# lab4d-org/lab4d

Hardware: AMD Instinct MI355X
Metric: rendered rays/sec (fwd+bwd) at 512² × 128 samples; PSNR vs ref (higher is better)
Workload: dtype bf16

## Files before the change

include/lab4d_mlp.h:

```cpp
#ifndef LAB4D_MLP_H
#define LAB4D_MLP_H

#include <stdint.h>

#define LAB4D_MLP_MAX_LAYERS 12

#define LAB4D_NET_FG_BASE 0
#define LAB4D_NET_FG_COLOR 1
#define LAB4D_NET_VIS 2
#define LAB4D_NET_FEAT 3
#define LAB4D_NET_SKIN 4
#define LAB4D_NET_DENSE 5
#define LAB4D_NET_BG_BASE 6
#define LAB4D_NET_BG_COLOR 7
#define LAB4D_NET_SKIN18 8
#define LAB4D_NET_HASH_GEO 9
#define LAB4D_NET_HASH_COLOR 10
#define LAB4D_NET_DENSE6 11
#define LAB4D_NET_SKIN_A 12
#define LAB4D_NET_SKIN18_A 13
#define LAB4D_NET_COUNT 14

#define LAB4D_PREC_F32 0
#define LAB4D_PREC_BF16 1

typedef struct {
  int ke;
  int kin;
  int mout;
  int mout_pad;
  int relu;
  int pf_bias;
  int add_ext;
  int ext_grad;
} lab4d_mlp_layer;

typedef struct {
  int n_layers;
  int emb_kind;
  int n_freq;
  int c_in;
  int emb_slots;
  int ke;
  int c_out;
  lab4d_mlp_layer layers[LAB4D_MLP_MAX_LAYERS];
} lab4d_mlp_desc;

int lab4d_mlp_describe(int net, lab4d_mlp_desc* out);

int64_t lab4d_mlp_packed_bytes(int net, int layer, int precision);

int lab4d_mlp_pack(int net, int layer, int precision, int transposed, const float* W_ref, int k_ref,
                   const int32_t* col_map, void* packed, void* stream);

typedef struct {
  int net, precision;
  int S;
  int S_pad;
  int ld;
  int spf;
  const float* x;
  const float* freq_w;
  const void* W[LAB4D_MLP_MAX_LAYERS];
  const float* bias[LAB4D_MLP_MAX_LAYERS];
  const float* pf_bias[LAB4D_MLP_MAX_LAYERS];
  void* act[LAB4D_MLP_MAX_LAYERS];
  void* mask[LAB4D_MLP_MAX_LAYERS];
  void* emb;
  const void* ext;
  float* out;
  const float* x2;
  const int32_t* S_dev;
  const int32_t* frame_idx;
  const float* aff;
} lab4d_mlp_fwd_args;
int lab4d_mlp_forward(const lab4d_mlp_fwd_args* a, void* stream);

typedef struct {
  int net, precision, S, spf;
  const float* x;
  const float* freq_w;
  const float* aff;
  const void* W[LAB4D_MLP_MAX_LAYERS];
  const void* WT[LAB4D_MLP_MAX_LAYERS];
  const float* bias[LAB4D_MLP_MAX_LAYERS];
  const float* pf_bias[LAB4D_MLP_MAX_LAYERS];
  const float* d_out;
  float* d_x;
  float* g_aff;
  float* dW[LAB4D_MLP_MAX_LAYERS];
  float* db[LAB4D_MLP_MAX_LAYERS];
  float* pf_db[LAB4D_MLP_MAX_LAYERS];
} lab4d_mlp_bwd_fused_args;
int lab4d_mlp_backward_fused(const lab4d_mlp_bwd_fused_args* a, void* stream);
int lab4d_mlp_fused_backward_supported(int net, int precision, int spf);

int lab4d_mlp_forward_tangent(const lab4d_mlp_fwd_args* a, void* stream);

typedef struct {
  int net, precision, S, S_pad, ld, spf;
  const void* WT[LAB4D_MLP_MAX_LAYERS];
  const void* act[LAB4D_MLP_MAX_LAYERS];
  const void* mask[LAB4D_MLP_MAX_LAYERS];
  const void* emb;
  const void* ext;
  const float* d_out;
  const void* ext_gin;
  void* ext_gout;
  void* dz[LAB4D_MLP_MAX_LAYERS];
  float* d_x;
  float* d_x2;
  const float* x;
  const float* aff;
  float* g_aff;
} lab4d_mlp_bwd_args;
int lab4d_mlp_backward(const lab4d_mlp_bwd_args* a, void* stream);

int lab4d_mlp_wgrad(int net, int layer, int precision, int S, int S_pad, int ld, int spf, const void* dz, const void* emb,
                    const void* act_prev, float* dW, float* db, float* pf_db, int M, void* stream);
int lab4d_mlp_wgrad_mapped(int net, int layer, int precision, int S, int S_pad, int ld, int spf, const void* dz, const void* emb,
                           const void* act_prev, float* dW_ref, int ld_ref, const int32_t* col_map, float* db, float* pf_db, int M,
                           void* stream);

#endif
```

lab4d_amd/csrc/mlp.hip:

```cpp
#include <cstdlib>
#include "mlp_kernels.hpp"
#include "mlp_fused_bwd.hpp"

namespace lab4d {

struct DwMap {
  const int* cmap;
  int ld, mout, db_rows;
};
__device__ __forceinline__ int dw_col(int k, const DwMap& wm) { return wm.cmap ? wm.cmap[k] : k; }
__device__ __forceinline__ void dw_add(float* dW, int o, int c, int K, const DwMap& wm, float v) {
  if (wm.cmap) {
    if (c >= 0 && o < wm.mout) atomicAdd(dW + (size_t)o * wm.ld + c, v);
  } else {
    atomicAdd(dW + (size_t)o * K + c, v);
  }
}

template <class P, int TM>
__global__ void __launch_bounds__(256) k_mlp_wgrad(const typename P::store_t* __restrict__ dz, const typename P::store_t* __restrict__ emb,
                                                    const typename P::store_t* __restrict__ actp, int mo_tiles, int ke, int kin,
                                                    int S_pad, int chunk, int spf, int cpf, float* __restrict__ dW, float* __restrict__ db, DwMap wm) {
  constexpr int TN = 4;
  constexpr int SPS = P::BF16 ? 16 : 8;
  __shared__ float red[TM * TN * 16 * 64];
  const int lane = threadIdx.x & 63, wid = threadIdx.x >> 6, row = lane & 31, h = lane >> 5;
  const int K = ke + kin, nk_tiles = K / 32;
  const int ob_n = (mo_tiles + TM - 1) / TM, kb_n = (nk_tiles + TN - 1) / TN;
  const int job = blockIdx.x;
  const int c = job / (ob_n * kb_n), rem = job - c * (ob_n * kb_n);
  const int ob = rem / kb_n, kb = rem - ob * kb_n;
  int s_begin, s_end;
  if (cpf > 0) {
    const int m = c / cpf, lc = c - m * cpf;
    s_begin = m * spf + lc * chunk;
    s_end = min(min(S_pad, (m + 1) * spf), s_begin + chunk);
    if (db) db += (size_t)m * (mo_tiles * 32);
    if (s_end == (m + 1) * spf && S_pad - s_end < 64 && S_pad > s_end) s_end = S_pad;
  } else {
    s_begin = c * chunk;
    s_end = min(S_pad, s_begin + chunk);
  }

  f32x16_t acc[TM][TN];
#pragma unroll
  for (int i = 0; i < TM; ++i)
#pragma unroll
    for (int j = 0; j < TN; ++j)
#pragma unroll
      for (int r = 0; r < 16; ++r) acc[i][j][r] = 0.f;
  float rs[TM];
#pragma unroll
  for (int i = 0; i < TM; ++i) rs[i] = 0.f;

  const typename P::store_t* ap[TM];
  const typename P::store_t* bp[TN];
  bool av_[TM], bv_[TN];
  int bF[TN];
#pragma unroll
  for (int i = 0; i < TM; ++i) {
    const int t = ob * TM + i;
    av_[i] = t < mo_tiles;
    ap[i] = dz + (size_t)(32 * (av_[i] ? t : 0) + row) * 64;
  }
#pragma unroll
  for (int j = 0; j < TN; ++j) {
    const int t = kb * TN + j;
    bv_[j] = t < nk_tiles;
    const int kr = 32 * (bv_[j] ? t : 0) + row;
    bp[j] = kr < ke ? emb + (size_t)kr * 64 : actp + (size_t)(kr - ke) * 64;
    bF[j] = kr < ke ? ke : kin;
  }
  const int off = P::BF16 ? 8 * h : 4 * h;
  const int moF = mo_tiles * 32;
  auto load_step = [&](int s, uint4 (&a4)[TM], uint4 (&b4)[TN]) {
    const size_t blk = (size_t)(s >> 6);
    const int in = (s & 63) + off;
#pragma unroll
    for (int i = 0; i < TM; ++i) a4[i] = av_[i] ? *reinterpret_cast<const uint4*>(ap[i] + blk * block_stride(moF) + in) : make_uint4(0, 0, 0, 0);
#pragma unroll
    for (int j = 0; j < TN; ++j) b4[j] = bv_[j] ? *reinterpret_cast<const uint4*>(bp[j] + blk * block_stride(bF[j]) + in) : make_uint4(0, 0, 0, 0);
  };
  auto compute = [&](const uint4 (&a4)[TM], const uint4 (&b4)[TN]) {
    if (kb == 0 && db) {
#pragma unroll
      for (int i = 0; i < TM; ++i) {
        if constexpr (P::BF16) {
          const unsigned int w[4] = {a4[i].x, a4[i].y, a4[i].z, a4[i].w};
#pragma unroll
          for (int q = 0; q < 4; ++q) rs[i] += bf2f((unsigned short)(w[q] & 0xffffu)) + bf2f((unsigned short)(w[q] >> 16));
        } else {
          rs[i] += __uint_as_float(a4[i].x) + __uint_as_float(a4[i].y) + __uint_as_float(a4[i].z) + __uint_as_float(a4[i].w);
        }
      }
    }
#pragma unroll
    for (int i = 0; i < TM; ++i)
#pragma unroll
      for (int j = 0; j < TN; ++j) mma_unit<P>(acc[i][j], a4[i], b4[j]);
  };
  const int step = 4 * SPS;
  int s = s_begin + wid * SPS;
  uint4 a0[TM], b0[TN], a1[TM], b1[TN];
  if (s < s_end) load_step(s, a0, b0);
  while (s < s_end) {
    const int s1 = s + step;
    if (s1 < s_end) load_step(s1, a1, b1);
    compute(a0, b0);
    if (s1 >= s_end) break;
    const int s2 = s1 + step;
    if (s2 < s_end) load_step(s2, a0, b0);
    compute(a1, b1);
    s = s2;
  }
  if (wid == 0) {
#pragma unroll
    for (int i = 0; i < TM; ++i)
#pragma unroll
      for (int j = 0; j < TN; ++j)
#pragma unroll
        for (int r = 0; r < 16; ++r) red[((i * TN + j) * 16 + r) * 64 + lane] = acc[i][j][r];
  }
  __syncthreads();
  if (wid != 0) {
#pragma unroll
    for (int i = 0; i < TM; ++i)
#pragma unroll
      for (int j = 0; j < TN; ++j)
#pragma unroll
        for (int r = 0; r < 16; ++r) atomicAdd(&red[((i * TN + j) * 16 + r) * 64 + lane], acc[i][j][r]);
  }
  __syncthreads();
  for (int e = threadIdx.x; e < TM * TN * 16 * 64; e += 256) {
    const int l2 = e & 63, r = (e >> 6) & 15, ij = e >> 10;
    const int i = ij / TN, j = ij - i * TN;
    const int to = ob * TM + i, tk = kb * TN + j;
    if (to < mo_tiles && tk < nk_tiles) {
      const int o = 32 * to + drow(r, l2 >> 5);
      const int k = 32 * tk + (l2 & 31);
      dw_add(dW, o, dw_col(k, wm), K, wm, red[e]);
    }
  }
  if (kb == 0 && db) {
#pragma unroll
    for (int i = 0; i < TM; ++i) {
      const float v = rs[i] + __shfl_xor(rs[i], 32, 64);
      if (h == 0 && av_[i] && 32 * (ob * TM + i) + row < wm.db_rows) atomicAdd(db + 32 * (ob * TM + i) + row, v);
    }
  }
}

template <class P>
__global__ void __launch_bounds__(256) k_mlp_wgrad_big(const typename P::store_t* __restrict__ dz, const typename P::store_t* __restrict__ emb,
                                                        const typename P::store_t* __restrict__ actp, int mo_tiles, int ke, int kin,
                                                        int S_pad, int chunk, int spf, int cpf, float* __restrict__ dW, float* __restrict__ db, DwMap wm) {
  constexpr int TM = 4, TN = 4;
  constexpr int SPS = P::BF16 ? 16 : 8;
  const int lane = threadIdx.x & 63, wid = threadIdx.x >> 6, row = lane & 31, h = lane >> 5;
  const int wr = wid >> 1, wc = wid & 1;
  const int K = ke + kin, nk_tiles = K / 32;
  const int ob_n = (mo_tiles + 7) / 8, kb_n = (nk_tiles + 7) / 8;
  const int job = blockIdx.x;
  const int c = job / (ob_n * kb_n), rem = job - c * (ob_n * kb_n);
  const int ob = rem / kb_n, kb = rem - ob * kb_n;
  int s_begin, s_end;
  if (cpf > 0) {
    const int m = c / cpf, lc = c - m * cpf;
    s_begin = m * spf + lc * chunk;
    s_end = min(min(S_pad, (m + 1) * spf), s_begin + chunk);
    if (db) db += (size_t)m * (mo_tiles * 32);
  } else {
    s_begin = c * chunk;
    s_end = min(S_pad, s_begin + chunk);
  }
  f32x16_t acc[TM][TN];
#pragma unroll
  for (int i = 0; i < TM; ++i)
#pragma unroll
    for (int j = 0; j < TN; ++j)
#pragma unroll
      for (int r = 0; r < 16; ++r) acc[i][j][r] = 0.f;
  float rs[TM];
#pragma unroll
  for (int i = 0; i < TM; ++i) rs[i] = 0.f;
  const typename P::store_t* ap[TM];
  const typename P::store_t* bp[TN];
  bool av_[TM], bv_[TN];
  int bF[TN];
#pragma unroll
  for (int i = 0; i < TM; ++i) {
    const int t = ob * 8 + wr * 4 + i;
    av_[i] = t < mo_tiles;
    ap[i] = dz + (size_t)(32 * (av_[i] ? t : 0) + row) * 64;
  }
#pragma unroll
  for (int j = 0; j < TN; ++j) {
    const int t = kb * 8 + wc * 4 + j;
    bv_[j] = t < nk_tiles;
    const int kr = 32 * (bv_[j] ? t : 0) + row;
    bp[j] = kr < ke ? emb + (size_t)kr * 64 : actp + (size_t)(kr - ke) * 64;
    bF[j] = kr < ke ? ke : kin;
  }
  const bool any = (av_[0] && bv_[0]);
  const bool do_db = (kb == 0 && wc == 0 && db != nullptr);
  const int off = P::BF16 ? 8 * h : 4 * h;
  const int moF = mo_tiles * 32;
  auto load_step = [&](int s, uint4 (&a4)[TM], uint4 (&b4)[TN]) {
    const size_t blk = (size_t)(s >> 6);
    const int in = (s & 63) + off;
#pragma unroll
    for (int i = 0; i < TM; ++i) a4[i] = av_[i] ? *reinterpret_cast<const uint4*>(ap[i] + blk * block_stride(moF) + in) : make_uint4(0, 0, 0, 0);
#pragma unroll
    for (int j = 0; j < TN; ++j) b4[j] = bv_[j] ? *reinterpret_cast<const uint4*>(bp[j] + blk * block_stride(bF[j]) + in) : make_uint4(0, 0, 0, 0);
  };
  auto compute = [&](const uint4 (&a4)[TM], const uint4 (&b4)[TN]) {
    if (do_db) {
#pragma unroll
      for (int i = 0; i < TM; ++i) {
        if constexpr (P::BF16) {
          const unsigned int w[4] = {a4[i].x, a4[i].y, a4[i].z, a4[i].w};
#pragma unroll
          for (int q = 0; q < 4; ++q) rs[i] += bf2f((unsigned short)(w[q] & 0xffffu)) + bf2f((unsigned short)(w[q] >> 16));
        } else {
          rs[i] += __uint_as_float(a4[i].x) + __uint_as_float(a4[i].y) + __uint_as_float(a4[i].z) + __uint_as_float(a4[i].w);
        }
      }
    }
#pragma unroll
    for (int i = 0; i < TM; ++i)
#pragma unroll
      for (int j = 0; j < TN; ++j) mma_unit<P>(acc[i][j], a4[i], b4[j]);
  };
  if (any) {
    int s = s_begin;
    uint4 a0[TM], b0[TN], a1[TM], b1[TN];
    if (s < s_end) load_step(s, a0, b0);
    while (s < s_end) {
      const int s1 = s + SPS;
      if (s1 < s_end) load_step(s1, a1, b1);
      compute(a0, b0);
      if (s1 >= s_end) break;
      const int s2 = s1 + SPS;
      if (s2 < s_end) load_step(s2, a0, b0);
      compute(a1, b1);
      s = s2;
    }
#pragma unroll
    for (int i = 0; i < TM; ++i) {
      if (!av_[i]) continue;
#pragma unroll
      for (int j = 0; j < TN; ++j) {
        if (!bv_[j]) continue;
        const int c = dw_col(32 * (kb * 8 + wc * 4 + j) + row, wm);
#pragma unroll
        for (int r = 0; r < 16; ++r) {
          const int o = 32 * (ob * 8 + wr * 4 + i) + drow(r, h);
          dw_add(dW, o, c, K, wm, acc[i][j][r]);
        }
      }
      if (do_db) {
        const float v = rs[i] + __shfl_xor(rs[i], 32, 64);
        if (h == 0 && 32 * (ob * 8 + wr * 4 + i) + row < wm.db_rows) atomicAdd(db + 32 * (ob * 8 + wr * 4 + i) + row, v);
      }
    }
  }
}

__device__ __forceinline__ void dma_1k(const void* gsrc_lane, void* lds_wave_base) {
  __builtin_amdgcn_global_load_lds((const __attribute__((address_space(1))) unsigned int*)gsrc_lane,
                                   (__attribute__((address_space(3))) unsigned int*)lds_wave_base, 16, 0, 0);
}
template <int OFF>
__device__ __forceinline__ u32x4_t lds_read16(unsigned addr) {
  u32x4_t v;
  asm volatile("ds_read_b128 %0, %1 offset:%2" : "=v"(v) : "v"(addr), "n"(OFF));
  return v;
}

template <int V>
using IC = std::integral_constant<int, V>;

template <int N>
__device__ __forceinline__ void wait_vmcnt() {
  asm volatile("s_waitcnt vmcnt(%0)" ::"n"(N) : "memory");
}

template <int MT, int NBW, int NW = 4, int WC = 2>
__global__ void __launch_bounds__(64 * NW) k_mlp_wgrad_dma(const unsigned short* __restrict__ dz, const unsigned short* __restrict__ emb,
                                                        const unsigned short* __restrict__ actp, int ke, int kin, int S_pad, int chunk,
                                                        int spf, int cpf, float* __restrict__ dW, float* __restrict__ db, DwMap wm) {
  using P = PBF16;
  static_assert(NW == 4 || NW == 8, "wave grid");
  constexpr int WR = NW / WC;
  static_assert(WR * WC == NW && (2 * NBW) % WC == 0, "wave grid");
  constexpr int TM = MT / WR, TN = 2 * NBW / WC, MO = 32 * MT, KB = 64 * NBW;
  static_assert(TM >= 1 && TM * WR == MT, "row tiles per wave");
  constexpr int A_BYTES = MT * 2048, STAGE = A_BYTES + NBW * 4096;
  constexpr int NS0 = 65536 / STAGE, NSTAGE = NS0 < 4 ? 4 : (NS0 > 8 ? 8 : NS0);
  constexpr int PA = (2 * MT + NW - 1) / NW, PB = (4 * NBW + NW - 1) / NW, PW = PA + PB;
  static_assert(PA * NW == 2 * MT || MT == 1, "A pieces per wave (MT = 1: two pieces, the other waves re-fetch the last one)");
  constexpr int AHEAD = NSTAGE - 1;
  constexpr bool DB_MFMA = WC == 2;
  static_assert(PW * (NSTAGE - 2) <= 63, "vmcnt range");
  static_assert(TM + TN <= 15, "lgkmcnt range");
  static_assert(NSTAGE * STAGE <= 160 * 1024, "LDS");
  __shared__ __attribute__((aligned(16))) unsigned char lds[NSTAGE * STAGE];
  const int lane = threadIdx.x & 63, wid = __builtin_amdgcn_readfirstlane((int)(threadIdx.x >> 6)), row = lane & 31, h = lane >> 5;
  const int wr = wid / WC, wc = wid % WC;
  const int K = ke + kin;
  const int kb_n = (K + KB - 1) / KB;
  const int job = blockIdx.x;
  const int c = job / kb_n, kb = job - c * kb_n;
  int s_begin, s_end;
  if (cpf > 0) {
    const int m = c / cpf, lc = c - m * cpf;
    s_begin = m * spf + lc * chunk;
    s_end = min(min(S_pad, (m + 1) * spf), s_begin + chunk);
    if (db) db += (size_t)m * MO;
  } else {
    s_begin = c * chunk;
    s_end = min(S_pad, s_begin + chunk);
  }
  const int k0 = kb * KB, nb = min(KB, K - k0);
  const int n1 = k0 < ke ? min(nb, ke - k0) : 0;
  const int r2 = (k0 > ke ? k0 : ke) - ke;
  bool bv_[TN];
#pragma unroll
  for (int j = 0; j < TN; ++j) bv_[j] = (wc * TN + j) * 32 < nb;
  const bool do_db = (kb == 0 && wc == 0 && db != nullptr);

  f32x16_t acc[TM][TN];
#pragma unroll
  for (int i = 0; i < TM; ++i)
#pragma unroll
    for (int j = 0; j < TN; ++j)
#pragma unroll
      for (int r = 0; r < 16; ++r) acc[i][j][r] = 0.f;
  float rs[TM];
  f32x4_t dbacc[TM];
#pragma unroll
  for (int i = 0; i < TM; ++i) {
    rs[i] = 0.f;
    dbacc[i] = f32x4_t{0.f, 0.f, 0.f, 0.f};
  }

  const int lane_src = (lane >> 2) * 128 + (((lane & 3) ^ ((lane >> 4) & 3)) * 16);
  const int nbp = nb / 16;
  auto issue = [&](int st_idx, int buf) {
    int blk = (s_begin >> 6) + (st_idx >> 1);
    const int half = st_idx & 1;
#ifdef LAB4D_ABL_WGRAD_L2
    blk &= 31;
#endif
    unsigned char* st = lds + buf * STAGE;
    const unsigned char* ga = reinterpret_cast<const unsigned char*>(dz + (size_t)blk * block_stride(MO)) + half * 64 + lane_src;
#pragma unroll
    for (int p = 0; p < PA; ++p) {
      int piece = wid + NW * p;
      if constexpr (PA * NW != 2 * MT) piece = piece < 2 * MT ? piece : 2 * MT - 1;
      dma_1k(ga + piece * 2048, st + piece * 1024);
    }
    unsigned char* sb = st + A_BYTES;
    const unsigned char* g1 = reinterpret_cast<const unsigned char*>(emb + (size_t)blk * block_stride(ke) + (size_t)k0 * 64) + half * 64 + lane_src;
    const unsigned char* g2 = reinterpret_cast<const unsigned char*>(actp + (size_t)blk * block_stride(kin) + (size_t)r2 * 64) + half * 64 + lane_src;
#pragma unroll
    for (int p = 0; p < PB; ++p) {
      int q = wid + NW * p;
      q = q < nbp ? q : nbp - 1;
      const int r0 = 16 * q;
      const unsigned char* src = r0 < n1 ? g1 + (size_t)r0 * 128 : g2 + (size_t)(r0 - n1) * 128;
      dma_1k(src, sb + q * 1024);
    }
  };
  const unsigned lds_base = (unsigned)(size_t)(__attribute__((address_space(3))) unsigned char*)lds;
  const unsigned f = (row >> 2) & 3;
  const unsigned la0 = lds_base + (unsigned)((wr * TM * 32 + row) * 64) + ((unsigned)(h ^ f) * 16u);
  const unsigned lb0 = lds_base + (unsigned)A_BYTES + (unsigned)((wc * TN * 32 + row) * 64) + ((unsigned)(h ^ f) * 16u);
  auto read_frags = [&](int buf, auto subc, u32x4_t (&a4)[TM], u32x4_t (&b4)[TN]) {
    constexpr unsigned X = 32u * decltype(subc)::value;
    const unsigned xa = (la0 + (unsigned)buf * STAGE) ^ X, xb = (lb0 + (unsigned)buf * STAGE) ^ X;
    sfor<0, TM>([&](auto ic) { a4[decltype(ic)::value] = lds_read16<decltype(ic)::value * 2048>(xa); });
    sfor<0, TN>([&](auto jc) { b4[decltype(jc)::value] = lds_read16<decltype(jc)::value * 2048>(xb); });
  };
  auto wait_frags = [&](auto cntc, u32x4_t (&a4)[TM], u32x4_t (&b4)[TN]) {
    constexpr int CNT = decltype(cntc)::value;
    if constexpr (TM == 4) asm volatile("s_waitcnt lgkmcnt(%4)" : "+v"(a4[0]), "+v"(a4[1]), "+v"(a4[2]), "+v"(a4[3]) : "n"(CNT));
    else if constexpr (TM == 2) asm volatile("s_waitcnt lgkmcnt(%2)" : "+v"(a4[0]), "+v"(a4[1]) : "n"(CNT));
    else asm volatile("s_waitcnt lgkmcnt(%1)" : "+v"(a4[0]) : "n"(CNT));
    if constexpr (TN == 5) asm volatile("" : "+v"(b4[0]), "+v"(b4[1]), "+v"(b4[2]), "+v"(b4[3]), "+v"(b4[4]));
    else if constexpr (TN == 4) asm volatile("" : "+v"(b4[0]), "+v"(b4[1]), "+v"(b4[2]), "+v"(b4[3]));
    else if constexpr (TN == 3) asm volatile("" : "+v"(b4[0]), "+v"(b4[1]), "+v"(b4[2]));
    else if constexpr (TN == 2) asm volatile("" : "+v"(b4[0]), "+v"(b4[1]));
    else asm volatile("" : "+v"(b4[0]));
    __builtin_amdgcn_sched_barrier(0);
  };
  const unsigned one2 = (((lane & 15) ^ (lane >> 4)) & 1) == 0 ? 0x3f803f80u : 0u;
  const u32x4_t ones4 = {one2, one2, one2, one2};
  auto mfmas = [&](const u32x4_t (&a4)[TM], const u32x4_t (&b4)[TN]) {
    if (do_db) {
      if constexpr (DB_MFMA) {
        bf16x8_t ov;
        __builtin_memcpy(&ov, &ones4, 16);
#pragma unroll
        for (int i = 0; i < TM; ++i) {
          bf16x8_t av;
          __builtin_memcpy(&av, &a4[i], 16);
          dbacc[i] = __builtin_amdgcn_mfma_f32_16x16x32_bf16(av, ov, dbacc[i], 0, 0, 0);
        }
      } else {
#pragma unroll
        for (int i = 0; i < TM; ++i) {
          const unsigned int w[4] = {a4[i].x, a4[i].y, a4[i].z, a4[i].w};
#pragma unroll
          for (int q = 0; q < 4; ++q) rs[i] += bf2f((unsigned short)(w[q] & 0xffffu)) + bf2f((unsigned short)(w[q] >> 16));
        }
      }
    }
#pragma unroll
    for (int i = 0; i < TM; ++i)
#pragma unroll
      for (int j = 0; j < TN; ++j) {
        bf16x8_t av, bv;
        __builtin_memcpy(&av, &a4[i], 16);
        __builtin_memcpy(&bv, &b4[j], 16);
        acc[i][j] = __builtin_amdgcn_mfma_f32_32x32x16_bf16(av, bv, acc[i][j], 0, 0, 0);
      }
    __builtin_amdgcn_sched_barrier(0);
  };
  auto wait_landed = [&](int later) {
    if (later == NSTAGE - 2) wait_vmcnt<PW * (NSTAGE - 2)>();
    else {
      bool done = false;
      sfor<0, NSTAGE - 2>([&](auto rc) {
        constexpr int R = decltype(rc)::value;
        if (!done && later == R) { wait_vmcnt<PW * R>(); done = true; }
      });
    }
  };
  const int N = ((s_end >> 6) - (s_begin >> 6)) * 2;
  if (N > 0) {
    u32x4_t a0[TM], b0[TN], a1[TM], b1[TN];
#pragma unroll
    for (int i = 0; i < AHEAD; ++i)
      if (i < N) issue(i, i);
    wait_landed(min(AHEAD - 1, N - 1));
    __builtin_amdgcn_s_barrier();
    asm volatile("" ::: "memory");
    read_frags(0, IC<0>{}, a0, b0);
    int buf = 0;
    for (int s = 0; s < N; ++s) {
      const int prev = buf == 0 ? NSTAGE - 1 : buf - 1, next = buf + 1 == NSTAGE ? 0 : buf + 1;
      read_frags(buf, IC<1>{}, a1, b1);
      wait_frags(IC<TM + TN>{}, a0, b0);
      mfmas(a0, b0);
      wait_frags(IC<0>{}, a1, b1);
      if (s + 1 < N) {
        if (s + NSTAGE - 1 < N) issue(s + NSTAGE - 1, prev);
        wait_landed(min(NSTAGE - 2, N - 2 - s));
        __builtin_amdgcn_s_barrier();
        asm volatile("" ::: "memory");
        read_frags(next, IC<0>{}, a0, b0);
        __builtin_amdgcn_sched_barrier(0);
      }
      mfmas(a1, b1);
      buf = next;
    }
  }
#pragma unroll
  for (int i = 0; i < TM; ++i) {
#pragma unroll
    for (int j = 0; j < TN; ++j) {
      if (!bv_[j]) continue;
      const int c = dw_col(k0 + 32 * (wc * TN + j) + row, wm);
#pragma unroll
      for (int r = 0; r < 16; ++r) {
        const int o = 32 * (wr * TM + i) + drow(r, h);
        dw_add(dW, o, c, K, wm, acc[i][j][r]);
      }
    }
    if (do_db) {
      if constexpr (DB_MFMA) {
        if ((lane & 15) < 2) {
#pragma unroll
          for (int r = 0; r < 4; ++r) {
            const int o = 32 * (wr * TM + i) + 16 * (lane & 15) + 4 * (lane >> 4) + r;
            if (o < wm.db_rows) atomicAdd(db + o, dbacc[i][r]);
          }
        }
      } else {
        const float v = rs[i] + __shfl_xor(rs[i], 32, 64);
        if (h == 0 && 32 * (wr * TM + i) + row < wm.db_rows) atomicAdd(db + 32 * (wr * TM + i) + row, v);
      }
    }
  }
}

template <class P>
__global__ void __launch_bounds__(256) k_rowsum_pf(const typename P::store_t* __restrict__ dz, int mo_pad, int S, int ld, int spf,
                                                    int M, int nseg, float* __restrict__ pf_db) {
  constexpr int SEG = 4096;
  const int lane = threadIdx.x & 63;
  const long job = (long)blockIdx.x * 4 + (threadIdx.x >> 6);
  if (job >= (long)mo_pad * nseg) return;
  const int o = (int)(job / nseg), seg = (int)(job % nseg);
  const long b = (long)seg * SEG, e = min((long)S, b + SEG);
  const typename P::store_t* row = dz + (size_t)o * 64;
  long i = b;
  while (i < e) {
    const int m = (int)(i / spf);
    const long fe = min(e, (long)(m + 1) * spf);
    float s = 0.f;
    for (long k = i + lane; k < fe; k += 64) {
      const size_t idx = (size_t)(k >> 6) * block_stride(mo_pad) + (k & 63);
      if constexpr (P::BF16) s += bf2f(row[idx]);
      else s += row[idx];
    }
    s = wave_sum(s);
    if (lane == 0) atomicAdd(pf_db + (size_t)m * mo_pad + o, s);
    i = fe;
  }
}

template <class P>
__global__ void __launch_bounds__(256) k_pack(const float* __restrict__ Wref, int mout, int k_ref, const int32_t* __restrict__ col_map,
                                               int ke, int kin, int mo_pad, int transposed, typename P::store_t* __restrict__ out) {
  constexpr int EPL = P::BF16 ? 8 : 4;
  const int K = ke + kin;
  const int rows = transposed ? K : mo_pad;
  const int kdim = transposed ? mo_pad : K;
  const int G = kdim / P::FPG;
  const long total = (long)(rows / 32) * G * 64 * EPL;
  for (long e = (long)blockIdx.x * blockDim.x + threadIdx.x; e < total; e += (long)gridDim.x * blockDim.x) {
    const int j = (int)(e % EPL);
    const int lane = (int)((e / EPL) % 64);
    const int g = (int)((e / (EPL * 64)) % G);
    const int mt = (int)(e / ((long)EPL * 64 * G));
    const int row = 32 * mt + (lane & 31), h = lane >> 5;
    const int ge = transposed ? 0 : ke / P::FPG;
    int kk;
    if (g < ge) {
      kk = P::BF16 ? 16 * g + 8 * h + j : 2 * (4 * g + j) + h;
    } else {
      const int gg = g - ge;
      int b, r;
      if (P::BF16) { b = gg >> 1; r = 8 * (gg & 1) + j; }
      else { const int kap = 4 * gg + j; b = kap >> 4; r = kap & 15; }
      kk = (transposed ? 0 : ke) + 32 * b + drow(r, h);
    }
    const int o = transposed ? kk : row;
    const int c = transposed ? row : kk;
    float v = 0.f;
    if (o < mout && c < K) {
      const int cr = col_map[c];
      if (cr >= 0) v = Wref[(size_t)o * k_ref + cr];
    }
    if constexpr (P::BF16) out[e] = f2bf(v);
    else out[e] = v;
  }
}

}
using namespace lab4d;

namespace {

template <class F>
int with_net(int net, F&& f) {
  switch (net) {
    case LAB4D_NET_FG_BASE: return f(NetFgBase{});
    case LAB4D_NET_FG_COLOR: return f(NetFgColor{});
    case LAB4D_NET_VIS: return f(NetVis{});
    case LAB4D_NET_FEAT: return f(NetFeat{});
    case LAB4D_NET_SKIN: return f(NetSkin{});
    case LAB4D_NET_SKIN18: return f(NetSkin18{});
    case LAB4D_NET_SKIN_A: return f(NetSkinA{});
    case LAB4D_NET_SKIN18_A: return f(NetSkin18A{});
    case LAB4D_NET_DENSE: return f(NetDense{});
    case LAB4D_NET_DENSE6: return f(NetDense6{});
    case LAB4D_NET_BG_BASE: return f(NetBgBase{});
    case LAB4D_NET_BG_COLOR: return f(NetBgColor{});
    case LAB4D_NET_HASH_GEO: return f(NetHashGeo{});
    case LAB4D_NET_HASH_COLOR: return f(NetHashColor{});
    default: set_error("unknown net id %d", net); return LAB4D_EINVAL;
  }
}

}

extern "C" int lab4d_mlp_describe(int net, lab4d_mlp_desc* out) {
  LAB4D_REQUIRE(out, "mlp_describe: null out");
  memset(out, 0, sizeof(*out));
  return with_net(net, [&](auto n) { fill_desc<decltype(n)>(out); return LAB4D_OK; });
}

extern "C" int64_t lab4d_mlp_packed_bytes(int net, int layer, int precision) {
  lab4d_mlp_desc d;
  if (lab4d_mlp_describe(net, &d) != LAB4D_OK || layer < 0 || layer >= d.n_layers) return -1;
  const lab4d_mlp_layer& L = d.layers[layer];
  return (int64_t)L.mout_pad * (L.ke + L.kin) * (precision == LAB4D_PREC_BF16 ? 2 : 4);
}

extern "C" int lab4d_mlp_pack(int net, int layer, int precision, int transposed, const float* W_ref, int k_ref,
                              const int32_t* col_map, void* packed, void* stream) {
  lab4d_mlp_desc d;
  if (int e = lab4d_mlp_describe(net, &d)) return e;
  LAB4D_REQUIRE(layer >= 0 && layer < d.n_layers, "mlp_pack: bad layer %d", layer);
  LAB4D_REQUIRE(W_ref && col_map && packed, "mlp_pack: null pointer");
  const lab4d_mlp_layer& L = d.layers[layer];
  const long total = (long)L.mout_pad * (L.ke + L.kin);
  int grid = div_up(total, 256); if (grid > 2048) grid = 2048;
  if (precision == LAB4D_PREC_BF16)
    hipLaunchKernelGGL((k_pack<PBF16>), dim3(grid), dim3(256), 0, (hipStream_t)stream, W_ref, L.mout, k_ref, col_map, L.ke, L.kin,
                       L.mout_pad, transposed, (unsigned short*)packed);
  else if (precision == LAB4D_PREC_F32)
    hipLaunchKernelGGL((k_pack<PF32>), dim3(grid), dim3(256), 0, (hipStream_t)stream, W_ref, L.mout, k_ref, col_map, L.ke, L.kin,
                       L.mout_pad, transposed, (float*)packed);
  else { set_error("mlp_pack: bad precision %d", precision); return LAB4D_EINVAL; }
  return check_launch("mlp_pack");
}

extern "C" int lab4d_mlp_forward(const lab4d_mlp_fwd_args* a, void* stream) {
  LAB4D_REQUIRE(a, "mlp_forward: null args");
  LAB4D_REQUIRE(a->S >= 0 && a->S_pad >= a->S && a->S_pad % 256 == 0 && a->spf > 0 && a->ld >= a->S_pad && a->ld % 8 == 0,
                "mlp_forward: bad sizes (S_pad must be a multiple of 256) S=%d S_pad=%d ld=%d spf=%d", a->S, a->S_pad, a->ld, a->spf);
  LAB4D_REQUIRE(a->x && a->out, "mlp_forward: null x/out");
  if (a->S == 0) return LAB4D_OK;
  return with_net(a->net, [&](auto n) {
    using Net = decltype(n);
    FwdK k;
    memset(&k, 0, sizeof(k));
    k.S = a->S; k.S_pad = a->S_pad; k.ld = a->ld; k.spf = a->spf; k.x = a->x; k.freq_w = a->freq_w; k.emb = a->emb; k.ext = a->ext; k.out = a->out; k.x2 = a->x2;
    k.S_dev = a->S_dev; k.frame_idx = a->frame_idx; k.aff = a->aff;
    LAB4D_REQUIRE(!a->aff || Net::EMB != 0, "mlp_forward: aff is for the raw-input nets only");
    LAB4D_REQUIRE(Net::EMB != 2 || a->aff, "mlp_forward: this network needs the per-frame affine table aff (M, ke, 4)");
    LAB4D_REQUIRE(!Net::AUX3 || a->x2, "mlp_forward: this network needs the second input x2");
    LAB4D_REQUIRE(!(a->S_dev && a->emb), "mlp_forward: a device-side sample count is for the evaluation path (no stored activations)");
    for (int l = 0; l < Net::NL; ++l) {
      LAB4D_REQUIRE(a->W[l] && a->bias[l], "mlp_forward: layer %d weights/bias missing", l);
      LAB4D_REQUIRE(!Net::L[l].pf || a->pf_bias[l], "mlp_forward: layer %d needs a per-frame bias", l);
      LAB4D_REQUIRE(!Net::L[l].add_ext || a->ext, "mlp_forward: layer %d needs ext", l);
      if (a->emb && l + 1 < Net::NL) {
        LAB4D_REQUIRE(a->act[l] || (dx_only_ok<Net>() && !a->act[0]), "mlp_forward: training mode (emb != NULL) needs act[%d]", l);
        LAB4D_REQUIRE(!Net::L[l].relu || a->mask[l], "mlp_forward: training mode (emb != NULL) needs mask[%d]", l);
      }
      k.W[l] = a->W[l]; k.bias[l] = a->bias[l]; k.pf_bias[l] = a->pf_bias[l]; k.act[l] = a->act[l]; k.mask[l] = (unsigned int*)a->mask[l];
    }
    return launch_mlp_fwd<Net>(a->precision, k, a->S, (hipStream_t)stream);
  });
}

extern "C" int lab4d_mlp_backward(const lab4d_mlp_bwd_args* a, void* stream) {
  LAB4D_REQUIRE(a, "mlp_backward: null args");
  LAB4D_REQUIRE(a->S >= 0 && a->S_pad >= a->S && a->S_pad % 256 == 0 && a->spf > 0 && a->ld >= a->S_pad && a->ld % 8 == 0, "mlp_backward: bad sizes (S_pad must be a multiple of 256)");
  LAB4D_REQUIRE(a->d_out, "mlp_backward: null d_out");
  if (a->S == 0) return LAB4D_OK;
  return with_net(a->net, [&](auto n) {
    using Net = decltype(n);
    BwdK k;
    memset(&k, 0, sizeof(k));
    k.S = a->S; k.S_pad = a->S_pad; k.ld = a->ld; k.spf = a->spf; k.emb = a->emb; k.ext = a->ext; k.d_out = a->d_out; k.ext_gin = a->ext_gin;
    k.ext_gout = a->ext_gout; k.d_x = a->d_x; k.d_x2 = a->d_x2; k.x = a->x; k.aff = a->aff; k.g_aff = a->g_aff;
    if (Net::EMB == 2) {
      LAB4D_REQUIRE(a->x && a->aff && a->emb, "mlp_backward: this network needs x, aff and the stored embedding");
    } else {
      LAB4D_REQUIRE(!a->g_aff, "mlp_backward: g_aff is for the affine-first-layer nets only");
    }
    LAB4D_REQUIRE(!(a->d_x && Net::EMB == 0) || a->emb, "mlp_backward: d_x needs the stored embedding");
    for (int l = 0; l < Net::NL; ++l) {
      LAB4D_REQUIRE(a->WT[l], "mlp_backward: layer %d transposed weights missing", l);
      LAB4D_REQUIRE(!(Net::L[l].relu && l + 1 < Net::NL) || a->mask[l], "mlp_backward: layer %d ReLU mask missing", l);
      LAB4D_REQUIRE(!Net::L[l].ext_grad || a->ext_gin, "mlp_backward: layer %d needs ext_gin", l);
      LAB4D_REQUIRE(a->dz[l] || (dx_only_ok<Net>() && !a->dz[0] && a->d_x), "mlp_backward: dz[%d] missing (every layer's dZ is written, or none: point gradient only)", l);
      LAB4D_REQUIRE(!Net::L[l].add_ext || a->ext_gout, "mlp_backward: layer %d needs ext_gout", l);
      k.WT[l] = a->WT[l]; k.act[l] = a->act[l]; k.mask[l] = (const unsigned int*)a->mask[l]; k.dz[l] = a->dz[l];
    }
    return launch_mlp_bwd<Net>(a->precision, k, a->S, (hipStream_t)stream);
  });
}

extern "C" int lab4d_mlp_fused_backward_supported(int net, int precision, int spf) {
  if (precision != LAB4D_PREC_BF16 || spf <= 0 || spf % 64 != 0) return 0;
  static const int vis_env = getenv("LAB4D_FUSED_VIS") ? atoi(getenv("LAB4D_FUSED_VIS")) : 0;
  return net == LAB4D_NET_SKIN_A || net == LAB4D_NET_SKIN18_A || (net == LAB4D_NET_VIS && vis_env != 0);
}

extern "C" int lab4d_mlp_backward_fused(const lab4d_mlp_bwd_fused_args* a, void* stream) {
  LAB4D_REQUIRE(a, "mlp_backward_fused: null args");
  LAB4D_REQUIRE(lab4d_mlp_fused_backward_supported(a->net, a->precision, a->spf), "mlp_backward_fused: net %d / precision %d / spf %d not supported (bf16, narrow nets, spf %% 64 == 0)",
                a->net, a->precision, a->spf);
  LAB4D_REQUIRE(a->S >= 0 && a->x && a->d_out, "mlp_backward_fused: null x / d_out");
  if (a->S == 0) return LAB4D_OK;
  auto run = [&](auto n) {
    using Net = decltype(n);
    FusedK k;
    memset(&k, 0, sizeof(k));
    k.S = a->S; k.spf = a->spf; k.ntiles = (a->S + 63) / 64; k.x = a->x; k.freq_w = a->freq_w; k.aff = a->aff; k.d_out = a->d_out; k.d_x = a->d_x; k.g_aff = a->g_aff;
    LAB4D_REQUIRE(Net::EMB != 2 || a->aff, "mlp_backward_fused: this network needs the per-frame affine table aff");
    for (int l = 0; l < Net::NL; ++l) {
      LAB4D_REQUIRE(a->WT[l] && a->dW[l], "mlp_backward_fused: layer %d transposed weights / dW missing", l);
      LAB4D_REQUIRE(l + 1 == Net::NL || (a->W[l] && (Net::L[l].pf ? (const void*)a->pf_bias[l] : (const void*)a->bias[l])), "mlp_backward_fused: layer %d forward weights / bias missing", l);
      LAB4D_REQUIRE((((uintptr_t)a->W[l] | (uintptr_t)a->WT[l]) & 15) == 0, "mlp_backward_fused: packed weights must be 16-byte aligned");
      k.W[l] = a->W[l]; k.WT[l] = a->WT[l]; k.bias[l] = a->bias[l]; k.pf_bias[l] = a->pf_bias[l]; k.dW[l] = a->dW[l]; k.db[l] = a->db[l]; k.pf_db[l] = a->pf_db[l];
    }
    return launch_mlp_bwd_fused<Net>(k, (hipStream_t)stream);
  };
  switch (a->net) {
    case LAB4D_NET_VIS: return run(NetVis{});
    case LAB4D_NET_SKIN_A: return run(NetSkinA{});
    default: return run(NetSkin18A{});
  }
}

extern "C" int lab4d_mlp_wgrad(int net, int layer, int precision, int S, int S_pad, int ld, int spf, const void* dz, const void* emb,
                               const void* act_prev, float* dW, float* db, float* pf_db, int M, void* stream) {
  return lab4d_mlp_wgrad_mapped(net, layer, precision, S, S_pad, ld, spf, dz, emb, act_prev, dW, 0, nullptr, db, pf_db, M, stream);
}

extern "C" int lab4d_mlp_wgrad_mapped(int net, int layer, int precision, int S, int S_pad, int ld, int spf, const void* dz, const void* emb,
                                      const void* act_prev, float* dW, int ld_ref, const int32_t* col_map, float* db, float* pf_db, int M,
                                      void* stream) {
  lab4d_mlp_desc d;
  if (int e = lab4d_mlp_describe(net, &d)) return e;
  LAB4D_REQUIRE(layer >= 0 && layer < d.n_layers, "mlp_wgrad: bad layer %d", layer);
  const lab4d_mlp_layer& L = d.layers[layer];
  LAB4D_REQUIRE(dz && dW, "mlp_wgrad: null dz/dW");
  LAB4D_REQUIRE(col_map == nullptr || ld_ref > 0, "mlp_wgrad_mapped: a column map needs the reference row stride");
  LAB4D_REQUIRE(L.ke == 0 || emb, "mlp_wgrad: layer %d needs the stored embedding", layer);
  LAB4D_REQUIRE(L.kin == 0 || act_prev, "mlp_wgrad: layer %d needs the previous activation", layer);
  LAB4D_REQUIRE(S_pad % 64 == 0 && S_pad >= S && ld >= S_pad && ld % 8 == 0, "mlp_wgrad: bad S_pad/ld");
  if (S == 0) return LAB4D_OK;
  const int mo_tiles = L.mout_pad / 32, nk_tiles = (L.ke + L.kin) / 32;
  const bool big = mo_tiles >= 8;
  const int Kt = L.ke + L.kin;
  static const int head_dma = getenv("LAB4D_WGRAD_HEAD_DMA") ? atoi(getenv("LAB4D_WGRAD_HEAD_DMA")) : 1;
  const bool dma = precision == LAB4D_PREC_BF16 && (mo_tiles == 8 || mo_tiles == 4 || mo_tiles == 2 || (mo_tiles == 1 && head_dma && Kt <= 256));
  const int nbw = (dma && mo_tiles == 1) ? (Kt <= 128 ? 2 : 4)
                  : Kt <= 64 ? 1 : (Kt <= 128 ? 2 : (Kt <= 192 ? 3 : (Kt <= 256 ? 4 : (mo_tiles == 8 && Kt <= 320 ? 5 : 3))));
  const int TM = mo_tiles >= 4 ? 4 : (mo_tiles >= 2 ? 2 : 1);
  const int ob_n = dma ? 1 : (big ? div_up(mo_tiles, 8) : div_up(mo_tiles, TM));
  const int kb_n = dma ? div_up(Kt, 64 * nbw) : (big ? div_up(nk_tiles, 8) : div_up(nk_tiles, 4));
  static const int jobs_env = getenv("LAB4D_WGRAD_JOBS") ? atoi(getenv("LAB4D_WGRAD_JOBS")) : 0;
  const int jobs_target = jobs_env > 0 ? jobs_env : ((dma && mo_tiles < 8) ? 512 : 256);
  int nchunks = jobs_target / (ob_n * kb_n); if (nchunks < 1) nchunks = 1;
  int chunk = div_up(div_up(S_pad, nchunks), 256) * 256; if (chunk < 1024) chunk = 1024;
  const bool fold_pf = pf_db != nullptr && spf % 256 == 0 && M > 0 && (long)M * spf >= S;
  LAB4D_REQUIRE(pf_db == nullptr || fold_pf || (M > 0 && spf > 0 && (long)M * spf >= S), "mlp_wgrad: pf_db needs M and spf, with M * spf >= S");
  int cpf = 0;
  if (fold_pf) {
    if (chunk > spf) chunk = spf;
    cpf = div_up(spf, chunk);
    nchunks = cpf * M;
  } else {
    nchunks = div_up(S_pad, chunk);
  }
  const int jobs = ob_n * kb_n * nchunks;
  const dim3 grid(jobs), block(256), block8(512);
  float* db_arg = fold_pf ? pf_db : db;
  const DwMap wm = {col_map, ld_ref, L.mout, (col_map && !fold_pf) ? L.mout : L.mout_pad};
  hipStream_t st = (hipStream_t)stream;
#define WG(P, TMV) hipLaunchKernelGGL((k_mlp_wgrad<P, TMV>), grid, block, 0, st, (const typename P::store_t*)dz, (const typename P::store_t*)emb, \
                                      (const typename P::store_t*)act_prev, mo_tiles, L.ke, L.kin, S_pad, chunk, spf, cpf, dW, db_arg, wm)
#define WGB(P) hipLaunchKernelGGL((k_mlp_wgrad_big<P>), grid, block, 0, st, (const typename P::store_t*)dz, (const typename P::store_t*)emb, \
                                  (const typename P::store_t*)act_prev, mo_tiles, L.ke, L.kin, S_pad, chunk, spf, cpf, dW, db_arg, wm)
#define WGD(MTV, NBV) hipLaunchKernelGGL((k_mlp_wgrad_dma<MTV, NBV>), grid, block, 0, st, (const unsigned short*)dz, (const unsigned short*)emb, \
                                         (const unsigned short*)act_prev, L.ke, L.kin, S_pad, chunk, spf, cpf, dW, db_arg, wm)
#define WGD8(NBV) hipLaunchKernelGGL((k_mlp_wgrad_dma<8, NBV, 8>), grid, block8, 0, st, (const unsigned short*)dz, (const unsigned short*)emb, \
                                     (const unsigned short*)act_prev, L.ke, L.kin, S_pad, chunk, spf, cpf, dW, db_arg, wm)
#define WGD_NB(MTV) do { if (nbw == 1) WGD(MTV, 1); else if (nbw == 2) WGD(MTV, 2); else if (nbw == 3) WGD(MTV, 3); else WGD(MTV, 4); } while (0)
  if (dma) {
    if (mo_tiles == 8) {
      if (nbw == 1) WGD8(1); else if (nbw == 2) WGD8(2); else if (nbw == 3) WGD8(3); else if (nbw == 4) WGD8(4); else WGD8(5);
    } else if (mo_tiles == 4) WGD_NB(4); else if (mo_tiles == 2) WGD_NB(2);
    else if (nbw == 2) hipLaunchKernelGGL((k_mlp_wgrad_dma<1, 2, 4, 4>), grid, block, 0, st, (const unsigned short*)dz, (const unsigned short*)emb,
                                          (const unsigned short*)act_prev, L.ke, L.kin, S_pad, chunk, spf, cpf, dW, db_arg, wm);
    else hipLaunchKernelGGL((k_mlp_wgrad_dma<1, 4, 4, 4>), grid, block, 0, st, (const unsigned short*)dz, (const unsigned short*)emb,
                            (const unsigned short*)act_prev, L.ke, L.kin, S_pad, chunk, spf, cpf, dW, db_arg, wm);
  }
#undef WGD_NB
#undef WGD8
#undef WGD
  else if (precision == LAB4D_PREC_BF16) { if (big) WGB(PBF16); else if (TM == 4) WG(PBF16, 4); else if (TM == 2) WG(PBF16, 2); else WG(PBF16, 1); }
  else if (precision == LAB4D_PREC_F32) { if (big) WGB(PF32); else if (TM == 4) WG(PF32, 4); else if (TM == 2) WG(PF32, 2); else WG(PF32, 1); }
  else { set_error("mlp_wgrad: bad precision %d", precision); return LAB4D_EINVAL; }
#undef WGB
#undef WG
  if (int e = check_launch("mlp_wgrad")) return e;
  if (pf_db && !fold_pf) {
    const int nseg = div_up(S, 4096);
    const long jobs2 = (long)L.mout_pad * nseg;
    if (precision == LAB4D_PREC_BF16)
      hipLaunchKernelGGL((k_rowsum_pf<PBF16>), dim3(div_up(jobs2, 4)), dim3(256), 0, st, (const unsigned short*)dz, L.mout_pad, S, ld, spf, M, nseg, pf_db);
    else
      hipLaunchKernelGGL((k_rowsum_pf<PF32>), dim3(div_up(jobs2, 4)), dim3(256), 0, st, (const float*)dz, L.mout_pad, S, ld, spf, M, nseg, pf_db);
    return check_launch("mlp_rowsum_pf");
  }
  return LAB4D_OK;
}

namespace {
template <class Net>
int forward_tangent_impl(const lab4d_mlp_fwd_args* a, void* stream) {
  FwdK k;
  memset(&k, 0, sizeof(k));
  k.S = a->S; k.S_pad = a->S_pad; k.ld = a->ld; k.spf = a->spf; k.x = a->x; k.emb = a->emb; k.out = a->out;
  for (int l = 0; l < Net::NL; ++l) {
    LAB4D_REQUIRE(a->W[l], "mlp_forward_tangent: layer %d weights missing", l);
    LAB4D_REQUIRE(!(Net::L[l].relu) || a->mask[l], "mlp_forward_tangent: layer %d primal ReLU mask missing", l);
    LAB4D_REQUIRE(l + 1 == Net::NL || a->act[l], "mlp_forward_tangent: act[%d] missing", l);
    k.W[l] = a->W[l]; k.bias[l] = a->bias[l] ? a->bias[l] : (const float*)a->W[l]; k.act[l] = a->act[l]; k.mask[l] = (unsigned int*)a->mask[l];
  }
  return launch_mlp_fwd_tangent<Net>(a->precision, k, a->S, (hipStream_t)stream);
}
}

extern "C" int lab4d_mlp_forward_tangent(const lab4d_mlp_fwd_args* a, void* stream) {
  LAB4D_REQUIRE(a, "mlp_forward_tangent: null args");
  LAB4D_REQUIRE(a->net == LAB4D_NET_FG_BASE || a->net == LAB4D_NET_BG_BASE,
                "mlp_forward_tangent: only the basefield/sdf networks (fg, bg) have an eikonal term (got net %d)", a->net);
  LAB4D_REQUIRE(a->S >= 0 && a->S_pad >= a->S && a->S_pad % 256 == 0 && a->spf > 0, "mlp_forward_tangent: bad sizes (S_pad must be a multiple of 256)");
  LAB4D_REQUIRE(a->x && a->emb, "mlp_forward_tangent: null x / emb");
  if (a->S == 0) return LAB4D_OK;
  if (a->net == LAB4D_NET_FG_BASE) return forward_tangent_impl<NetFgBase>(a, stream);
  return forward_tangent_impl<NetBgBase>(a, stream);
}
```

lab4d_amd/csrc/mlp_kernels.hpp:

```cpp
#pragma once
#include <cstddef>
#include <cstdlib>
#include <type_traits>

#include "common.hpp"
#include "mlp_nets.hpp"

namespace lab4d {

typedef __attribute__((ext_vector_type(8))) short bf16x8_t;
typedef __attribute__((ext_vector_type(16))) float f32x16_t;

struct PBF16 {
  static constexpr bool BF16 = true;
  static constexpr int NT = 2, TILE = 64, FPG = 16, UPT = 2;
  using store_t = unsigned short;
};
struct PF32 {
  static constexpr bool BF16 = false;
  static constexpr int NT = 1, TILE = 32, FPG = 8, UPT = 4;
  using store_t = float;
};

__device__ __forceinline__ unsigned short f2bf(float x) {
// ... 639 lines not shown
            float w[4];
#pragma unroll
            for (int e = 0; e < 4; ++e) {
              float v0, v1;
              emb_pair<Net>(4 * g + e, x, a.freq_w, v0, v1);
              w[e] = h ? v1 : v0;
            }
            emb[t][g] = make_uint4(__float_as_uint(w[0]), __float_as_uint(w[1]), __float_as_uint(w[2]), __float_as_uint(w[3]));
          }
        }
      } else {
        const float* xr = stagef + (NT * n + t) * CINR;
#pragma unroll
        for (int g = 0; g < UE; ++g) {
          if constexpr (P::BF16) {
            float v[8];
#pragma unroll
            for (int j = 0; j < 8; ++j) {
              const int c = 16 * g + 8 * h + j;
              v[j] = c < CINR ? xr[c] : 0.f;
            }
            emb[t][g] = make_uint4(pack2bf(v[0], v[1]), pack2bf(v[2], v[3]), pack2bf(v[4], v[5]), pack2bf(v[6], v[7]));
          } else {
            float v[4];
#pragma unroll
            for (int e = 0; e < 4; ++e) {
              const int c = 2 * (4 * g + e) + h;
              v[e] = c < CINR ? xr[c] : 0.f;
            }
            emb[t][g] = make_uint4(__float_as_uint(v[0]), __float_as_uint(v[1]), __float_as_uint(v[2]), __float_as_uint(v[3]));
          }
        }
      }
    }
    if constexpr (ST) {
      const int q = n & 3, kq = n >> 2;
      GLOBAL_AS char* base = (GLOBAL_AS char*)a.emb + tile_base_offset<P>(KE, s0, 0);
#pragma unroll
      for (int g = 0; g < UE; ++g) {
        if constexpr (P::BF16) {
          const unsigned int w0[4] = {emb[0][g].x, emb[0][g].y, emb[0][g].z, emb[0][g].w};
          const unsigned int w1[4] = {emb[1][g].x, emb[1][g].y, emb[1][g].z, emb[1][g].w};
#pragma unroll
          for (int half = 0; half < 2; ++half) {
            unsigned int d[4];
#pragma unroll
            for (int jj = 0; jj < 4; ++jj) {
              const int j = 4 * half + jj;
              const unsigned int lo = (w0[j >> 1] >> (16 * (j & 1))) & 0xffffu, hi = (w1[j >> 1] >> (16 * (j & 1))) & 0xffffu;
              d[jj] = lo | (hi << 16);
            }
            quad_transpose(d, q);
            gst16(base + tile_lane_offset<P>(16 * g + 8 * h + 4 * half + q, kq), d[0], d[1], d[2], d[3]);
          }
        } else {
          unsigned int d[4] = {emb[0][g].x, emb[0][g].y, emb[0][g].z, emb[0][g].w};
          quad_transpose(d, q);
          gst16(base + tile_lane_offset<P>(2 * (4 * g + q) + h, kq), d[0], d[1], d[2], d[3]);
        }
      }
    }

#pragma nounroll
    for (int l = 0; l < Net::NL; ++l)
    sfor<0, Net::NL>([&](auto ri) {
      constexpr int R = decltype(ri)::value;
      if constexpr (fwd_rep<Net>(R) != R) return;
      constexpr unsigned MEMBERS = fwd_members<Net>(R);
      if (!((MEMBERS >> l) & 1u)) return;
      constexpr LS ls = Net::L[R];
      constexpr bool LAST = (R == Net::NL - 1);
      constexpr int MT = pad32(ls.mout) / 32;
      constexpr int GE = ls.ke / P::FPG, GA = ls.kin / P::FPG, G = GE + GA;
      constexpr int GL = G < ACG ? G : ACG, NQ = (GL + 3) / 4;
      const GLOBAL_AS void* Wl = KARG_PTR(FwdK, const void*, W, l);
      const GLOBAL_AS float* bl = KARG_PTR(FwdK, const float*, bias, l);
      const GLOBAL_AS float* pfl = KARG_PTR(FwdK, const float*, pf_bias, l);
      GLOBAL_AS unsigned int* maskl = KARG_PTR(FwdK, unsigned int*, mask, l);
      GLOBAL_AS void* actl = KARG_PTR(FwdK, void*, act, l);
      uint4 bin[NT][GA > 0 ? GA : 1];
#pragma unroll
      for (int t = 0; t < NT; ++t)
#pragma unroll
        for (int u = 0; u < GA; ++u) bin[t][u] = slab[(t * UW + u) * 64];
      constexpr int NB = (ls.pf != 0 && !TAN) ? NT : 1;
      auto load_bias = [&](int mt, f32x16_t (&bv)[NB]) {
        if constexpr (TAN) {
#pragma unroll
          for (int r = 0; r < 16; ++r) bv[0][r] = 0.f;
        } else {
#pragma unroll
          for (int t = 0; t < NB; ++t)
#pragma unroll
            for (int i = 0; i < 4; ++i) {
              const GLOBAL_AS float* src = (ls.pf != 0) ? pfl + (size_t)frame[t] * (32 * MT) : bl;
              const f32x4_t v = *(const GLOBAL_AS f32x4_t*)(src + 32 * mt + 8 * i + 4 * h);
              bv[t][4 * i + 0] = v.x; bv[t][4 * i + 1] = v.y; bv[t][4 * i + 2] = v.z; bv[t][4 * i + 3] = v.w;
            }
        }
      };
      auto mfma_tile = [&](auto has_pre, int pre, int rbuf, uint4 (&A)[G], f32x16_t (&bv)[NB], f32x16_t (&acc)[NT]) {
        constexpr bool PRE = decltype(has_pre)::value;
#pragma unroll
        for (int t = 0; t < NT; ++t) acc[t] = bv[NB == 1 ? 0 : t];
#pragma unroll
        for (int g = 0; g < G; ++g) {
#pragma unroll
          for (int t = 0; t < NT; ++t) mma_unit<P>(acc[t], A[g], g < GE ? emb[t][g < GE ? g : 0] : bin[t][g >= GE ? g - GE : 0]);
          if constexpr (PRE) {
            if (g >= GL) A[g] = load_a(Wl, G, pre, g, lane);
            else if (rbuf >= 0) A[g] = abuf[(rbuf * ACG + g) * 64 + lane];
          }
        }
        if constexpr (PRE) load_bias(pre, bv);
      };
      auto a_fetch = [&](int mt, uint4 (&stg)[NQ]) {
#pragma unroll
        for (int i = 0; i < NQ; ++i) {
          const int g = wid + 4 * i < GL ? wid + 4 * i : GL - 1;
          stg[i] = load_a(Wl, G, mt, g, lane);
        }
      };
      auto a_stash = [&](int buf, const uint4 (&stg)[NQ]) {
#pragma unroll
        for (int i = 0; i < NQ; ++i) {
          const int g = wid + 4 * i < GL ? wid + 4 * i : GL - 1;
          abuf[(buf * ACG + g) * 64 + lane] = stg[i];
        }
      };
      auto a_grab = [&](int buf, uint4 (&A)[G]) {
#pragma unroll
        for (int g = 0; g < GL; ++g) A[g] = abuf[(buf * ACG + g) * 64 + lane];
      };
      unsigned int tan_bits = 0;
      uint4 ext_raw[4];
      auto prefetch = [&](int mt) {
        if constexpr (TAN && ls.relu != 0) tan_bits = maskl[((size_t)tile * MT + mt) * 64 + lane];
        if constexpr (ls.add_ext != 0 && !TAN) load_tile_raw<P>((const GLOBAL_AS void*)a.ext, 32 * MT, s0, mt, lane, ext_raw);
      };
      constexpr bool PACKED = P::BF16 && !TAN && ls.add_ext == 0 && !LAST;
      auto epilogue = [&](int mt, f32x16_t (&acc)[NT], unsigned int (&w)[2][8], unsigned int& wbits) {
        if constexpr (PACKED) {
#pragma unroll
          for (int t = 0; t < NT; ++t) acc_fence_if<(want_occ<Net, P>() == 2)>(acc[t]);
#pragma unroll
          for (int t = 0; t < 2; ++t)
#pragma unroll
            for (int k = 0; k < 8; ++k) w[t][k] = pack2bf_op(acc[t][2 * k], acc[t][2 * k + 1]);
          if constexpr (ls.relu != 0) {
            if constexpr (ST) wbits = pk_alive_bits(w);
#pragma unroll
            for (int t = 0; t < 2; ++t)
#pragma unroll
              for (int k = 0; k < 8; ++k) w[t][k] = pk_relu_bf16(w[t][k]);
          }
#pragma unroll
          for (int t = 0; t < 2; ++t)
#pragma unroll
            for (int q = 0; q < 2; ++q) slab[(t * UW + 2 * mt + q) * 64] = make_uint4(w[t][4 * q], w[t][4 * q + 1], w[t][4 * q + 2], w[t][4 * q + 3]);
          return;
        }
        if constexpr (ls.relu != 0) {
          if constexpr (TAN) {
            const unsigned int bits = tan_bits;
#pragma unroll
            for (int t = 0; t < NT; ++t)
#pragma unroll
              for (int r = 0; r < 16; ++r)
                acc[t][r] = __uint_as_float(__float_as_uint(acc[t][r]) & (unsigned int)__builtin_amdgcn_sbfe((int)bits, mask_bit<P>(t, r), 1));
          } else {
            if constexpr (ST && !LAST) {
              unsigned int bits = 0;
#pragma unroll
              for (int t = 0; t < NT; ++t)
#pragma unroll
                for (int r = 0; r < 16; ++r) bits |= (acc[t][r] > 0.f ? 1u : 0u) << mask_bit<P>(t, r);
              maskl[((size_t)tile * MT + mt) * 64 + lane] = bits;
            }
#pragma unroll
            for (int t = 0; t < NT; ++t)
#pragma unroll
              for (int r = 0; r < 16; ++r) acc[t][r] = relu1(acc[t][r]);
          }
        }
        if constexpr (ls.add_ext != 0 && !TAN) {
          f32x16_t e[NT];
          tile_from_raw<P>(ext_raw, lane, e);
#pragma unroll
          for (int t = 0; t < NT; ++t)
#pragma unroll
            for (int r = 0; r < 16; ++r) acc[t][r] += e[t][r];
        }
        if constexpr (ST) {
          if constexpr (!LAST && ACTS) store_tile<P>(actl, 32 * MT, s0, mt, lane, acc);
        } else if constexpr (fwd_any_export<Net>(R)) {
          if (actl) store_tile<P>(actl, 32 * MT, s0, mt, lane, acc);
        }
        if constexpr (!LAST) {
#pragma unroll
          for (int t = 0; t < NT; ++t) {
            uint4 u[P::UPT];
            tile_to_units<P>(acc[t], u);
#pragma unroll
            for (int q = 0; q < P::UPT; ++q) slab[(t * UW + P::UPT * mt + q) * 64] = u[q];
          }
        } else if constexpr (head_staged<Net>() && !TAN) {
          static_assert(pad32(Net::COUT) == 32, "one row tile");
          __builtin_amdgcn_wave_barrier();
#pragma unroll
          for (int t = 0; t < NT; ++t)
#pragma unroll
            for (int r = 0; r < 16; ++r) {
              const int f = drow(r, h);
              if (f < Net::COUT) stagef[(NT * n + t) * Net::COUT + f] = acc[t][r];
            }
          __builtin_amdgcn_wave_barrier();
          if (a.out) stage_out(stagef, a.out, (long)s0 * Net::COUT, TILE * Net::COUT, (long)S_eff * Net::COUT - 1, lane);
          __builtin_amdgcn_wave_barrier();
        } else {
#pragma unroll
          for (int t = 0; t < NT; ++t)
#pragma unroll
            for (int r = 0; r < 16; ++r) {
              const int f = 32 * mt + drow(r, h);
              if (f < Net::COUT && sidx[t] < S_eff && a.out) a.out[(size_t)sidx[t] * Net::COUT + f] = acc[t][r];
            }
        }
      };
      auto flush = [&](int mt, const unsigned int (&w)[2][8], unsigned int wbits) {
        if constexpr (PACKED) {
          if constexpr (ST) {
            if constexpr (ls.relu != 0) maskl[((size_t)tile * MT + mt) * 64 + lane] = wbits;
            if constexpr (ACTS) store_tile_packed(actl, 32 * MT, s0, mt, lane, w);
          } else if constexpr (fwd_any_export<Net>(R)) {
            if (actl) store_tile_packed(actl, 32 * MT, s0, mt, lane, w);
          }
        }
      };
      uint4 A[G], stg[NQ];
      f32x16_t bv[NB];
      f32x16_t acc0[NT], acc1[NT];
      unsigned int pw[2][8], pbits = 0;
      wg_step_barrier();
      a_fetch(0, stg);
      a_stash(0, stg);
      if constexpr (MT > 1) {
        a_fetch(1, stg);
        a_stash(1, stg);
      }
      a_fetch(MT > 2 ? 2 : MT - 1, stg);
#pragma unroll
      for (int g = GL; g < G; ++g) A[g] = load_a(Wl, G, 0, g, lane);
      load_bias(0, bv);
      prefetch(0);
      wg_step_barrier();
      a_grab(0, A);
      constexpr int NSTEP = MT - 1, NPAIR = NSTEP / 2;
      mfma_tile(std::bool_constant<(MT > 1)>{}, 1, -1, A, bv, acc0);
      if constexpr (NPAIR > 0) {
#pragma nounroll
        for (int k = 0; k < 2 * NPAIR; k += 2) {
          wg_step_barrier();
          a_grab(1, A);
          mfma_tile(std::true_type{}, k + 2 < MT ? k + 2 : MT - 1, -1, A, bv, acc1);
          epilogue(k, acc0, pw, pbits);
          prefetch(k + 1);
          a_stash(0, stg);
          a_fetch(k + 3 < MT ? k + 3 : MT - 1, stg);
          flush(k, pw, pbits);
          wg_step_barrier();
          a_grab(0, A);
          mfma_tile(std::true_type{}, k + 3 < MT ? k + 3 : MT - 1, -1, A, bv, acc0);
          epilogue(k + 1, acc1, pw, pbits);
          prefetch(k + 2 < MT ? k + 2 : MT - 1);
          a_stash(1, stg);
          a_fetch(k + 4 < MT ? k + 4 : MT - 1, stg);
          flush(k + 1, pw, pbits);
        }
      }
      if constexpr (NSTEP % 2 == 1) {
        wg_step_barrier();
        a_grab(1, A);
        mfma_tile(std::false_type{}, 0, -1, A, bv, acc1);
        epilogue(MT - 2, acc0, pw, pbits);
        flush(MT - 2, pw, pbits);
        prefetch(MT - 1);
        epilogue(MT - 1, acc1, pw, pbits);
        flush(MT - 1, pw, pbits);
      } else {
        epilogue(MT - 1, acc0, pw, pbits);
        flush(MT - 1, pw, pbits);
      }
    });
  }
}

template <class Net>
constexpr int emb_layer_count() {
  int c = 0;
  for (int l = 0; l < Net::NL; ++l) c += Net::L[l].ke ? 1 : 0;
  return c;
}

template <class Net, class P, bool AU = true, bool DZ = true>
__global__ void __launch_bounds__(256, (want_occ<Net, P, true>())) k_mlp_bwd(BwdK a) {
  static_assert(Net::EMB == 0 || emb_layer_count<Net>() == 1, "raw-input nets may use the input in one layer only");
  constexpr int NT = P::NT, TILE = P::TILE, NL = Net::NL, UW = Slab<Net, P>::UW;
  constexpr int ACG = acache_g<Net, P>();
  __shared__ uint4 slab_all[4 * Slab<Net, P>::UNITS_PER_WAVE];
  __shared__ uint4 abuf0[ACG * 64];
  __shared__ uint4 abuf1[ACG * 64];
#define LAB4D_ABUF(buf) ((buf) ? abuf1 : abuf0)
  __shared__ float4 afftab[Net::EMB == 2 ? 4 * 96 : 1];
  constexpr int NGA = (Net::EMB == 2 && AU) ? (Net::KE / 32) * 16 * 4 : 1;
  float gacc[NGA];
#pragma unroll
  for (int i = 0; i < NGA; ++i) gacc[i] = 0.f;
  int gframe = -1;
  auto gram_flush = [&]() {
    if constexpr (Net::EMB == 2 && AU) {
      if (gframe >= 0 && a.g_aff != nullptr) {
#pragma unroll
        for (int i = 0; i < NGA; ++i) {
          float v = gacc[i];
#pragma unroll
          for (int off = 1; off < 32; off <<= 1) v += __shfl_xor(v, off, 64);
          const int mt = i / 64, r = (i >> 2) & 15, j = i & 3;
          if ((threadIdx.x & 31) == 0) atomicAdd(a.g_aff + ((size_t)gframe * Net::KE + 32 * mt + drow(r, (int)((threadIdx.x & 63) >> 5))) * 4 + j, v);
          gacc[i] = 0.f;
        }
      }
    }
  };
  const int lane = threadIdx.x & 63, n = lane & 31, h = lane >> 5;
  const int wid = __builtin_amdgcn_readfirstlane((int)(threadIdx.x >> 6));
  uint4* slab = slab_all + wid * Slab<Net, P>::UNITS_PER_WAVE + lane;
  float* stagef = reinterpret_cast<float*>(slab_all + wid * Slab<Net, P>::UNITS_PER_WAVE);
  const int wave = blockIdx.x * 4 + wid, nwaves = gridDim.x * 4;

  for (int tile = wave; tile < a.ntiles; tile += nwaves) {
    const int s0 = tile * TILE;
    int sidx[NT];
#pragma unroll
    for (int t = 0; t < NT; ++t) sidx[t] = s0 + NT * n + t;
    float dx[NT][3];
    float dx2[NT][3];
#pragma unroll
    for (int t = 0; t < NT; ++t) { dx[t][0] = dx[t][1] = dx[t][2] = 0.f; dx2[t][0] = dx2[t][1] = dx2[t][2] = 0.f; }
    float xs[NT][3];
    int frm[NT];
    float4* ltab = afftab + wid * 96;
    constexpr bool uni = AU;
    if constexpr (Net::EMB == 2) {
#pragma unroll
      for (int t = 0; t < NT; ++t) {
        const int sc = sidx[t] < a.S ? sidx[t] : a.S - 1;
        frm[t] = sc / a.spf;
#pragma unroll
        for (int k = 0; k < 3; ++k) xs[t][k] = ((const GLOBAL_AS float*)a.x)[(size_t)sc * 3 + k];
      }
      if constexpr (uni) {
        const int m = __builtin_amdgcn_readfirstlane(frm[0]);
        if (m != gframe) {
          gram_flush();
          gframe = m;
        }
        for (int e = lane; e < Net::KE; e += 64) {
          const f32x4_t r4 = *(const GLOBAL_AS f32x4_t*)((const GLOBAL_AS float4*)a.aff + (size_t)m * Net::KE + e);
          ltab[e] = make_float4(r4.x, r4.y, r4.z, r4.w);
        }
      }
      __builtin_amdgcn_wave_barrier();
    }

    {
      f32x16_t g[NT];
      if constexpr (head_staged<Net>()) {
        __builtin_amdgcn_wave_barrier();
        stage_in<TILE * Net::COUT>(stagef, a.d_out, (long)s0 * Net::COUT, (long)a.S * Net::COUT - 1, lane);
        __builtin_amdgcn_wave_barrier();
#pragma unroll
        for (int t = 0; t < NT; ++t)
#pragma unroll
          for (int r = 0; r < 16; ++r) {
            const int f = drow(r, h);
            g[t][r] = (f < Net::COUT && sidx[t] < a.S) ? stagef[(NT * n + t) * Net::COUT + (f < Net::COUT ? f : 0)] : 0.f;
          }
        __builtin_amdgcn_wave_barrier();
      } else {
#pragma unroll
      for (int t = 0; t < NT; ++t)
#pragma unroll
        for (int r = 0; r < 16; ++r) {
          const int f = drow(r, h);
          g[t][r] = (f < Net::COUT && sidx[t] < a.S) ? a.d_out[(size_t)sidx[t] * Net::COUT + f] : 0.f;
        }
      }
      if constexpr (DZ) store_tile<P>((GLOBAL_AS void*)a.dz[NL - 1], pad32(Net::L[NL - 1].mout), s0, 0, lane, g);
#pragma unroll
      for (int t = 0; t < NT; ++t) {
        uint4 u[P::UPT];
        tile_to_units<P>(g[t], u);
#pragma unroll
        for (int q = 0; q < P::UPT; ++q) slab[(t * UW + q) * 64] = u[q];
      }
    }

#pragma nounroll
    for (int l = NL - 1; l >= 0; --l)
    sfor<0, NL>([&](auto ri) {
      constexpr int R = NL - 1 - decltype(ri)::value;
      if constexpr (bwd_rep<Net>(R) != R) return;
      constexpr unsigned MEMBERS = bwd_members<Net>(R);
      if (!((MEMBERS >> l) & 1u)) return;
      constexpr LS ls = Net::L[R];
      constexpr LS lp = Net::L[R > 0 ? R - 1 : 0];
      constexpr int GK = pad32(ls.mout) / P::FPG;
      constexpr int GL = GK < ACG ? GK : ACG, NQ = (GL + 3) / 4;
      constexpr int MTE = ls.ke / 32, MTA = ls.kin / 32;
      constexpr bool DO_ACT = (R > 0 && MTA > 0);
      const int lm1 = l > 0 ? l - 1 : 0;
      const GLOBAL_AS void* Wt = KARG_PTR(BwdK, const void*, WT, l);
      const GLOBAL_AS unsigned int* maskp = KARG_PTR(BwdK, const unsigned int*, mask, lm1);
      GLOBAL_AS void* dzp = KARG_PTR(BwdK, void*, dz, lm1);
      uint4 bin[NT][GK];
#pragma unroll
      for (int t = 0; t < NT; ++t)
#pragma unroll
        for (int u = 0; u < GK; ++u) bin[t][u] = slab[(t * UW + u) * 64];

      auto mfma_tile = [&](auto has_pre, int pre, int rbuf, uint4 (&A)[GK], f32x16_t (&acc)[NT]) {
        constexpr bool PRE = decltype(has_pre)::value;
#pragma unroll
        for (int t = 0; t < NT; ++t)
#pragma unroll
          for (int r = 0; r < 16; ++r) acc[t][r] = 0.f;
        sfor<0, GK>([&](auto gc) {
          constexpr int g = decltype(gc)::value;
#pragma unroll
          for (int t = 0; t < NT; ++t) mma_unit<P>(acc[t], A[g], bin[t][g]);
          if constexpr (PRE) {
            if (g >= GL) A[g] = load_a(Wt, GK, pre, g, lane);
            else if (rbuf >= 0) A[g] = LAB4D_ABUF(rbuf)[g * 64 + lane];
          }
        });
      };
      auto a_fetch = [&](int mt, uint4 (&stg)[NQ]) {
#pragma unroll
        for (int i = 0; i < NQ; ++i) {
          const int g = wid + 4 * i < GL ? wid + 4 * i : GL - 1;
          stg[i] = load_a(Wt, GK, mt, g, lane);
        }
      };
      auto a_stash = [&](int buf, const uint4 (&stg)[NQ]) {
#pragma unroll
        for (int i = 0; i < NQ; ++i) {
          const int g = wid + 4 * i < GL ? wid + 4 * i : GL - 1;
          LAB4D_ABUF(buf)[g * 64 + lane] = stg[i];
        }
      };
      auto a_grab = [&](int buf, uint4 (&A)[GK]) {
#pragma unroll
        for (int g = 0; g < GL; ++g) A[g] = LAB4D_ABUF(buf)[g * 64 + lane];
      };
      auto pipeline = [&](auto n_c, int tile0, auto&& pre, auto&& epi, auto&& fl, auto&& prem) {
        constexpr int N = decltype(n_c)::value;
        if constexpr (N > 0) {
          uint4 A[GK], stg[NQ];
          f32x16_t acc0[NT], acc1[NT];
          unsigned int pw[2][8];
          wg_step_barrier();
          a_fetch(tile0, stg);
          a_stash(0, stg);
          if constexpr (N > 1) {
            a_fetch(tile0 + 1, stg);
            a_stash(1, stg);
          }
          a_fetch(tile0 + (N > 2 ? 2 : N - 1), stg);
#pragma unroll
          for (int g = GL; g < GK; ++g) A[g] = load_a(Wt, GK, tile0, g, lane);
          pre(0);
          prem(std::integral_constant<int, 0>{}, 0);
          prem(std::integral_constant<int, 1>{}, N > 1 ? 1 : 0);
          wg_step_barrier();
          a_grab(0, A);
          constexpr int NSTEP = N - 1, NPAIR = NSTEP / 2;
          mfma_tile(std::bool_constant<(N > 1)>{}, tile0 + 1, 1, A, acc0);
          if constexpr (N > 1) {
            wg_step_barrier();
            a_stash(0, stg);
            a_fetch(tile0 + (N > 3 ? 3 : N - 1), stg);
          }
          if constexpr (NPAIR > 0) {
#pragma nounroll
            for (int k = 0; k < 2 * NPAIR; k += 2) {
              wg_step_barrier();
              mfma_tile(std::true_type{}, tile0 + (k + 2 < N ? k + 2 : N - 1), 0, A, acc1);
              epi(k, acc0, pw);
              pre(k + 1);
              prem(std::integral_constant<int, 0>{}, k + 2 < N ? k + 2 : N - 1);
              a_stash(1, stg);
              a_fetch(tile0 + (k + 4 < N ? k + 4 : N - 1), stg);
              fl(k, pw);
              wg_step_barrier();
              mfma_tile(std::true_type{}, tile0 + (k + 3 < N ? k + 3 : N - 1), 1, A, acc0);
              epi(k + 1, acc1, pw);
              pre(k + 2 < N ? k + 2 : N - 1);
              prem(std::integral_constant<int, 1>{}, k + 3 < N ? k + 3 : N - 1);
              a_stash(0, stg);
              a_fetch(tile0 + (k + 5 < N ? k + 5 : N - 1), stg);
              fl(k + 1, pw);
            }
          }
          if constexpr (NSTEP % 2 == 1) {
            wg_step_barrier();
            mfma_tile(std::false_type{}, 0, -1, A, acc1);
            epi(N - 2, acc0, pw);
            fl(N - 2, pw);
            pre(N - 1);
            epi(N - 1, acc1, pw);
            fl(N - 1, pw);
          } else {
            epi(N - 1, acc0, pw);
            fl(N - 1, pw);
          }
        }
      };
      uint4 raw[4];
      unsigned int mb0 = 0, mb1 = 0;
      auto no_prem = [&](auto, int) {};
      auto pre_mask = [&](auto par_c, int j) {
        if constexpr (lp.relu != 0) {
          const unsigned int v = maskp[((size_t)tile * (pad32(lp.mout) / 32) + j) * 64 + lane];
          if constexpr (decltype(par_c)::value == 0) mb0 = v; else mb1 = v;
        }
      };
      auto pre_emb = [&](int mt) {
        if constexpr (Net::EMB != 1) load_tile_raw<P>((const GLOBAL_AS void*)a.emb, Net::KE, s0, mt, lane, raw);
      };
      auto pre_act = [&](int j) {
        if constexpr (lp.ext_grad != 0) load_tile_raw<P>((const GLOBAL_AS void*)a.ext_gin, pad32(lp.mout), s0, j, lane, raw);
      };
      auto no_flush = [&](int, const unsigned int (&)[2][8]) {};
      auto epi_emb = [&](int mt, f32x16_t (&acc)[NT], unsigned int (&)[2][8]) {
        if constexpr (Net::EMB == 0) {
          f32x16_t e[NT];
          tile_from_raw<P>(raw, lane, e);
          constexpr int L = Net::NFREQ;
#pragma unroll
          for (int t = 0; t < NT; ++t)
#pragma unroll
            for (int r = 0; r < 16; ++r) {
              const int slot = 32 * mt + drow(r, h);
              const float gv = acc[t][r];
              if (slot < 6 * L) {
                const int pair = slot >> 1, f = pair / 3, ax = pair - 3 * f;
                const float partner = e[t][r ^ 1];
                const float c = ldexpf((r & 1) ? -partner : partner, f) * gv;
                dx[t][0] += ax == 0 ? c : 0.f;
                dx[t][1] += ax == 1 ? c : 0.f;
                dx[t][2] += ax == 2 ? c : 0.f;
              } else if (slot < 6 * L + 3) {
                const int ax = slot - 6 * L;
                dx[t][0] += ax == 0 ? gv : 0.f;
                dx[t][1] += ax == 1 ? gv : 0.f;
                dx[t][2] += ax == 2 ? gv : 0.f;
              } else if (Net::AUX3 && slot < 6 * L + 6) {
                const int ax = slot - 6 * L - 3;
                dx2[t][0] += ax == 0 ? gv : 0.f;
                dx2[t][1] += ax == 1 ? gv : 0.f;
                dx2[t][2] += ax == 2 ? gv : 0.f;
              }
            }
        } else if constexpr (Net::EMB == 2) {
          f32x16_t e[NT];
          tile_from_raw<P>(raw, lane, e);
          auto body = [&](auto uni_c) {
            constexpr bool U = decltype(uni_c)::value;
            sfor<0, 16>([&](auto rc) {
              constexpr int r = decltype(rc)::value;
              const int slot = 32 * mt + drow(r, h);
              float4 row;
              if constexpr (U) row = ltab[slot];
#pragma unroll
              for (int t = 0; t < NT; ++t) {
                if constexpr (!U) {
                  const f32x4_t g4 = *(const GLOBAL_AS f32x4_t*)((const GLOBAL_AS float4*)a.aff + (size_t)frm[t] * Net::KE + slot);
                  row = make_float4(g4.x, g4.y, g4.z, g4.w);
                }
                const float dz = e[t][r] > 0.f ? acc[t][r] : 0.f;
                dx[t][0] += row.x * dz;
                dx[t][1] += row.y * dz;
                dx[t][2] += row.z * dz;
                if constexpr (U) {
                  sfor<0, Net::KE / 32>([&](auto mc) {
                    constexpr int mm = decltype(mc)::value;
                    if (mt == mm) {
                      gacc[(mm * 16 + r) * 4 + 0] += dz * xs[t][0];
                      gacc[(mm * 16 + r) * 4 + 1] += dz * xs[t][1];
                      gacc[(mm * 16 + r) * 4 + 2] += dz * xs[t][2];
                      gacc[(mm * 16 + r) * 4 + 3] += dz;
                    }
                  });
                } else if (a.g_aff != nullptr && dz != 0.f && sidx[t] < a.S) {
                  float* gp = a.g_aff + ((size_t)frm[t] * Net::KE + slot) * 4;
                  atomicAdd(gp + 0, dz * xs[t][0]);
                  atomicAdd(gp + 1, dz * xs[t][1]);
                  atomicAdd(gp + 2, dz * xs[t][2]);
                  atomicAdd(gp + 3, dz);
                }
              }
            });
          };
          body(std::bool_constant<uni>{});
        } else {
#pragma unroll
          for (int t = 0; t < NT; ++t)
#pragma unroll
            for (int r = 0; r < 16; ++r) {
              const int c = 32 * mt + drow(r, h);
              if (c < Net::CIN) stagef[(NT * n + t) * Net::CIN + c] = acc[t][r];
            }
        }
      };
      auto epi_act = [&](int j, f32x16_t (&acc)[NT], unsigned int (&w)[2][8]) {
        const unsigned int bits = (j & 1) ? mb1 : mb0;
        if constexpr (P::BF16) {
#pragma unroll
          for (int t = 0; t < NT; ++t) acc_fence_if<(want_occ<Net, P, true>() == 2)>(acc[t]);
        }
        if constexpr (lp.ext_grad != 0) {
          f32x16_t eg[NT];
          tile_from_raw<P>(raw, lane, eg);
#pragma unroll
          for (int t = 0; t < NT; ++t)
#pragma unroll
            for (int r = 0; r < 16; ++r) acc[t][r] += eg[t][r];
        }
        if constexpr (lp.add_ext != 0) {
          store_tile<P>((GLOBAL_AS void*)a.ext_gout, pad32(lp.mout), s0, j, lane, acc);
        }
        if constexpr (P::BF16) {
#pragma unroll
          for (int t = 0; t < 2; ++t)
#pragma unroll
            for (int k = 0; k < 8; ++k) w[t][k] = pack2bf_op(acc[t][2 * k], acc[t][2 * k + 1]);
          {
            unsigned int alive = lp.relu != 0 ? bits : 0xffffffffu;
#pragma unroll
            for (int t = 0; t < 2; ++t)
              if (sidx[t] >= a.S) alive &= ~(0x00ff00ffu << (8 * t));
#pragma unroll
            for (int t = 0; t < 2; ++t)
#pragma unroll
              for (int k = 0; k < 8; ++k) w[t][k] = pk_mask_bf16(w[t][k], pk_m01(alive, t, k));
          }
#pragma unroll
          for (int t = 0; t < 2; ++t)
#pragma unroll
            for (int q = 0; q < 2; ++q) slab[(t * UW + 2 * j + q) * 64] = make_uint4(w[t][4 * q], w[t][4 * q + 1], w[t][4 * q + 2], w[t][4 * q + 3]);
        } else {
          unsigned int keep = lp.relu != 0 ? bits : 0xffffffffu;
#pragma unroll
          for (int t = 0; t < NT; ++t)
            if (sidx[t] >= a.S) keep &= ~(0xffffu << (16 * t));
#pragma unroll
          for (int t = 0; t < NT; ++t)
#pragma unroll
            for (int r = 0; r < 16; ++r)
              acc[t][r] = __uint_as_float(__float_as_uint(acc[t][r]) & (unsigned int)__builtin_amdgcn_sbfe((int)keep, 16 * t + r, 1));
          if constexpr (DZ) store_tile<P>(dzp, pad32(lp.mout), s0, j, lane, acc);
#pragma unroll
          for (int t = 0; t < NT; ++t) {
            uint4 u[P::UPT];
            tile_to_units<P>(acc[t], u);
#pragma unroll
            for (int q = 0; q < P::UPT; ++q) slab[(t * UW + P::UPT * j + q) * 64] = u[q];
          }
        }
      };
      auto flush_act = [&](int j, const unsigned int (&w)[2][8]) {
        if constexpr (P::BF16 && DZ) store_tile_packed(dzp, pad32(lp.mout), s0, j, lane, w);
      };
      if constexpr (MTE > 0) {
        if (a.d_x != nullptr) {
          pipeline(std::integral_constant<int, MTE>{}, 0, pre_emb, epi_emb, no_flush, no_prem);
          if constexpr (Net::EMB == 1) stage_out(stagef, a.d_x, (long)s0 * Net::CIN, TILE * Net::CIN, (long)a.S * Net::CIN - 1, lane);
        }
      }
      if constexpr (DO_ACT) pipeline(std::integral_constant<int, MTA>{}, MTE, pre_act, epi_act, flush_act, pre_mask);
    });

    if constexpr (Net::EMB != 1) {
      if (a.d_x) {
#pragma unroll
        for (int t = 0; t < NT; ++t) {
#pragma unroll
          for (int k = 0; k < 3; ++k) dx[t][k] += __shfl_xor(dx[t][k], 32, 64);
          if (h == 0 && sidx[t] < a.S) {
            a.d_x[(size_t)sidx[t] * 3 + 0] = dx[t][0];
            a.d_x[(size_t)sidx[t] * 3 + 1] = dx[t][1];
            a.d_x[(size_t)sidx[t] * 3 + 2] = dx[t][2];
          }
          if constexpr (Net::AUX3) {
#pragma unroll
            for (int k = 0; k < 3; ++k) dx2[t][k] += __shfl_xor(dx2[t][k], 32, 64);
            if (h == 0 && sidx[t] < a.S && a.d_x2) {
              a.d_x2[(size_t)sidx[t] * 3 + 0] = dx2[t][0];
              a.d_x2[(size_t)sidx[t] * 3 + 1] = dx2[t][1];
              a.d_x2[(size_t)sidx[t] * 3 + 2] = dx2[t][2];
            }
          }
        }
      }
    }
  }
  gram_flush();
#undef LAB4D_ABUF
}

template <class Net>
int launch_mlp_fwd(int precision, const FwdK& k, int S, hipStream_t st);
template <class Net>
int launch_mlp_bwd(int precision, const BwdK& k, int S, hipStream_t st);
template <class Net>
int launch_mlp_fwd_tangent(int precision, const FwdK& k, int S, hipStream_t st);

template <auto kernel>
inline int mlp_grid(int ntiles) {
  static int per_cu = 0, n_cu = 0;
  if (per_cu == 0) {
    int nb = 0, dev = 0;
    hipDeviceProp_t prop;
    if (hipOccupancyMaxActiveBlocksPerMultiprocessor(&nb, kernel, 256, 0) != hipSuccess || nb < 1) nb = 1;
    if (hipGetDevice(&dev) != hipSuccess || hipGetDeviceProperties(&prop, dev) != hipSuccess) prop.multiProcessorCount = 256;
    n_cu = prop.multiProcessorCount > 0 ? prop.multiProcessorCount : 256;
    per_cu = nb > 2 ? 2 : nb;
  }
  int g = (ntiles + 3) / 4;
  if (g > n_cu * per_cu) g = n_cu * per_cu;
  static const int grid_env = getenv("LAB4D_CHAIN_GRID") ? atoi(getenv("LAB4D_CHAIN_GRID")) : 0;
  if (grid_env > 0 && g > grid_env * per_cu) g = grid_env * per_cu;
  return g < 1 ? 1 : g;
}
#define LAB4D_MLP_LAUNCH(KERNEL, k, st)                                                              \
  do {                                                                                               \
    constexpr auto kfn = &KERNEL;                                                                    \
    hipLaunchKernelGGL(kfn, dim3(mlp_grid<kfn>((k).ntiles)), dim3(256), 0, st, k);                   \
  } while (0)

}
#include "mlp_kernels_ws.hpp"
namespace lab4d {
template <class Net>
constexpr bool dx_only_ok() { return Net::ID == LAB4D_NET_FG_BASE || Net::ID == LAB4D_NET_BG_BASE; }
template <class Net>
inline bool launch_ws_bwd(const BwdK& k0, hipStream_t st) {
  if constexpr (ws_ok<Net>()) {
    if (!ws_enabled()) return false;
    if (!k0.dz[0]) {
      if constexpr (dx_only_ok<Net>()) {
        hipLaunchKernelGGL((k_mlp_bwd_ws<Net, false>), dim3(mlp_grid_ws(k0.S_pad / WS_TILE)), dim3(512), 0, st, k0);
        return true;
      }
      return false;
    }
    hipLaunchKernelGGL((k_mlp_bwd_ws<Net, true>), dim3(mlp_grid_ws(k0.S_pad / WS_TILE)), dim3(512), 0, st, k0);
    return true;
  } else {
    return false;
  }
}
template <class Net>
inline bool launch_ws_fwd(const FwdK& k0, hipStream_t st) {
  if constexpr (ws_ok<Net>()) {
    if (!ws_enabled()) return false;
    FwdK k = k0;
    if (k.emb && !k.act[0]) {
      if constexpr (dx_only_ok<Net>()) {
        hipLaunchKernelGGL((k_mlp_fwd_ws<Net, true, false>), dim3(mlp_grid_ws(k.S_pad / WS_TILE)), dim3(512), 0, st, k);
        return true;
      }
      return false;
    }
    if (k.emb) hipLaunchKernelGGL((k_mlp_fwd_ws<Net, true>), dim3(mlp_grid_ws(k.S_pad / WS_TILE)), dim3(512), 0, st, k);
    else hipLaunchKernelGGL((k_mlp_fwd_ws<Net, false>), dim3(mlp_grid_ws(k.S_pad / WS_TILE)), dim3(512), 0, st, k);
    return true;
  } else {
    return false;
  }
}

#define LAB4D_MLP_INSTANTIATE(Net)                                                                                        \
  namespace lab4d {                                                                                                       \
  template <>                                                                                                             \
  int launch_mlp_fwd<Net>(int precision, const FwdK& k0, int S, hipStream_t st) {                                         \
    FwdK k = k0;                                                                                                          \
    if (precision == LAB4D_PREC_BF16) {                                                                                   \
      if (launch_ws_fwd<Net>(k, st)) return check_launch("mlp_forward");                                                  \
      k.ntiles = k.S_pad / PBF16::TILE;                                                                                   \
      if (k.emb && !k.act[0]) {                                                                                           \
        if constexpr (dx_only_ok<Net>()) LAB4D_MLP_LAUNCH((k_mlp_fwd<Net, PBF16, false, true, false>), k, st);            \
      } else if (k.emb) LAB4D_MLP_LAUNCH((k_mlp_fwd<Net, PBF16, false, true>), k, st);  \
      else LAB4D_MLP_LAUNCH((k_mlp_fwd<Net, PBF16, false, false>), k, st);       \
    } else if (precision == LAB4D_PREC_F32) {                                                                             \
      k.ntiles = k.S_pad / PF32::TILE;                                                                                   \
      if (k.emb && !k.act[0]) {                                                                                           \
        if constexpr (dx_only_ok<Net>()) LAB4D_MLP_LAUNCH((k_mlp_fwd<Net, PF32, false, true, false>), k, st);             \
      } else if (k.emb) LAB4D_MLP_LAUNCH((k_mlp_fwd<Net, PF32, false, true>), k, st);   \
      else LAB4D_MLP_LAUNCH((k_mlp_fwd<Net, PF32, false, false>), k, st);        \
    } else {                                                                                                              \
      set_error("mlp_forward: bad precision %d", precision);                                                              \
      return LAB4D_EINVAL;                                                                                                \
    }                                                                                                                     \
    return check_launch("mlp_forward");                                                                                   \
  }                                                                                                                       \
  template <>                                                                                                             \
  int launch_mlp_bwd<Net>(int precision, const BwdK& k0, int S, hipStream_t st) {                                         \
    BwdK k = k0;                                                                                                          \
    if (precision == LAB4D_PREC_BF16) {                                                                                   \
      if (launch_ws_bwd<Net>(k, st)) return check_launch("mlp_backward");                                                 \
      k.ntiles = k.S_pad / PBF16::TILE;                                                                                   \
      if constexpr (Net::EMB == 2) {                                                                                      \
        if (k.spf % PBF16::TILE) LAB4D_MLP_LAUNCH((k_mlp_bwd<Net, PBF16, false>), k, st);                                 \
        else LAB4D_MLP_LAUNCH((k_mlp_bwd<Net, PBF16, true>), k, st);                                                      \
      } else if (!k.dz[0]) {                                                                                              \
        if constexpr (dx_only_ok<Net>()) LAB4D_MLP_LAUNCH((k_mlp_bwd<Net, PBF16, true, false>), k, st);                   \
      } else LAB4D_MLP_LAUNCH((k_mlp_bwd<Net, PBF16>), k, st);                         \
    } else if (precision == LAB4D_PREC_F32) {                                                                             \
      k.ntiles = k.S_pad / PF32::TILE;                                                                                   \
      if constexpr (Net::EMB == 2) {                                                                                      \
        if (k.spf % PF32::TILE) LAB4D_MLP_LAUNCH((k_mlp_bwd<Net, PF32, false>), k, st);                                   \
        else LAB4D_MLP_LAUNCH((k_mlp_bwd<Net, PF32, true>), k, st);                                                       \
      } else if (!k.dz[0]) {                                                                                              \
        if constexpr (dx_only_ok<Net>()) LAB4D_MLP_LAUNCH((k_mlp_bwd<Net, PF32, true, false>), k, st);                    \
      } else LAB4D_MLP_LAUNCH((k_mlp_bwd<Net, PF32>), k, st);                          \
    } else {                                                                                                              \
      set_error("mlp_backward: bad precision %d", precision);                                                             \
      return LAB4D_EINVAL;                                                                                                \
    }                                                                                                                     \
    return check_launch("mlp_backward");                                                                                  \
  }                                                                                                                       \
  }

}
```

lab4d_amd/csrc/mlp_kernels_ws.hpp:

```cpp
#pragma once
#include "mlp_kernels.hpp"

namespace lab4d {

template <class Net>
constexpr bool ws_ok() {
  if (!(Net::EMB == 0 && Net::AUX3 == 0 && net_wmax<Net>() == 256 && Net::KE % 32 == 0)) return false;
  for (int l = 0; l < Net::NL; ++l) {
    const int mt = pad32(Net::L[l].mout) / 32;
    if (!(mt == 1 || mt == 2 || mt == 4 || mt == 8)) return false;
    if (Net::L[l].kin % 32 != 0 || Net::L[l].kin > 256) return false;
    if (Net::L[l].ke != 0 && Net::L[l].ke != Net::KE) return false;
  }
  return true;
}
template <class Net>
constexpr int ws_g(int l) { return (Net::L[l].ke + Net::L[l].kin) / 16; }
template <class Net>
constexpr int ws_mt(int l) { return pad32(Net::L[l].mout) / 32; }
template <class Net>
constexpr int ws_gmax() {
  int g = 0;
  for (int l = 0; l < Net::NL; ++l) g = ws_g<Net>(l) > g ? ws_g<Net>(l) : g;
  return g;
// ... 317 lines not shown
          gst16(base + tile_lane_offset<P>(16 * g + 8 * h + 4 * half + q, kq), d[0], d[1], d[2], d[3]);
        }
      }
    }
    wg_step_barrier();

#pragma nounroll
    for (int l = 0; l < NL; ++l)
    sfor<0, NL>([&](auto ri) {
      constexpr int R = decltype(ri)::value;
      if constexpr (wsf_rep<Net>(R) != R) return;
      constexpr unsigned MEMBERS = wsf_members<Net>(R);
      if (!((MEMBERS >> l) & 1u)) return;
      constexpr LS ls = Net::L[R];
      constexpr bool LAST = (R == NL - 1);
      constexpr int MT = ws_mt<Net>(R), GE = ls.ke / 16, GA = ls.kin / 16, G = GE + GA;
      constexpr int Gn = ws_g<Net>((R + 1) % NL);
      using IT = WsItems<MT>;
      const GLOBAL_AS float* bl = KARG_PTR(FwdK, const float*, bias, l);
      const GLOBAL_AS float* pfl = KARG_PTR(FwdK, const float*, pf_bias, l);
      const int ln = l + 1 < NL ? l + 1 : 0;
      const GLOBAL_AS void* Wn = Wn_c;
      const int mtn = w & (ws_mt_rt<Net>(ln) - 1);
      const int ib = l & 1;
      const uint4* xin = xbuf + ib * WS_BUF;
      uint4* xout = xbuf + (ib ^ 1) * WS_BUF;
      const int mt = IT::mt(w);
      const bool active = IT::active(w);

      const bool bias_lds_path = ls.pf == 0 || tile_uni;
      u32x4_t br[4];
      auto load_bias = [&](int b, f32x16_t (&bv)[2]) {
        if (bias_lds_path) return;
#pragma unroll
        for (int t = 0; t < (ls.pf != 0 ? 2 : 1); ++t) {
          const int fr = frame[0][t] + b * (frame[1][t] - frame[0][t]);
          const GLOBAL_AS float* src = (ls.pf != 0) ? pfl + (size_t)fr * (32 * MT) : bl;
#pragma unroll
          for (int i = 0; i < 4; ++i) {
            const f32x4_t v = *(const GLOBAL_AS f32x4_t*)(src + 32 * mt + 8 * i + 4 * h);
            bv[t][4 * i + 0] = v.x; bv[t][4 * i + 1] = v.y; bv[t][4 * i + 2] = v.z; bv[t][4 * i + 3] = v.w;
          }
        }
        if constexpr (ls.pf == 0) bv[1] = bv[0];
      };
      uint4 ext_raw[4];
      auto load_ext = [&](int b) {
        if constexpr (ls.add_ext != 0) load_tile_raw<P>((const GLOBAL_AS void*)a.ext, 32 * MT, s0 + 64 * b, mt, lane, ext_raw);
      };

#pragma unroll
      for (int g = G; g < Gn; ++g) A[g] = load_a(Wn, Gn, mtn, g, lane);
      unsigned int tbits[2] = {0xffffffffu, 0xffffffffu};
      if constexpr (TAN && ls.relu != 0 && !LAST) {
        if (active) {
          const GLOBAL_AS unsigned int* mown = KARG_PTR(FwdK, unsigned int*, mask, l);
#pragma unroll
          for (int k = 0; k < IT::IPW; ++k) tbits[k] = mown[((size_t)(2 * tile + IT::blk(w, k)) * MT + mt) * 64 + lane];
        }
      }
      f32x16_t bv[2];
      if (active) {
        if (bias_lds_path) {
          const unsigned ba = lds_addr(bias_lds) + (unsigned)((l * 256 + 32 * mt + 4 * h) * 4);
          ws_lds_read<0>(br[0], ba);
          ws_lds_read<32>(br[1], ba);
          ws_lds_read<64>(br[2], ba);
          ws_lds_read<96>(br[3], ba);
        } else {
          load_bias(IT::blk(w, 0), bv);
        }
        load_ext(IT::blk(w, 0));
      }
      constexpr int MTp = R > 0 ? ws_mt<Net>(R > 0 ? R - 1 : 0) : 1;
      using ITp = WsItems<MTp>;
      constexpr int NP = R > 0 ? 4 * ITp::IPW : 0;
      constexpr int NHOST = IT::IPW;
      constexpr int NPI = NP / NHOST;
      constexpr bool SPREAD = ST && ACTS && R > 0 && !LAST && IT::ITEMS >= 8 && ITp::ITEMS >= 8 && NP % NHOST == 0 && WsSpread<G, (NPI > 0 ? NPI : 1)>::OK;
      GLOBAL_AS void* actp = act_c;
      GLOBAL_AS unsigned int* maskp = mask_c;
      const GLOBAL_AS void* Wn_n = KARG_PTR(FwdK, const void*, W, (ln + 1 < NL ? ln + 1 : 0));
      GLOBAL_AS void* act_n = KARG_PTR(FwdK, void*, act, l);
      GLOBAL_AS unsigned int* mask_n = KARG_PTR(FwdK, unsigned int*, mask, l);
      const int mtp = ITp::mt(w);
      if constexpr (R > 0 && !SPREAD) {
        auto flush_prev = [&]() {
#pragma unroll
          for (int k = 0; k < ITp::IPW; ++k) {
            const int b = ITp::blk(w, k);
            if constexpr (ACTS) {
              {
                const unsigned tb_ = xbuf_lds + (unsigned)(ib * WS_BUF * 16 + b * 2 * 16 * 1024 + mtp * 2048);
                ws_tr_issue(tb_ + trl, tb_ + trl2, trt);
              }
              tr_wait(trt);
              tr_store(actp, 32 * MTp, s0 + 64 * b, mtp, lane, trt);
            }
            if constexpr (ST && !TAN && Net::L[R > 0 ? R - 1 : 0].relu != 0) maskp[((size_t)(2 * tile + b) * MTp + mtp) * 64 + lane] = pbits[k];
          }
        };
        if constexpr (ST) {
          if (ITp::active(w)) flush_prev();
        } else {
          if (actp != nullptr && ITp::active(w)) flush_prev();
        }
      }
      WsPiece tp;

      if (active) {
        sfor<0, IT::IPW>([&](auto kc) {
          constexpr int k = decltype(kc)::value;
          const int b = IT::blk(w, k);
          constexpr int KL = IT::IPW - 1;
          f32x16_t acc[2];
          constexpr int BD = G < WS_BD ? G : WS_BD;
          u32x4_t bq[BD][2];
          const unsigned pe_a = ebuf_lds + (unsigned)((2 * b * UE) * 1024 + lane * 16), px_a = xbuf_lds + (unsigned)(ib * WS_BUF * 16 + (2 * b * 16) * 1024 + lane_s * 16);
          auto b_read = [&](auto gc, u32x4_t (&dst)[2]) {
            constexpr int g = decltype(gc)::value;
            if constexpr (g < GE) {
              ws_lds_read<g * 1024>(dst[0], pe_a);
              ws_lds_read<(UE + g) * 1024>(dst[1], pe_a);
            } else {
              ws_lds_read<(g - GE) * 1024>(dst[0], px_a);
              ws_lds_read<(16 + g - GE) * 1024>(dst[1], px_a);
            }
          };
          sfor<0, BD>([&](auto gc) { b_read(gc, bq[decltype(gc)::value]); });
          if constexpr (k == 0) {
            if (bias_lds_path) {
              ws_lds_wait4<2 * BD>(br);
#pragma unroll
              for (int i = 0; i < 4; ++i) {
                bv[0][4 * i + 0] = __uint_as_float(br[i].x); bv[0][4 * i + 1] = __uint_as_float(br[i].y);
                bv[0][4 * i + 2] = __uint_as_float(br[i].z); bv[0][4 * i + 3] = __uint_as_float(br[i].w);
              }
              bv[1] = bv[0];
            }
          }
          acc[0] = bv[0];
          acc[1] = bv[1];
          sfor<0, G>([&](auto gc) {
            constexpr int g = decltype(gc)::value;
            constexpr int NEWER = 2 * ((G - 1 - g) < (BD - 1) ? (G - 1 - g) : (BD - 1));
            ws_lds_wait<NEWER>(bq[g % BD][0], bq[g % BD][1]);
            mma_b(acc[0], A[g], bq[g % BD][0]);
            mma_b(acc[1], A[g], bq[g % BD][1]);
            if constexpr (SPREAD && k < NHOST) {
              using SP = WsSpread<G, (NPI > 0 ? NPI : 1)>;
              sfor<0, (SPREAD ? NPI : 0)>([&](auto ic) {
                constexpr int i = decltype(ic)::value, pi = k * NPI + i, kp = pi / 4, qa = pi % 4;
                if constexpr (SP::issue_at(i) == g) {
                  const unsigned tb_ = xbuf_lds + (unsigned)(ib * WS_BUF * 16 + ITp::blk(w, kp) * 2 * 16 * 1024 + mtp * 2048);
                  ws_trp_issue<qa>(tb_ + trl, tb_ + trl2, tp);
                }
              });
            }
            if constexpr (g + BD < G) b_read(std::integral_constant<int, g + BD>{}, bq[g % BD]);
            if constexpr (SPREAD && k < NHOST) {
              using SP = WsSpread<G, (NPI > 0 ? NPI : 1)>;
              sfor<0, (SPREAD ? NPI : 0)>([&](auto ic) {
                constexpr int i = decltype(ic)::value, pi = k * NPI + i, kp = pi / 4, qa = pi % 4;
                if constexpr (SP::perm_at(i) == g) ws_trp_perm<SP::newer(SP::issue_at(i), true, g, BD)>(tp);
                if constexpr (SP::store_at(i) == g) {
                  ws_trp_store<qa, SP::newer(SP::perm_at(i), false, g, BD)>(actp, 32 * MTp, s0 + 64 * ITp::blk(w, kp), mtp, lane, tp);
                  if constexpr (!TAN && qa == 3 && Net::L[R > 0 ? R - 1 : 0].relu != 0) maskp[((size_t)(2 * tile + ITp::blk(w, kp)) * MTp + mtp) * 64 + lane] = pbits[kp];
                }
              });
            }
            if (k == KL && g < Gn) A[g] = load_a(Wn, Gn, mtn, g, lane);
          });
          if (k < KL) {
            if constexpr (ls.pf != 0) load_bias(IT::blk(w, k + 1), bv);
          }
          if constexpr (!LAST && ls.add_ext == 0) {
#pragma unroll
            for (int t = 0; t < 2; ++t) acc_fence(acc[t]);
            unsigned int pw[2][8];
#pragma unroll
            for (int t = 0; t < 2; ++t)
#pragma unroll
              for (int kk = 0; kk < 8; ++kk) pw[t][kk] = pack2bf_op(acc[t][2 * kk], acc[t][2 * kk + 1]);
            if constexpr (ls.relu != 0 && TAN) {
#pragma unroll
              for (int t = 0; t < 2; ++t)
#pragma unroll
                for (int kk = 0; kk < 8; ++kk) pw[t][kk] = pk_mask_bf16(pw[t][kk], pk_m01(tbits[k], t, kk));
            } else if constexpr (ls.relu != 0) {
              if constexpr (ST) pbits[k] = pk_alive_bits(pw);
#pragma unroll
              for (int t = 0; t < 2; ++t)
#pragma unroll
                for (int kk = 0; kk < 8; ++kk) pw[t][kk] = pk_relu_bf16(pw[t][kk]);
            }
#pragma unroll
            for (int t = 0; t < 2; ++t)
#pragma unroll
              for (int q = 0; q < 2; ++q)
                xout[((2 * b + t) * 16 + 2 * mt + q) * 64 + lane_s] = make_uint4(pw[t][4 * q], pw[t][4 * q + 1], pw[t][4 * q + 2], pw[t][4 * q + 3]);
          } else if constexpr (!LAST) {
            if constexpr (ls.relu != 0) {
              if constexpr (ST) {
                unsigned int bits = 0;
#pragma unroll
                for (int t = 0; t < 2; ++t)
#pragma unroll
                  for (int r = 0; r < 16; ++r) bits |= (acc[t][r] > 0.f ? 1u : 0u) << mask_bit<P>(t, r);
                pbits[k] = bits;
              }
#pragma unroll
              for (int t = 0; t < 2; ++t)
#pragma unroll
                for (int r = 0; r < 16; ++r) acc[t][r] = relu1(acc[t][r]);
            }
            {
              f32x16_t e[2];
              tile_from_raw<P>(ext_raw, lane, e);
#pragma unroll
              for (int t = 0; t < 2; ++t)
#pragma unroll
                for (int r = 0; r < 16; ++r) acc[t][r] += e[t][r];
            }
            if (k < KL) load_ext(IT::blk(w, k + 1));
#pragma unroll
            for (int t = 0; t < 2; ++t) {
              uint4 u[2];
              tile_to_units<P>(acc[t], u);
#pragma unroll
              for (int q = 0; q < 2; ++q) xout[((2 * b + t) * 16 + 2 * mt + q) * 64 + lane_s] = u[q];
            }
          } else {
#pragma unroll
            for (int t = 0; t < 2; ++t) {
              const int s = s0 + 64 * b + 2 * n + t;
#pragma unroll
              for (int r = 0; r < 16; ++r) {
                const int f = 32 * mt + drow(r, h);
                if (f < Net::COUT && s < S_eff && a.out) a.out[(size_t)s * Net::COUT + f] = acc[t][r];
              }
            }
          }
        });
      } else {
        a_load(std::integral_constant<int, 0>{}, std::integral_constant<int, (Gn < G ? Gn : G)>{}, Wn, Gn, mtn);
      }
      ws_layer_barrier();
      Wn_c = Wn_n;
      act_c = act_n;
      mask_c = mask_n;
      ws_pin_sgpr(Wn_c);
      ws_pin_sgpr(act_c);
      ws_pin_sgpr(mask_c);
    });
    xcur = xnext;
  }
}

template <class Net>
constexpr int wsb_gk(int l) { return pad32(Net::L[l].mout) / 16; }
template <class Net>
constexpr bool wsb_same(int a, int b) {
  if (!bwd_same<Net>(a, b)) return false;
  if ((a == Net::NL - 1) != (b == Net::NL - 1)) return false;
  const int an = a > 0 ? a - 1 : Net::NL - 1, bn = b > 0 ? b - 1 : Net::NL - 1;
  return wsb_gk<Net>(an) == wsb_gk<Net>(bn);
}
template <class Net>
constexpr int wsb_rep(int l) {
  for (int j = Net::NL - 1; j > l; --j)
    if (wsb_same<Net>(j, l)) return j;
  return l;
}
template <class Net>
constexpr unsigned wsb_members(int r) {
  unsigned m = 0;
  for (int l = 0; l < Net::NL; ++l)
    if (wsb_rep<Net>(l) == r) m |= 1u << l;
  return m;
}
template <class Net>
__device__ __forceinline__ int wsb_first_tile(int l, int w, bool want_dx) {
  int v = 0;
  sfor<0, Net::NL>([&](auto ic) {
    constexpr int i = decltype(ic)::value;
    constexpr int MTE = Net::L[i].ke / 32, MTA = Net::L[i].kin / 32;
    if (l == i) {
      if (MTE > 0 && want_dx && w < 2 * MTE) v = w % (MTE > 0 ? MTE : 1);
      else v = (i > 0 && MTA > 0) ? MTE + (w & ((MTA > 0 ? MTA : 1) - 1)) : 0;
    }
  });
  return v;
}
template <class Net>
__device__ __forceinline__ int wsb_mta_rt(int l) {
  int v = 0;
  sfor<0, Net::NL>([&](auto ic) {
    constexpr int i = decltype(ic)::value;
    if (l == i) v = i > 0 ? Net::L[i].kin / 32 : 0;
  });
  return v;
}

template <class Net, bool DZ = true>
__global__ void __launch_bounds__(512) k_mlp_bwd_ws(BwdK a) {
  static_assert(ws_ok<Net>(), "weights-stationary chain: 256-wide posenc nets only");
  using P = PBF16;
  constexpr int NL = Net::NL, KE = Net::KE, GMAX = 16;
  constexpr int MTE_ANY = KE / 32;
  __shared__ uint4 xbuf[2 * WS_BUF];
  __shared__ float red[8 * 2 * 3 * 32];
  const int tid = threadIdx.x, lane = tid & 63, n = lane & 31, h = lane >> 5;
  const int w = __builtin_amdgcn_readfirstlane((int)(threadIdx.x >> 6));
  const unsigned xbuf_lds = lds_addr(xbuf);
  const unsigned trl = ws_tr_lane(lane), trl2 = trl ^ 32u;
  const int lane_s = ws_slot(lane);
  const int ntw = a.S_pad / WS_TILE;
  const bool want_dx = a.d_x != nullptr;

  uint4 A[GMAX];
  auto a_load = [&](auto g1c, const GLOBAL_AS void* Wp, int G, int rt) {
    constexpr int G1 = decltype(g1c)::value;
#pragma unroll
    for (int g = 0; g < G1; ++g) A[g] = load_a(Wp, G, rt, g, lane);
  };
  if ((int)blockIdx.x < ntw) {
    constexpr int GK0 = wsb_gk<Net>(NL - 1);
    a_load(std::integral_constant<int, GK0>{}, KARG_PTR(BwdK, const void*, WT, NL - 1), GK0, wsb_first_tile<Net>(NL - 1, w, want_dx));
  }
  TrTile trt;
  auto mask_slot_after = [](int ln_) { const int q = ln_ > 0 ? ln_ - 1 : 0; return q >= 1 ? q - 1 : 0; };
  const GLOBAL_AS void* Wn_c = KARG_PTR(BwdK, const void*, WT, (NL >= 2 ? NL - 2 : 0));
  GLOBAL_AS void* dz_c = KARG_PTR(BwdK, void*, dz, NL - 1);
  const GLOBAL_AS unsigned int* maskq_c = KARG_PTR(BwdK, const unsigned int*, mask, mask_slot_after(NL - 1));
  auto mask_req = [&](int lq , int tile, unsigned int (&m)[2], const GLOBAL_AS unsigned int* mp) {
    int mta = wsb_mta_rt<Net>(lq >= 1 ? lq : 1);
    mta = mta > 0 ? mta : 8;
    const int j = w & (mta - 1);
#pragma unroll
    for (int k = 0; k < 2; ++k) {
      const int b = mta >= 8 ? k : ((w / mta) & 1);
      m[k] = mp[((size_t)(2 * tile + b) * mta + j) * 64 + lane];
    }
  };

  constexpr bool DPRE = Net::COUT <= 4;
  constexpr int DN = DPRE ? Net::COUT : 1;
  auto d_fetch = [&](int tile_, float (&d)[2][DN]) {
    if constexpr (DPRE) {
      if (w < 2 && tile_ < ntw) {
#pragma unroll
        for (int t = 0; t < 2; ++t) {
          const int s = tile_ * WS_TILE + 64 * w + 2 * n + t;
#pragma unroll
          for (int r = 0; r < DN; ++r) {
            const int f = drow(r, h);
            d[t][r] = (f < Net::COUT && s < a.S) ? a.d_out[(size_t)s * Net::COUT + f] : 0.f;
          }
        }
      }
    }
  };
  float dcur[2][DN], dnext[2][DN];
#pragma unroll
  for (int t = 0; t < 2; ++t)
#pragma unroll
    for (int r = 0; r < DN; ++r) dcur[t][r] = dnext[t][r] = 0.f;
  d_fetch((int)blockIdx.x, dcur);
  for (int tile = blockIdx.x; tile < ntw; tile += gridDim.x) {
    const int s0 = tile * WS_TILE;
    d_fetch(tile + (int)gridDim.x, dnext);
    float dx[2][3];
#pragma unroll
    for (int t = 0; t < 2; ++t) dx[t][0] = dx[t][1] = dx[t][2] = 0.f;
    unsigned int mcur[2], mnext[2];
    mask_req(NL - 1, tile, mcur, KARG_PTR(BwdK, const unsigned int*, mask, (NL >= 2 ? NL - 2 : 0)));

    if (w < 2) {
      const int b = w;
      f32x16_t g[2];
#pragma unroll
      for (int t = 0; t < 2; ++t) {
        const int s = s0 + 64 * b + 2 * n + t;
#pragma unroll
        for (int r = 0; r < 16; ++r) {
          const int f = drow(r, h);
          if constexpr (DPRE) g[t][r] = r < DN ? dcur[t][r < DN ? r : 0] : 0.f;
          else g[t][r] = (f < Net::COUT && s < a.S) ? a.d_out[(size_t)s * Net::COUT + f] : 0.f;
        }
      }
      if constexpr (DZ) store_tile<P>((GLOBAL_AS void*)a.dz[NL - 1], pad32(Net::L[NL - 1].mout), s0 + 64 * b, 0, lane, g);
#pragma unroll
      for (int t = 0; t < 2; ++t) {
        uint4 u[2];
        tile_to_units<P>(g[t], u);
#pragma unroll
        for (int q = 0; q < 2; ++q) xbuf[((2 * b + t) * 16 + q) * 64 + lane_s] = u[q];
      }
    }
    wg_step_barrier();

#pragma nounroll
    for (int l = NL - 1; l >= 0; --l)
    sfor<0, NL>([&](auto ri) {
      constexpr int R = NL - 1 - decltype(ri)::value;
      if constexpr (wsb_rep<Net>(R) != R) return;
      constexpr unsigned MEMBERS = wsb_members<Net>(R);
      if (!((MEMBERS >> l) & 1u)) return;
      constexpr LS ls = Net::L[R];
      constexpr LS lp = Net::L[R > 0 ? R - 1 : 0];
      constexpr int GK = wsb_gk<Net>(R);
      constexpr int MTE = ls.ke / 32, MTA = ls.kin / 32;
      constexpr bool DO_ACT = (R > 0 && MTA > 0);
      constexpr int GKn = wsb_gk<Net>(R > 0 ? R - 1 : NL - 1);
      using IT = WsItems<(DO_ACT ? MTA : 1)>;
      const int lm1 = l > 0 ? l - 1 : 0;
      const int ln = l > 0 ? l - 1 : NL - 1;
      const GLOBAL_AS void* Wn = Wn_c;
      const GLOBAL_AS void* Wn_n = KARG_PTR(BwdK, const void*, WT, (ln > 0 ? ln - 1 : NL - 1));
      GLOBAL_AS void* dz_n = KARG_PTR(BwdK, void*, dz, ln);
      const GLOBAL_AS unsigned int* maskq_n = KARG_PTR(BwdK, const unsigned int*, mask, mask_slot_after(ln));
      const int rtn = wsb_first_tile<Net>(ln, w, want_dx);
      const int ib = (NL - 1 - l) & 1;
      uint4* xout = xbuf + (ib ^ 1) * WS_BUF;
      const bool act_on = DO_ACT && IT::active(w);
      const bool emb_on = MTE > 0 && want_dx && w < 2 * MTE;
      const int j = IT::mt(w);
      const int me = MTE > 0 ? w % (MTE > 0 ? MTE : 1) : 0, be = MTE > 0 ? (w / (MTE > 0 ? MTE : 1)) & 1 : 0;

#pragma unroll
      for (int g = GK; g < GKn; ++g) A[g] = load_a(Wn, GKn, rtn, g, lane);
      mask_req(lm1, tile, mnext, maskq_c);
      uint4 raw[4];
      if constexpr (MTE > 0) {
        if (emb_on) load_tile_raw<P>((const GLOBAL_AS void*)a.emb, KE, s0 + 64 * be, me, lane, raw);
      }
      if constexpr (DO_ACT && lp.ext_grad != 0) {
        if (act_on && !emb_on) load_tile_raw<P>((const GLOBAL_AS void*)a.ext_gin, pad32(lp.mout), s0 + 64 * IT::blk(w, 0), j, lane, raw);
      }
      static_assert(!(MTE > 0 && DO_ACT && lp.ext_grad != 0), "one prefetched tile per layer");
      constexpr int MTp = GK / 2;
      using ITp = WsItems<MTp>;
      constexpr int NP = (DZ && R < NL - 1) ? 4 * ITp::IPW : 0;
      constexpr int NHOST = IT::IPW;
      constexpr int NPI = NP / NHOST;
      constexpr bool SPREAD = NP > 0 && DO_ACT && IT::ITEMS >= 8 && ITp::ITEMS >= 8 && NP % NHOST == 0 && WsSpread<GK, (NPI > 0 ? NPI : 1)>::OK;
      GLOBAL_AS void* dzl = dz_c;
      const int jp = ITp::mt(w);
      if constexpr (NP > 0 && !SPREAD) {
        if (ITp::active(w)) {
#pragma unroll
          for (int k = 0; k < ITp::IPW; ++k) {
            const int b = ITp::blk(w, k);
            {
              const unsigned tb_ = xbuf_lds + (unsigned)(ib * WS_BUF * 16 + b * 2 * 16 * 1024 + jp * 2048);
              ws_tr_issue(tb_ + trl, tb_ + trl2, trt);
            }
            tr_wait(trt);
            tr_store(dzl, 32 * MTp, s0 + 64 * b, jp, lane, trt);
          }
        }
      }
      WsPiece tp;

      auto mfma_item = [&](int b, f32x16_t (&acc)[2], auto pf_c, auto gp_c, const GLOBAL_AS void* Wp, int rt, auto host_c) {
        constexpr bool PF = decltype(pf_c)::value;
        constexpr int GP = decltype(gp_c)::value;
        constexpr int HK = decltype(host_c)::value;
#pragma unroll
        for (int t = 0; t < 2; ++t)
#pragma unroll
          for (int r = 0; r < 16; ++r) acc[t][r] = 0.f;
        constexpr int BD = GK < WS_BD ? GK : WS_BD;
        u32x4_t bq[BD][2];
        const unsigned px_a = xbuf_lds + (unsigned)(ib * WS_BUF * 16 + (2 * b * 16) * 1024 + lane_s * 16);
        auto b_read = [&](auto gc, u32x4_t (&dst)[2]) {
          constexpr int g = decltype(gc)::value;
          ws_lds_read<g * 1024>(dst[0], px_a);
          ws_lds_read<(16 + g) * 1024>(dst[1], px_a);
        };
        sfor<0, BD>([&](auto gc) { b_read(gc, bq[decltype(gc)::value]); });
        sfor<0, GK>([&](auto gc) {
          constexpr int g = decltype(gc)::value;
          constexpr int NEWER = 2 * ((GK - 1 - g) < (BD - 1) ? (GK - 1 - g) : (BD - 1));
          ws_lds_wait<NEWER>(bq[g % BD][0], bq[g % BD][1]);
          mma_b(acc[0], A[g], bq[g % BD][0]);
          mma_b(acc[1], A[g], bq[g % BD][1]);
          if constexpr (SPREAD && HK >= 0 && HK < NHOST) {
            using SP = WsSpread<GK, (NPI > 0 ? NPI : 1)>;
            sfor<0, (SPREAD ? NPI : 0)>([&](auto ic) {
              constexpr int i = decltype(ic)::value, pi = (HK >= 0 ? HK : 0) * NPI + i, kp = pi / 4, qa = pi % 4;
              if constexpr (SP::issue_at(i) == g) {
                const unsigned tb_ = xbuf_lds + (unsigned)(ib * WS_BUF * 16 + ITp::blk(w, kp) * 2 * 16 * 1024 + jp * 2048);
                ws_trp_issue<qa>(tb_ + trl, tb_ + trl2, tp);
              }
            });
          }
          if constexpr (g + BD < GK) b_read(std::integral_constant<int, g + BD>{}, bq[g % BD]);
          if constexpr (SPREAD && HK >= 0 && HK < NHOST) {
            using SP = WsSpread<GK, (NPI > 0 ? NPI : 1)>;
            sfor<0, (SPREAD ? NPI : 0)>([&](auto ic) {
              constexpr int i = decltype(ic)::value, pi = (HK >= 0 ? HK : 0) * NPI + i, kp = pi / 4, qa = pi % 4;
              if constexpr (SP::perm_at(i) == g) ws_trp_perm<SP::newer(SP::issue_at(i), true, g, BD)>(tp);
              if constexpr (SP::store_at(i) == g) ws_trp_store<qa, SP::newer(SP::perm_at(i), false, g, BD)>(dzl, 32 * MTp, s0 + 64 * ITp::blk(w, kp), jp, lane, tp);
            });
          }
          if constexpr (PF && g < GP) A[g] = load_a(Wp, GP, rt, g, lane);
        });
      };

      bool loaded_next = false;
      if constexpr (MTE > 0) {
        if (emb_on) {
          f32x16_t acc[2];
          if constexpr (DO_ACT) mfma_item(be, acc, std::true_type{}, std::integral_constant<int, GK>{}, KARG_PTR(BwdK, const void*, WT, l), MTE + j, std::integral_constant<int, -1>{});
          else { mfma_item(be, acc, std::true_type{}, std::integral_constant<int, GKn>{}, Wn, rtn, std::integral_constant<int, -1>{}); loaded_next = true; }
          f32x16_t e[2];
          tile_from_raw<P>(raw, lane, e);
          constexpr int L = Net::NFREQ;
          sfor<0, (MTE > 0 ? MTE : 1)>([&](auto mc) {
            constexpr int MEc = decltype(mc)::value;
            if (me != MEc) return;
            sfor<0, 16>([&](auto rc) {
              constexpr int r = decltype(rc)::value;
              constexpr int S0 = 32 * MEc + (r & 3) + 8 * (r >> 2), S1 = S0 + 4;
              constexpr int K0 = S0 < 6 * L ? 1 : (S0 < 6 * L + 3 ? 2 : 0), K1 = S1 < 6 * L ? 1 : (S1 < 6 * L + 3 ? 2 : 0);
              if constexpr (K0 != 0 || K1 != 0) {
                constexpr int F0 = (S0 >> 1) / 3, F1 = (S1 >> 1) / 3;
                constexpr int A0 = K0 == 1 ? (S0 >> 1) % 3 : (K0 == 2 ? S0 - 6 * L : -1), A1 = K1 == 1 ? (S1 >> 1) % 3 : (K1 == 2 ? S1 - 6 * L : -1);
#pragma unroll
                for (int t = 0; t < 2; ++t) {
                  const float gv = acc[t][r];
                  const float partner = e[t][r ^ 1];
                  const float sp = (r & 1) ? -partner : partner;
                  float c;
                  if constexpr (K0 == 1 && K1 == 1) {
                    c = ldexpf(sp, h ? F1 : F0) * gv;
                  } else {
                    const float c0 = K0 == 1 ? ldexpf(sp, F0) * gv : (K0 == 2 ? gv : 0.f);
                    const float c1 = K1 == 1 ? ldexpf(sp, F1) * gv : (K1 == 2 ? gv : 0.f);
                    c = h ? c1 : c0;
                  }
#pragma unroll
                  for (int k = 0; k < 3; ++k) {
                    if (A0 == k && A1 == k) dx[t][k] += c;
                    else if (A0 == k) dx[t][k] += h ? 0.f : c;
                    else if (A1 == k) dx[t][k] += h ? c : 0.f;
                  }
                }
              }
            });
          });
        }
      }
      if constexpr (DO_ACT) {
        if (act_on) {
          sfor<0, IT::IPW>([&](auto kc) {
            constexpr int k = decltype(kc)::value;
            const int b = IT::blk(w, k);
            constexpr int KL = IT::IPW - 1;
              f32x16_t acc[2];
            if constexpr (k == KL) mfma_item(b, acc, std::true_type{}, std::integral_constant<int, GKn>{}, Wn, rtn, kc);
            else mfma_item(b, acc, std::false_type{}, std::integral_constant<int, 0>{}, Wn, rtn, kc);
            if constexpr (lp.ext_grad != 0) {
              f32x16_t eg[2];
              tile_from_raw<P>(raw, lane, eg);
#pragma unroll
              for (int t = 0; t < 2; ++t)
#pragma unroll
                for (int r = 0; r < 16; ++r) acc[t][r] += eg[t][r];
              if (k < KL) load_tile_raw<P>((const GLOBAL_AS void*)a.ext_gin, pad32(lp.mout), s0 + 64 * IT::blk(w, k + 1), j, lane, raw);
            }
            if constexpr (lp.add_ext != 0) store_tile<P>((GLOBAL_AS void*)a.ext_gout, pad32(lp.mout), s0 + 64 * b, j, lane, acc);
#pragma unroll
            for (int t = 0; t < 2; ++t) acc_fence(acc[t]);
            unsigned int pw[2][8];
#pragma unroll
            for (int t = 0; t < 2; ++t)
#pragma unroll
              for (int kk = 0; kk < 8; ++kk) pw[t][kk] = pack2bf_op(acc[t][2 * kk], acc[t][2 * kk + 1]);
            {
              unsigned int alive = lp.relu != 0 ? mcur[k] : 0xffffffffu;
#pragma unroll
              for (int t = 0; t < 2; ++t)
                if (s0 + 64 * b + 2 * n + t >= a.S) alive &= ~(0x00ff00ffu << (8 * t));
#pragma unroll
              for (int t = 0; t < 2; ++t)
#pragma unroll
                for (int kk = 0; kk < 8; ++kk) pw[t][kk] = pk_mask_bf16(pw[t][kk], pk_m01(alive, t, kk));
            }
#pragma unroll
            for (int t = 0; t < 2; ++t)
#pragma unroll
              for (int q = 0; q < 2; ++q)
                xout[((2 * b + t) * 16 + 2 * j + q) * 64 + lane_s] = make_uint4(pw[t][4 * q], pw[t][4 * q + 1], pw[t][4 * q + 2], pw[t][4 * q + 3]);
          });
          loaded_next = true;
        }
      }
      if (!loaded_next) a_load(std::integral_constant<int, (GKn < GK ? GKn : GK)>{}, Wn, GKn, rtn);
      mcur[0] = mnext[0];
      mcur[1] = mnext[1];
      ws_layer_barrier();
      Wn_c = Wn_n;
      dz_c = dz_n;
      maskq_c = maskq_n;
      ws_pin_sgpr(Wn_c);
      ws_pin_sgpr(dz_c);
      ws_pin_sgpr(maskq_c);
    });

#pragma unroll
    for (int t = 0; t < 2; ++t)
#pragma unroll
      for (int r = 0; r < DN; ++r) dcur[t][r] = dnext[t][r];
    if (want_dx) {
      if (w < 2 * MTE_ANY) {
#pragma unroll
        for (int t = 0; t < 2; ++t)
#pragma unroll
          for (int k = 0; k < 3; ++k) {
            const float v = dx[t][k] + __shfl_xor(dx[t][k], 32, 64);
            if (h == 0) red[((w * 2 + t) * 3 + k) * 32 + n] = v;
          }
      }
      wg_step_barrier();
      if (w < 2 && h == 0) {
        const int b = w;
#pragma unroll
        for (int t = 0; t < 2; ++t) {
          const int s = s0 + 64 * b + 2 * n + t;
          float v[3] = {0.f, 0.f, 0.f};
#pragma unroll
          for (int m = 0; m < MTE_ANY; ++m)
#pragma unroll
            for (int k = 0; k < 3; ++k) v[k] += red[(((b * MTE_ANY + m) * 2 + t) * 3 + k) * 32 + n];
          if (s < a.S) {
            a.d_x[(size_t)s * 3 + 0] = v[0];
            a.d_x[(size_t)s * 3 + 1] = v[1];
            a.d_x[(size_t)s * 3 + 2] = v[2];
          }
        }
      }
    }
  }
}

inline int mlp_grid_ws(int ntiles) {
  static int n_cu = 0;
  if (n_cu == 0) {
    int dev = 0;
    hipDeviceProp_t prop;
    if (hipGetDevice(&dev) != hipSuccess || hipGetDeviceProperties(&prop, dev) != hipSuccess) prop.multiProcessorCount = 256;
    n_cu = prop.multiProcessorCount > 0 ? prop.multiProcessorCount : 256;
  }
  const char* ge = getenv("LAB4D_CHAIN_GRID");
  const int grid_env = ge ? atoi(ge) : 0;
  int g = ntiles < n_cu ? ntiles : n_cu;
  if (grid_env > 0 && g > grid_env) g = grid_env;
  return g < 1 ? 1 : g;
}

inline bool ws_enabled() {
  const char* e = getenv("LAB4D_WS");
  return e == nullptr || atoi(e) != 0;
}

}
```

lab4d_amd/mlp.py:

```python
import ctypes
import os
import weakref
from typing import NamedTuple

import torch
from torch.autograd import Function
from torch.autograd.function import once_differentiable

from . import _lib

MAXL = 12
PREC_F32, PREC_BF16 = 0, 1
vp, ci = ctypes.c_void_p, ctypes.c_int


@_lib.mirrors("lab4d_mlp_layer")
class LayerDesc(ctypes.Structure):
    _fields_ = [(n, ci) for n in ("ke", "kin", "mout", "mout_pad", "relu", "pf_bias", "add_ext", "ext_grad")]


@_lib.mirrors("lab4d_mlp_desc")
class NetDesc(ctypes.Structure):
    _fields_ = [(n, ci) for n in ("n_layers", "emb_kind", "n_freq", "c_in", "emb_slots", "ke", "c_out")] + [("layers", LayerDesc * MAXL)]


@_lib.mirrors("lab4d_mlp_fwd_args")
class FwdArgs(ctypes.Structure):
    _fields_ = [("net", ci), ("precision", ci), ("S", ci), ("S_pad", ci), ("ld", ci), ("spf", ci), ("x", vp), ("freq_w", vp),
                ("W", vp * MAXL), ("bias", vp * MAXL), ("pf_bias", vp * MAXL), ("act", vp * MAXL), ("mask", vp * MAXL), ("emb", vp),
                ("ext", vp), ("out", vp), ("x2", vp), ("S_dev", vp), ("frame_idx", vp), ("aff", vp)]


@_lib.mirrors("lab4d_mlp_bwd_args")
class BwdArgs(ctypes.Structure):
    _fields_ = [("net", ci), ("precision", ci), ("S", ci), ("S_pad", ci), ("ld", ci), ("spf", ci), ("WT", vp * MAXL), ("act", vp * MAXL),
                ("mask", vp * MAXL), ("emb", vp), ("ext", vp), ("d_out", vp), ("ext_gin", vp), ("ext_gout", vp), ("dz", vp * MAXL), ("d_x", vp),
                ("d_x2", vp), ("x", vp), ("aff", vp), ("g_aff", vp)]


@_lib.mirrors("lab4d_mlp_bwd_fused_args")
class BwdFusedArgs(ctypes.Structure):
    _fields_ = [("net", ci), ("precision", ci), ("S", ci), ("spf", ci), ("x", vp), ("freq_w", vp), ("aff", vp), ("W", vp * MAXL), ("WT", vp * MAXL),
                ("bias", vp * MAXL), ("pf_bias", vp * MAXL), ("d_out", vp), ("d_x", vp), ("g_aff", vp), ("dW", vp * MAXL), ("db", vp * MAXL),
                ("pf_db", vp * MAXL)]


class NetInfo(NamedTuple):
    id: int
    name: str
    kernel: str
    macs: int
    ws: bool


NETS = (
    NetInfo(0, "fg_base", "FgBase", 572928 + 256, True),
    NetInfo(1, "fg_color", "FgColor", 158464 + 37248, True),
    NetInfo(2, "vis", "Vis", 10240, False),
    NetInfo(3, "feat", "Feat", 77568, False),
    NetInfo(4, "skin", "Skin", 20736, False),
    NetInfo(5, "dense", "Dense", 39 * 256 + 256 * 256 + 256 * 3, True),
    NetInfo(6, "bg_base", "BgBase", 100096 + 128, False),
    NetInfo(7, "bg_color", "BgColor", 43392 + 8576, False),
    NetInfo(8, "skin18", "Skin18", (54 + 160) * 64 + 64 * 64 + 64 * 18, False),
    NetInfo(9, "hash_geo", "HashGeo", 32 * 64 + 64 * 16, False),
    NetInfo(10, "hash_color", "HashColor", 19 * 64 + 64 * 64 + 64 * 3, False),
    NetInfo(11, "dense6", "Dense6", 199 * 256 + 3 * 256 * 256 + 455 * 256 + 256 * 256 + 256 * 3, True),
    NetInfo(12, "skin_a", "SkinA", 4 * 64 + 64 * 64 + 64 * 25, False),
    NetInfo(13, "skin18_a", "Skin18A", 4 * 64 + 64 * 64 + 64 * 18, False),
)
(NET_FG_BASE, NET_FG_COLOR, NET_VIS, NET_FEAT, NET_SKIN, NET_DENSE, NET_BG_BASE, NET_BG_COLOR, NET_SKIN18, NET_HASH_GEO, NET_HASH_COLOR, NET_DENSE6,
 NET_SKIN_A, NET_SKIN18_A) = (n.id for n in NETS)
NET_NAMES = {n.id: n.name for n in NETS}
KERNEL_NET = {n.id: n.kernel for n in NETS}
NET_MACS = {n.id: n.macs for n in NETS}
WS_NETS = tuple(n.id for n in NETS if n.ws)


def ws_active(net, prec, dx_only=False):
    e = os.environ.get("LAB4D_WS")
    try:
        on = e is None or int(e.strip() or "0") != 0
    except ValueError:
        on = False
    return bool(on and prec == PREC_BF16 and net in WS_NETS)


def chain_kernel_name(kind, net, prec, dx_only=False):
    return "k_mlp_%s%s<%s>" % (kind, "_ws" if ws_active(net, prec, dx_only) else "", KERNEL_NET[net])


def wgrad_kernel_name(L, prec):
    if prec == PREC_BF16 and L.mout_pad == 32 and os.environ.get("LAB4D_WGRAD_HEAD_DMA", "1") not in ("", "0") and L.ke + L.kin <= 256:
        return "k_mlp_wgrad_dma<1,%d>" % (2 if L.ke + L.kin <= 128 else 4)
    if prec == PREC_BF16 and L.mout_pad in (64, 128, 256):
        K = L.ke + L.kin
        nbw = 1 if K <= 64 else (2 if K <= 128 else (3 if K <= 192 else (4 if K <= 256 else (5 if (L.mout_pad == 256 and K <= 320) else 3))))
        return "k_mlp_wgrad_dma<%d,%d>" % (L.mout_pad // 32, nbw)
    if L.mout_pad >= 256:
        return "k_mlp_wgrad_big"
    return "k_mlp_wgrad<%d>" % (4 if L.mout_pad >= 128 else (2 if L.mout_pad >= 64 else 1))


def wgrad_work(L, S_pad, prec):
    K = L.ke + L.kin
    esize = 2 if prec == PREC_BF16 else 4
    return (2.0 * S_pad * L.mout * K, float((L.mout_pad + K) * S_pad * esize + L.mout_pad * K * 4))


_DESC = {}


def describe(net):
    if net not in _DESC:
        d = NetDesc()
        _lib.call("mlp_describe", net, ctypes.byref(d))
        _DESC[net] = d
    return _DESC[net]


def store_dtype(prec):
    return torch.bfloat16 if prec == PREC_BF16 else torch.float32


def posenc_slot_to_ref_channel(n_freq, ke):
    out = []
    for slot in range(ke):
        if slot < 6 * n_freq:
            pair, t = slot >> 1, slot & 1
            f, a = pair // 3, pair % 3
            out.append(3 + f * 6 + t * 3 + a)
        elif slot < 6 * n_freq + 3:
            out.append(slot - 6 * n_freq)
        else:
            out.append(-1)
    return out


class LayerBinding:

    def __init__(self, wname, bname, emb0=None, cond=None, prev0=None, aux0=None):
        self.wname, self.bname = wname, bname
        self.aux0 = aux0
        self.emb0 = emb0
        self.cond = cond
        self.prev0 = prev0


def _lb(q, name, **blocks):
    return LayerBinding(q + name + ".weight", q + name + ".bias", **blocks)


def _hidden(q, D, n_emb, n_cond=0, skip=None):
    cond = (n_emb, n_cond) if n_cond else None
    out = [_lb(q, "linear_1.0", emb0=0, cond=cond)]
    for i in range(2, D + 1):
        out.append(_lb(q, "linear_%d.0" % i, emb0=0, cond=cond, prev0=n_emb + n_cond) if i == (skip or 0) + 1 else _lb(q, "linear_%d.0" % i, prev0=0))
    return out


def _mlp(q, D, n_emb, n_cond=0, skip=None):
    return _hidden(q, D, n_emb, n_cond, skip) + [_lb(q, "linear_final", prev0=0)]


def bindings(net, prefix=""):
    p = prefix
    if net == NET_FG_BASE:
        return _hidden(p + "basefield.", 8, 63, 32, skip=4) + [_lb(p, "basefield.linear_final.0", prev0=0), _lb(p, "sdf", prev0=0)]
    if net == NET_BG_BASE:
        return _hidden(p + "basefield.", 5, 39, 32, skip=4) + [_lb(p, "basefield.linear_final.0", prev0=0), _lb(p, "sdf", prev0=0)]
    if net == NET_FG_COLOR:
        return _hidden(p + "colorfield.", 2, 75, 32) + [_lb(p, "colorfield.linear_final.0", prev0=0), _lb(p, "rgb.0", prev0=0, cond=(256, 32)),
                                                        _lb(p, "rgb.2", prev0=0)]
    if net == NET_BG_COLOR:
        return _hidden(p + "colorfield.", 2, 51, 32) + [_lb(p, "colorfield.linear_final.0", prev0=0), _lb(p, "rgb.0", prev0=0, aux0=128),
                                                        _lb(p, "rgb.2", prev0=0)]
    if net == NET_VIS:
        return _mlp(p + "vis_mlp.basefield.", 2, 63, 32)
    if net == NET_FEAT:
        return _mlp(p + "feature_field.", 5, 39, skip=4)
    if net in (NET_SKIN, NET_SKIN18):
        return _mlp(p + "warp.skinning_model.delta_field.", 2, 75 if net == NET_SKIN else 54, 160)
    if net in (NET_SKIN_A, NET_SKIN18_A):
        q = p + "warp.skinning_model.delta_field."
        return [_lb(q, "linear_2.0", emb0=0), _lb(q, "linear_final", prev0=0)]
    if net == NET_DENSE:
        return _mlp(p, 2, 39, 160)
    if net == NET_DENSE6:
        return _mlp(p, 6, 39, 160, skip=4)
    if net == NET_HASH_GEO:
        return [_lb(p, "hash.geo.0", emb0=0), _lb(p, "hash.geo.2", prev0=0)]
    if net == NET_HASH_COLOR:
        return [_lb(p, "hash.color.0", emb0=0), _lb(p, "hash.color.2", prev0=0), _lb(p, "hash.color.4", prev0=0)]
    raise ValueError(net)


def skin_net_for(n_bones, affine=False):
    if n_bones == 25:
        return NET_SKIN_A if affine else NET_SKIN
    if n_bones == 18:
        return NET_SKIN18_A if affine else NET_SKIN18
    raise NotImplementedError("lab4d_amd: the delta-skin network is instantiated for 25 and 18 bones (got %d)" % n_bones)


_COLMAP = {}


def col_map(net, layer, device):
    key = (net, layer, str(device))
    if key not in _COLMAP:
        d = describe(net)
        L = d.layers[layer]
        bd = bindings(net)[layer]
        cm = []
        if L.ke:
            if d.emb_kind == 0:
                ref = posenc_slot_to_ref_channel(d.n_freq, L.ke)
                for slot in range(L.ke):
                    c = ref[slot]
                    a0 = 6 * d.n_freq + 3
                    if bd.emb0 is not None and c >= 0:
                        cm.append(bd.emb0 + c)
                    elif bd.aux0 is not None and a0 <= slot < a0 + 3:
                        cm.append(bd.aux0 + slot - a0)
                    else:
                        cm.append(-1)
            elif d.emb_kind == 2:
                cm += [bd.emb0 + c for c in range(L.ke)]
            else:
                cm += [(bd.emb0 + c if c < d.c_in else -1) for c in range(L.ke)]
        if L.kin:
            cm += [bd.prev0 + j for j in range(L.kin)]
        _COLMAP[key] = torch.tensor(cm, dtype=torch.int32, device=device)
    return _COLMAP[key]


FUSED_GRAD_ACCUM = False


FUSED_NARROW_BWD = os.environ.get("LAB4D_FUSED_NARROW", "1") != "0"


def _grad_sink(p):
    g = p.grad if FUSED_GRAD_ACCUM else None
    if g is None or g.dtype != torch.float32 or not g.is_contiguous() or g.shape != p.shape:
        return None
    return g


ALWAYS_PACK = False
_COLIDX = {}


def col_index(net, layer, device):
    key = (net, layer, str(device))
    if key not in _COLIDX:
        cm = col_map(net, layer, device).cpu()
        k = torch.nonzero(cm >= 0).flatten()
        _COLIDX[key] = (k.to(device), cm[k].long().to(device))
    return _COLIDX[key]


_PACK_CACHE = {}


def packed_weights(net, layer, prec, W, transposed):
    key = (net, layer, prec, transposed)
    ver = W._version
    ent = _PACK_CACHE.get(id(W))
    if ent is None or ent[0]() is not W:
        ent = (weakref.ref(W), {})
        _PACK_CACHE[id(W)] = ent
        weakref.finalize(W, _PACK_CACHE.pop, id(W), None)
    per = ent[1]
    hit = per.get(key)
    if hit is not None and hit[0] == ver and hit[1].device == W.device and not ALWAYS_PACK:
        return hit[1]
    out = _pack_into(net, layer, prec, W, transposed, hit[1] if (hit is not None and hit[1].device == W.device) else None)
    if not ALWAYS_PACK:
        per[key] = (ver, out)
    return out


def _pack_into(net, layer, prec, W, transposed, out=None):
    d = describe(net)
    L = d.layers[layer]
    Wc = W.detach().contiguous()
    _lib.require_device(Wc)
    if out is None or ALWAYS_PACK:
        out = torch.empty(L.mout_pad * (L.ke + L.kin), dtype=store_dtype(prec), device=W.device)
    cm = col_map(net, layer, W.device)
    _lib.call("mlp_pack", net, layer, prec, 1 if transposed else 0, Wc, Wc.shape[1], cm, out)
    return out


def repack_all(force=False):
    n = 0
    for ref, per in list(_PACK_CACHE.values()):
        W = ref()
        if W is None:
            continue
        for key, (ver, buf) in list(per.items()):
            if force or ver != W._version:
                per[key] = (W._version, _pack_into(key[0], key[1], key[2], W, key[3], buf))
                n += 1
    return n


def clear_caches():
    _PACK_CACHE.clear()
    _COLMAP.clear()
    _COLIDX.clear()


def pf_bias_of(net, layer, W, cond):
    c0, n = bindings(net)[layer].cond
    return cond @ W[:, c0:c0 + n].t()


def s_pad_of(S):
    return (S + 255) // 256 * 256


def buf_numel(F, S_pad):
    return (S_pad // 64) * (F * 64 + 128)


def mask_numel(L, S_pad, prec):
    return (S_pad // (64 if prec == PREC_BF16 else 32)) * (L.mout_pad // 32) * 64


def bind_forward(net, prec, S, S_pad, spf, Ws, bs, pfs):
    d = describe(net)
    a = FwdArgs()
    a.net, a.precision, a.S, a.S_pad, a.ld, a.spf = net, prec, S, S_pad, S_pad, spf
    pfs = iter(pfs)
    packed, biases, tables = [], [], []
    for l in range(d.n_layers):
        L = d.layers[l]
        pw = packed_weights(net, l, prec, Ws[l], False)
        b = bs[l].detach().float()
        if b.numel() != L.mout_pad:
            b = torch.nn.functional.pad(b, (0, L.mout_pad - b.numel()))
        b = b.contiguous()
        a.W[l], a.bias[l] = _lib.dp(pw), _lib.dp(b)
        pf = None
        if L.pf_bias:
            pf = (next(pfs).detach().float() + b[None]).contiguous()
            if pf.shape[1] != L.mout_pad:
                raise RuntimeError("per-frame bias of layer %d must have %d columns" % (l, L.mout_pad))
            a.pf_bias[l] = _lib.dp(pf)
        packed.append(pw)
        biases.append(b)
        tables.append(pf)
    return a, packed, biases, tables


def bind_backward(net, prec, S, S_pad, spf, Ws, masks, with_dz=True, ext_gin=None):
    d = describe(net)
    dev, sdt = Ws[0].device, store_dtype(prec)
    a = BwdArgs()
    a.net, a.precision, a.S, a.S_pad, a.ld, a.spf = net, prec, S, S_pad, S_pad, spf
    packed_t, dz = [], [None] * d.n_layers
    for l in range(d.n_layers):
        L = d.layers[l]
        pw = packed_weights(net, l, prec, Ws[l], True)
        a.WT[l] = _lib.dp(pw)
        packed_t.append(pw)
        if masks[l] is not None:
            a.mask[l] = _lib.dp(masks[l])
        if with_dz:
            dz[l] = torch.empty(buf_numel(L.mout_pad, S_pad), dtype=sdt, device=dev)
            a.dz[l] = _lib.dp(dz[l])
        if L.ext_grad:
            if ext_gin is None:
                ext_gin = torch.zeros(buf_numel(L.mout_pad, S_pad), dtype=sdt, device=dev)
            ext_gin = ext_gin.contiguous()
            a.ext_gin = _lib.dp(ext_gin)
    return a, packed_t, dz, ext_gin


def _to_reference(net, l, W, dWk, sink=None):
    kcols, rcols = col_index(net, l, W.device)
    mout = describe(net).layers[l].mout
    if sink is not None:
        sink.index_add_(1, rcols, dWk[:mout].index_select(1, kcols))
        return None
    gW = torch.zeros_like(W, dtype=torch.float32)
    gW[:, rcols] = dWk[:mout][:, kcols]
    return gW


def collect_wgrads(net, prec, S, S_pad, spf, M, Ws, bs, emb, layers, eikonal=False):
    d = describe(net)
    bias_out, tag, what = (False, "@eik", "(eikonal)") if eikonal else (True, "", "")
    dev = emb.device
    sinks, sizes = [], []
    for l, (_, _, need_w, need_b, _) in enumerate(layers):
        L = d.layers[l]
        sw = _grad_sink(Ws[l]) if need_w else None
        sb = _grad_sink(bs[l]) if (need_b and sw is not None and not L.pf_bias) else None
        sinks.append((sw, sb))
        sizes.append((0 if sw is not None else L.mout_pad * (L.ke + L.kin), L.mout_pad if (bias_out and sb is None) else 0,
                      M * L.mout_pad if L.pf_bias else 0))
    arena = torch.zeros(sum(sum(t) for t in sizes), device=dev)
    aoff = 0
    out = []
    for l, (dz, prev, need_w, need_b, need_pf) in enumerate(layers):
        L = d.layers[l]
        gW = gb = pfd = None
        if need_w or need_b or need_pf:
            (n0, n1, n2), (sw, sb) = sizes[l], sinks[l]
            dWk = arena[aoff:aoff + n0].view(L.mout_pad, L.ke + L.kin) if sw is None else None
            dbk = arena[aoff + n0:aoff + n0 + n1] if (bias_out and sb is None) else None
            pfd = arena[aoff + n0 + n1:aoff + n0 + n1 + n2].view(M, L.mout_pad) if need_pf else None
            with _lib.timed(wgrad_kernel_name(L, prec) + tag, wgrad_work(L, S_pad, prec)):
                if sw is not None:
                    _lib.call("mlp_wgrad_mapped", net, l, prec, S, S_pad, S_pad, spf, dz, emb, prev, sw, sw.shape[1], col_map(net, l, dev),
                              sb if sb is not None else dbk, pfd, M, what="mlp_wgrad_mapped" + what)
                else:
                    _lib.call("mlp_wgrad", net, l, prec, S, S_pad, S_pad, spf, dz, emb, prev, dWk, dbk, pfd, M, what="mlp_wgrad" + what)
            if need_w and sw is None:
                gW = _to_reference(net, l, Ws[l], dWk)
            if need_b and sb is None:
                gb = (pfd.sum(0) if need_pf else dbk)[:L.mout].reshape(bs[l].shape)
        aoff += sum(sizes[l])
        out.append((gW, gb, pfd))
    return out


CHAIN_LEAD = ("net", "prec", "spf", "x", "ext", "freq_w", "export_layer", "n_pf", "x2", "tap")


class Wants:

    def __init__(self, x=False, ext=False, freq_w=False, x2=False, pfs=(), params=()):
        self.x, self.ext, self.freq_w, self.x2, self.pfs, self.params = bool(x), bool(ext), bool(freq_w), bool(x2), tuple(pfs), tuple(params)

    @property
    def beyond_x(self):
        return self.ext or self.freq_w or self.x2 or any(self.pfs) or any(self.params)

    @property
    def any(self):
        return self.x or self.beyond_x


class ChainState:
    __slots__ = ("net", "prec", "spf", "S", "S_pad",
                 "want",
                 "params",
                 "pf_used",
                 "acts", "masks", "emb", "ext",
                 "dx_only",
                 "fused",
                 "x_shape", "has_x2",
                 "aff_in",
                 "g_aff")

    def __init__(self, **kw):
        for k in self.__slots__:
            setattr(self, k, kw.pop(k))
        assert not kw, kw


def chain_forward(net, prec, spf, x, pfs, params, want, ext=None, freq_w=None, export_layer=-1, x2=None, aff=None, tap=None):
    d = describe(net)
    NL = d.n_layers
    pfs, params = list(pfs), list(params)
    assert len(params) == 2 * NL
    Ws, bs = params[0::2], params[1::2]
    spf = int(spf)
    x = x.contiguous()
    _lib.require_device(x)
    if x.dtype != torch.float32:
        raise RuntimeError("MlpChain: x must be fp32")
    S = x.shape[0]
    S_pad = s_pad_of(S)
    dev = x.device
    sdt = store_dtype(prec)
    need_grad = want.any
    fused = bool(need_grad and FUSED_NARROW_BWD and export_layer < 0 and ext is None and x2 is None and tap is None
                 and _lib.lib().lab4d_mlp_fused_backward_supported(net, prec, spf))
    store = need_grad and not fused
    dx_only = bool(store and net in (NET_FG_BASE, NET_BG_BASE) and export_layer < 0 and ext is None and tap is None and not want.beyond_x)
    if d.emb_kind == 2 and aff is None:
        raise RuntimeError("MlpChain: net %d needs the per-frame affine table aff" % net)
    if aff is not None:
        rows = d.ke if d.emb_kind == 2 else d.c_in
        if tuple(aff.shape[1:]) != (rows, 4) or x.shape[1] != 3 or aff.dtype != torch.float32 or not aff.is_contiguous():
            raise RuntimeError("MlpChain: aff must be a contiguous fp32 (M, %d, 4) table and x the (S,3) points" % rows)
        _lib.require_device(aff)
    a, pw_used, bias_used, pf_used = bind_forward(net, prec, S, S_pad, spf, Ws, bs, pfs)
    a.x = _lib.dp(x)
    if aff is not None:
        a.aff = _lib.dp(aff)
    if x2 is not None:
        x2 = x2.contiguous().float()
        _lib.require_device(x2)
        a.x2 = _lib.dp(x2)
    if freq_w is not None:
        freq_w = freq_w.contiguous().float()
        a.freq_w = _lib.dp(freq_w)
    acts = [None] * NL
    masks = [None] * NL
    for l in range(NL):
        L = d.layers[l]
        if (store and not dx_only and l + 1 < NL) or l == export_layer:
            acts[l] = torch.empty(buf_numel(L.mout_pad, S_pad), dtype=sdt, device=dev)
            a.act[l] = _lib.dp(acts[l])
        if store and L.relu and l + 1 < NL:
            masks[l] = torch.empty(mask_numel(L, S_pad, prec), dtype=torch.int32, device=dev)
            a.mask[l] = _lib.dp(masks[l])
    emb = None
    if store:
        emb = torch.empty(buf_numel(d.ke, S_pad), dtype=sdt, device=dev)
        a.emb = _lib.dp(emb)
    if ext is not None:
        ext = ext.contiguous()
        if ext.dtype != sdt:
            raise RuntimeError("ext must be stored as %s" % sdt)
        a.ext = _lib.dp(ext)
    out = torch.empty(S, d.c_out, device=dev)
    a.out = _lib.dp(out)
    nbytes = sum(t.numel() * t.element_size() for t in acts + masks + [emb, ext, out, x] if t is not None)
    with _lib.timed(chain_kernel_name("fwd", net, prec, dx_only) + ("" if store else " inference"), (2.0 * S * NET_MACS[net], float(nbytes))):
        _lib.call("mlp_forward", ctypes.byref(a))
    if tap is not None and need_grad:
        tap.update(net=net, prec=prec, S=S, S_pad=S_pad, masks=list(masks), emb=emb)
    st = ChainState(net=net, prec=prec, spf=spf, S=S, S_pad=S_pad, want=want, params=params, pf_used=pf_used, acts=acts, masks=masks, emb=emb,
                    ext=ext, dx_only=dx_only, g_aff=None,
                    fused={"x": x, "freq_w": freq_w, "aff": aff, "W": pw_used, "bias": bias_used} if fused else None,
                    x_shape=x.shape if aff is None else (S, d.c_in),
                    has_x2=x2 is not None,
                    aff_in=(x, aff) if (d.emb_kind == 2 and need_grad) else None)
    return out, (acts[export_layer].view(-1) if export_layer >= 0 else None), st


def chain_backward(st, d_out, d_export=None):
    if st.params is None:
        raise RuntimeError("MlpChain: backward a second time through a chain whose stored activations have been released")
    if st.fused is not None:
        return chain_backward_fused(st, d_out)
    net, prec, spf, S, S_pad, want = st.net, st.prec, st.spf, st.S, st.S_pad, st.want
    d = describe(net)
    NL = d.n_layers
    Ws, bs = st.params[0::2], st.params[1::2]
    dev = d_out.device
    a, packed_t, dz, d_export = bind_backward(net, prec, S, S_pad, spf, Ws, st.masks, with_dz=not st.dx_only, ext_gin=d_export)
    for l in range(NL):
        if st.acts[l] is not None:
            a.act[l] = _lib.dp(st.acts[l])
    if st.emb is not None:
        a.emb = _lib.dp(st.emb)
    ext_g = None
    if st.ext is not None:
        a.ext = _lib.dp(st.ext)
        ext_g = torch.empty_like(st.ext)
        a.ext_gout = _lib.dp(ext_g)
    d_out = d_out.contiguous().float()
    a.d_out = _lib.dp(d_out)
    d_x = d_x2 = g_aff = None
    if st.aff_in is not None:
        xin, aff = st.aff_in
        a.x, a.aff = _lib.dp(xin), _lib.dp(aff)
        g_aff = torch.zeros_like(aff)
        a.g_aff = _lib.dp(g_aff)
    if want.x or want.x2 or g_aff is not None:
        d_x = torch.empty(st.x_shape, device=dev)
        a.d_x = _lib.dp(d_x)
        if st.has_x2:
            d_x2 = torch.empty(st.x_shape, device=dev)
            a.d_x2 = _lib.dp(d_x2)
    nbytes = sum(t.numel() * t.element_size() for t in list(dz) + list(st.masks) + [d_out, d_x, ext_g, st.emb if d_x is not None else None, d_export]
                 if t is not None)
    with _lib.timed(chain_kernel_name("bwd", net, prec, st.dx_only), (2.0 * S * NET_MACS[net], float(nbytes))):
        _lib.call("mlp_backward", ctypes.byref(a))
    need_pf = iter(want.pfs)
    layers = [(dz[l], st.acts[l - 1] if d.layers[l].kin else None, want.params[2 * l], want.params[2 * l + 1],
               bool(d.layers[l].pf_bias) and bool(next(need_pf))) for l in range(NL)]
    grads = collect_wgrads(net, prec, S, S_pad, spf, (S + spf - 1) // spf, Ws, bs, st.emb, layers)
    _release(st, g_aff)
    return d_x, ext_g, d_x2, [g[2] for l, g in enumerate(grads) if d.layers[l].pf_bias], [t for g in grads for t in g[:2]]


def _release(st, g_aff):
    st.acts = st.masks = st.emb = st.ext = st.params = st.aff_in = st.fused = None
    st.g_aff = g_aff


def chain_backward_fused(st, d_out):
    net, prec, spf, S, want = st.net, st.prec, st.spf, st.S, st.want
    d = describe(net)
    NL = d.n_layers
    Ws, bs = st.params[0::2], st.params[1::2]
    f = st.fused
    dev = d_out.device
    M = (S + spf - 1) // spf
    a = BwdFusedArgs()
    a.net, a.precision, a.S, a.spf = net, prec, S, spf
    a.x = _lib.dp(f["x"])
    if f["freq_w"] is not None:
        a.freq_w = _lib.dp(f["freq_w"])
    g_aff = None
    if f["aff"] is not None:
        a.aff = _lib.dp(f["aff"])
        g_aff = torch.zeros_like(f["aff"])
        a.g_aff = _lib.dp(g_aff)
    d_out = d_out.contiguous().float()
    a.d_out = _lib.dp(d_out)
    d_x = None
    if want.x or g_aff is not None:
        d_x = torch.empty(st.x_shape, device=dev)
        a.d_x = _lib.dp(d_x)
    sizes = [(L.mout_pad * (L.ke + L.kin), L.mout_pad, M * L.mout_pad if L.pf_bias else 0) for L in (d.layers[l] for l in range(NL))]
    arena = torch.zeros(sum(sum(t) for t in sizes), device=dev)
    keep, views, aoff = [], [], 0
    for l in range(NL):
        L = d.layers[l]
        n0, n1, n2 = sizes[l]
        dWk, dbk = arena[aoff:aoff + n0].view(L.mout_pad, L.ke + L.kin), arena[aoff + n0:aoff + n0 + n1]
        pfd = arena[aoff + n0 + n1:aoff + n0 + n1 + n2].view(M, L.mout_pad) if L.pf_bias else None
        aoff += n0 + n1 + n2
        views.append((dWk, dbk, pfd))
        pwt = packed_weights(net, l, prec, Ws[l], True)
        keep.append(pwt)
        a.WT[l], a.dW[l] = _lib.dp(pwt), _lib.dp(dWk)
        if l + 1 < NL:
            a.W[l] = _lib.dp(f["W"][l])
        if L.pf_bias:
            a.pf_bias[l], a.pf_db[l] = _lib.dp(st.pf_used[l]), _lib.dp(pfd)
        else:
            a.bias[l], a.db[l] = _lib.dp(f["bias"][l]), _lib.dp(dbk)
    nbytes = 4.0 * S * (3 + d.c_out + (3 if d_x is not None else 0))
    with _lib.timed("k_mlp_bwd_fused<%s>" % KERNEL_NET[net], (2.0 * S * NET_MACS[net] * 3, nbytes)):
        _lib.call("mlp_backward_fused", ctypes.byref(a))
    grads_pf, grads_params = [], []
    need_pf = iter(want.pfs)
    for l in range(NL):
        L = d.layers[l]
        dWk, dbk, pfd = views[l]
        need_w, need_b = want.params[2 * l], want.params[2 * l + 1]
        sw = _grad_sink(Ws[l]) if need_w else None
        gW = _to_reference(net, l, Ws[l], dWk, sw) if need_w else None
        gb = None
        if need_b:
            gb = (pfd.sum(0) if L.pf_bias else dbk)[:L.mout].reshape(bs[l].shape)
            sb = _grad_sink(bs[l]) if sw is not None else None
            if sb is not None:
                sb.add_(gb)
                gb = None
        if L.pf_bias:
            grads_pf.append(pfd if next(need_pf) else None)
        grads_params += [gW, gb]
    _release(st, g_aff)
    return d_x, None, None, grads_pf, grads_params


class MlpChain(Function):

    @staticmethod
    def forward(ctx, *args):
        lead, rest = dict(zip(CHAIN_LEAD, args)), args[len(CHAIN_LEAD):]
        need = dict(zip(CHAIN_LEAD, ctx.needs_input_grad))
        n_pf = lead["n_pf"]
        want = Wants(need["x"], need["ext"], need["freq_w"], need["x2"], ctx.needs_input_grad[len(CHAIN_LEAD):][:n_pf],
                     ctx.needs_input_grad[len(CHAIN_LEAD):][n_pf:])
        out, exported, ctx.state = chain_forward(lead["net"], lead["prec"], lead["spf"], lead["x"], rest[:n_pf], rest[n_pf:], want, ext=lead["ext"],
                                                 freq_w=lead["freq_w"], export_layer=lead["export_layer"], x2=lead["x2"], tap=lead["tap"])
        return out if exported is None else (out, exported)

    @staticmethod
    @once_differentiable
    def backward(ctx, d_out, d_export=None):
        d_x, d_ext, d_x2, g_pfs, g_params = chain_backward(ctx.state, d_out, d_export)
        lead = dict.fromkeys(CHAIN_LEAD)
        lead.update(x=d_x, ext=d_ext, x2=d_x2)
        return (*lead.values(), *g_pfs, *g_params)


def chain_params(net, P, prefix=""):
    return [P[n] for bd in bindings(net, prefix) for n in (bd.wname, bd.bname)]


def run_chain(net, prec, P, x, spf, conds=None, ext=None, freq_w=None, export_layer=None, prefix="", x2=None, pfs_pre=None, tap=None):
    d = describe(net)
    bd = bindings(net, prefix)
    pfs = []
    for l in range(d.n_layers):
        if d.layers[l].pf_bias:
            pfs.append(pfs_pre[l] if pfs_pre is not None and l in pfs_pre else pf_bias_of(net, l, P[bd[l].wname], conds[l]))
    return MlpChain.apply(net, prec, spf, x, ext, freq_w, -1 if export_layer is None else export_layer, len(pfs), x2, tap, *pfs,
                          *chain_params(net, P, prefix))


@torch.no_grad()
def run_chain_compacted(net, prec, P, x, frame_idx, count, conds=None, ext=None, freq_w=None, export_layer=None, prefix=""):
    d = describe(net)
    x = x.contiguous()
    _lib.require_device(x, frame_idx, count)
    if frame_idx.dtype != torch.int32 or count.dtype != torch.int32:
        raise RuntimeError("run_chain_compacted: frame_idx and count must be int32")
    S = x.shape[0]
    S_pad = s_pad_of(S)
    dev, sdt = x.device, store_dtype(prec)
    params = chain_params(net, P, prefix)
    pfs = [pf_bias_of(net, l, params[2 * l], conds[l]) for l in range(d.n_layers) if d.layers[l].pf_bias]
    a, *keep = bind_forward(net, prec, S, S_pad, 1, params[0::2], params[1::2], pfs)
    a.x, a.S_dev, a.frame_idx = _lib.dp(x), _lib.dp(count), _lib.dp(frame_idx)
    if freq_w is not None:
        freq_w = freq_w.contiguous().float()
        a.freq_w = _lib.dp(freq_w)
    exported = None
    if export_layer is not None and export_layer >= 0:
        exported = torch.empty(buf_numel(d.layers[export_layer].mout_pad, S_pad), dtype=sdt, device=dev)
        a.act[export_layer] = _lib.dp(exported)
    if ext is not None:
        if ext.dtype != sdt:
            raise RuntimeError("ext must be stored as %s" % sdt)
        a.ext = _lib.dp(ext)
    out = torch.empty(S, d.c_out, device=dev)
    a.out = _lib.dp(out)
    with _lib.timed(chain_kernel_name("fwd", net, prec) + " inference", (2.0 * S * NET_MACS[net], 0.0)):
        _lib.call("mlp_forward", ctypes.byref(a), what="mlp_forward(compacted)")
    return (out, exported) if exported is not None else out


class EikonalSdf(Function):

    @staticmethod
    def forward(ctx, net, prec, spf, x, freq_w, pf0, pf4, tap, *params):
        if net not in (NET_FG_BASE, NET_BG_BASE):
            raise RuntimeError("EikonalSdf: the eikonal term exists for the basefield / sdf networks only (net %d)" % net)
        d = describe(net)
        NL = d.n_layers
        Ws, bs = params[0::2], params[1::2]
        x = x.detach().contiguous()
        _lib.require_device(x)
        S = x.shape[0]
        S_pad = s_pad_of(S)
        spf = int(spf)
        dev, sdt = x.device, store_dtype(prec)
        a, packed, *keep = bind_forward(net, prec, S, S_pad, spf, Ws, bs, [pf0, pf4])
        a.x = _lib.dp(x)
        fw = None
        if freq_w is not None:
            fw = freq_w.detach().contiguous().float()
            a.freq_w = _lib.dp(fw)
        masks, tact = [None] * NL, [None] * NL
        for l in range(NL - 1):
            L = d.layers[l]
            if L.relu:
                masks[l] = torch.empty(mask_numel(L, S_pad, prec), dtype=torch.int32, device=dev)
                a.mask[l] = _lib.dp(masks[l])
            tact[l] = torch.empty(buf_numel(L.mout_pad, S_pad), dtype=sdt, device=dev)
            a.act[l] = _lib.dp(tact[l])
        emb = torch.empty(buf_numel(d.ke, S_pad), dtype=sdt, device=dev)
        a.emb = _lib.dp(emb)
        sdf = torch.empty(S, 1, device=dev)
        a.out = _lib.dp(sdf)
        reused = False
        if tap is not None:
            src, blk_map = tap
            ok = (src.get("net") == net and src.get("prec") == prec and S % 64 == 0 and S_pad == S and blk_map.numel() == S // 64
                  and src.get("emb") is not None and all((masks[l] is None) == (src["masks"][l] is None) for l in range(NL)))
            if ok:
                nb_src = src["S_pad"] // 64
                tpb = 2 if prec == PREC_F32 else 1
                tile_map = blk_map if tpb == 1 else (blk_map[:, None] * tpb + torch.arange(tpb, device=dev)).reshape(-1)
                for l in range(NL):
                    if masks[l] is not None:
                        masks[l] = src["masks"][l].view(nb_src * tpb, -1).index_select(0, tile_map).reshape(-1)
                emb = src["emb"].view(nb_src, -1).index_select(0, blk_map).reshape(-1)
                reused = True
        if not reused:
            with _lib.timed(chain_kernel_name("fwd", net, prec) + "@eik"):
                _lib.call("mlp_forward", ctypes.byref(a), what="mlp_forward(eikonal primal)")
        bk, packed_t, dz, zero_gin = bind_backward(net, prec, S, S_pad, spf, Ws, masks)
        bk.emb = _lib.dp(emb)
        ones = torch.ones(S, 1, device=dev)
        bk.d_out = _lib.dp(ones)
        g = torch.empty(S, 3, device=dev)
        bk.d_x = _lib.dp(g)
        with _lib.timed(chain_kernel_name("bwd", net, prec) + "@eik"):
            _lib.call("mlp_backward", ctypes.byref(bk), what="mlp_backward(eikonal primal)")
        gn = g.norm(2, dim=-1, keepdim=True)
        ctx.meta = (net, prec, spf, S, S_pad)
        ctx.saved = (x, fw, g, gn, dz, masks, packed, tact)
        ctx.params = params
        return (gn - 1) ** 2

    @staticmethod
    @once_differentiable
    def backward(ctx, ge):
        net, prec, spf, S, S_pad = ctx.meta
        x, fw, g, gn, dz, masks, packed, tact = ctx.saved
        d = describe(net)
        NL, L0 = d.n_layers, d.n_freq
        Ws, bs = ctx.params[0::2], ctx.params[1::2]
        dev, sdt = x.device, store_dtype(prec)
        u = torch.empty(S, d.ke, device=dev)
        _lib.call("eikonal_tangent_input", x, g, ge.contiguous().float(), fw, S, L0, d.ke, u)
        a = FwdArgs()
        a.net, a.precision, a.S, a.S_pad, a.ld, a.spf = net, prec, S, S_pad, S_pad, spf
        a.x = _lib.dp(u)
        for l in range(NL):
            a.W[l] = _lib.dp(packed[l])
            if masks[l] is not None:
                a.mask[l] = _lib.dp(masks[l])
            if l + 1 < NL:
                a.act[l] = _lib.dp(tact[l])
        temb = torch.empty(buf_numel(d.ke, S_pad), dtype=sdt, device=dev)
        a.emb = _lib.dp(temb)
        with _lib.timed(("k_mlp_fwd_ws_tangent<%s>@eik" if (ws_active(net, prec) and net == NET_FG_BASE) else "k_mlp_fwd_tangent<%s>@eik") % KERNEL_NET[net]):
            _lib.call("mlp_forward_tangent", ctypes.byref(a))
        need_w = ctx.needs_input_grad[-2 * NL:][0::2]
        layers = [(dz[l], tact[l - 1] if d.layers[l].kin else None, need_w[l], False, False) for l in range(NL)]
        grads = collect_wgrads(net, prec, S, S_pad, spf, 0, Ws, bs, temb, layers, eikonal=True)
        ctx.saved = None
        return (None,) * (len(ctx.needs_input_grad) - 2 * NL) + tuple(t for gr in grads for t in (gr[0], None))


def eikonal_sdf(P, x, ray_code, spf, prec, freq_w=None, prefix="", net=NET_FG_BASE, pf_rows=None, tap=None):
    bd = bindings(net, prefix)
    if pf_rows is not None:
        pf0, pf4 = pf_rows
    else:
        pf0 = pf_bias_of(net, 0, P[bd[0].wname], ray_code)
        pf4 = pf_bias_of(net, 4, P[bd[4].wname], ray_code)
    return EikonalSdf.apply(net, prec, spf, x, freq_w, pf0, pf4, tap, *chain_params(net, P, prefix))
```

Measured before the change: 776,500.

## Compute head weight gradient directly from fp32 d_out, skipping head dZ buffer

The backward kernels no longer write the output-layer dZ tile when the head gradient is taken directly from d_out. The head weight-gradient DMA kernel gains a mode that streams raw fp32 d_out into LDS through async loads, converts it to the swizzled bf16 A-tile in place, and feeds the existing MFMA pipeline. This removes one padded dZ store and its reload per backward pass, and the allocation that went with it. The cost is extra LDS staging, a conversion step with its own barrier in the pipelined loop, and narrower eligibility (bf16, small heads, no per-frame bias).

```diff
diff --git a/include/lab4d_mlp.h b/include/lab4d_mlp.h
--- a/include/lab4d_mlp.h
+++ b/include/lab4d_mlp.h
@@ -121,5 +121,8 @@
 int lab4d_mlp_wgrad_mapped(int net, int layer, int precision, int S, int S_pad, int ld, int spf, const void* dz, const void* emb,
                            const void* act_prev, float* dW_ref, int ld_ref, const int32_t* col_map, float* db, float* pf_db, int M,
                            void* stream);
+int lab4d_mlp_wgrad_head_mapped(int net, int layer, int precision, int S, int S_pad, int ld, int spf, const float* d_out, const void* emb,
+                                const void* act_prev, float* dW_ref, int ld_ref, const int32_t* col_map, float* db, float* pf_db, int M,
+                                void* stream);
 
 #endif
diff --git a/lab4d_amd/csrc/mlp.hip b/lab4d_amd/csrc/mlp.hip
--- a/lab4d_amd/csrc/mlp.hip
+++ b/lab4d_amd/csrc/mlp.hip
@@ -285,26 +285,29 @@
   asm volatile("s_waitcnt vmcnt(%0)" ::"n"(N) : "memory");
 }
 
-template <int MT, int NBW, int NW = 4, int WC = 2>
+template <int MT, int NBW, int NW = 4, int WC = 2, int HD = 0>
 __global__ void __launch_bounds__(64 * NW) k_mlp_wgrad_dma(const unsigned short* __restrict__ dz, const unsigned short* __restrict__ emb,
                                                         const unsigned short* __restrict__ actp, int ke, int kin, int S_pad, int chunk,
-                                                        int spf, int cpf, float* __restrict__ dW, float* __restrict__ db, DwMap wm) {
+                                                        int spf, int cpf, float* __restrict__ dW, float* __restrict__ db, DwMap wm,
+                                                        const float* __restrict__ dout, int S) {
   using P = PBF16;
   static_assert(NW == 4 || NW == 8, "wave grid");
+  static_assert(HD == 0 || (MT == 1 && NW == 4 && WC == 4 && (HD == 1 || HD == 2)), "head-gradient mode: the 1 x 4 head grid");
   constexpr int WR = NW / WC;
   static_assert(WR * WC == NW && (2 * NBW) % WC == 0, "wave grid");
   constexpr int TM = MT / WR, TN = 2 * NBW / WC, MO = 32 * MT, KB = 64 * NBW;
   static_assert(TM >= 1 && TM * WR == MT, "row tiles per wave");
   constexpr int A_BYTES = MT * 2048, STAGE = A_BYTES + NBW * 4096;
   constexpr int NS0 = 65536 / STAGE, NSTAGE = NS0 < 4 ? 4 : (NS0 > 8 ? 8 : NS0);
-  constexpr int PA = (2 * MT + NW - 1) / NW, PB = (4 * NBW + NW - 1) / NW, PW = PA + PB;
-  static_assert(PA * NW == 2 * MT || MT == 1, "A pieces per wave (MT = 1: two pieces, the other waves re-fetch the last one)");
+  constexpr int RAW = HD * 1024;
+  constexpr int PA = HD ? HD : (2 * MT + NW - 1) / NW, PB = (4 * NBW + NW - 1) / NW, PW = PA + PB;
+  static_assert(HD || PA * NW == 2 * MT || MT == 1, "A pieces per wave (MT = 1: two pieces, the other waves re-fetch the last one)");
   constexpr int AHEAD = NSTAGE - 1;
   constexpr bool DB_MFMA = WC == 2;
   static_assert(PW * (NSTAGE - 2) <= 63, "vmcnt range");
   static_assert(TM + TN <= 15, "lgkmcnt range");
-  static_assert(NSTAGE * STAGE <= 160 * 1024, "LDS");
-  __shared__ __attribute__((aligned(16))) unsigned char lds[NSTAGE * STAGE];
+  static_assert(NSTAGE * (STAGE + RAW) <= 160 * 1024, "LDS");
+  __shared__ __attribute__((aligned(16))) unsigned char lds[NSTAGE * (STAGE + RAW)];
   const int lane = threadIdx.x & 63, wid = __builtin_amdgcn_readfirstlane((int)(threadIdx.x >> 6)), row = lane & 31, h = lane >> 5;
   const int wr = wid / WC, wc = wid % WC;
   const int K = ke + kin;
@@ -346,6 +349,19 @@
 
   const int lane_src = (lane >> 2) * 128 + (((lane & 3) ^ ((lane >> 4) & 3)) * 16);
   const int nbp = nb / 16;
+  const long e_last = (long)S * wm.mout - 1;
+  auto issue_raw = [&](int t, int slot) {
+    const long e0 = ((long)((s_begin >> 6) + (t >> 1)) * 64 + (t & 1) * 32) * wm.mout;
+    const int e_n = 32 * wm.mout;
+#pragma unroll
+    for (int g = 0; g < HD; ++g) {
+      const int e = (wid * HD + g) * 64 + lane;
+      long idx = e0 + (e < e_n ? e : e_n - 1);
+      idx = idx < e_last ? idx : e_last;
+      __builtin_amdgcn_global_load_lds((const __attribute__((address_space(1))) unsigned int*)(dout + idx),
+                                       (__attribute__((address_space(3))) unsigned int*)(lds + NSTAGE * STAGE + slot * RAW + (wid * HD + g) * 256), 4, 0, 0);
+    }
+  };
   auto issue = [&](int st_idx, int buf) {
     int blk = (s_begin >> 6) + (st_idx >> 1);
     const int half = st_idx & 1;
@@ -353,12 +369,16 @@
     blk &= 31;
 #endif
     unsigned char* st = lds + buf * STAGE;
-    const unsigned char* ga = reinterpret_cast<const unsigned char*>(dz + (size_t)blk * block_stride(MO)) + half * 64 + lane_src;
-#pragma unroll
-    for (int p = 0; p < PA; ++p) {
-      int piece = wid + NW * p;
-      if constexpr (PA * NW != 2 * MT) piece = piece < 2 * MT ? piece : 2 * MT - 1;
-      dma_1k(ga + piece * 2048, st + piece * 1024);
+    if constexpr (HD) {
+      issue_raw(st_idx + 1, buf + 1 == NSTAGE ? 0 : buf + 1);
+    } else {
+      const unsigned char* ga = reinterpret_cast<const unsigned char*>(dz + (size_t)blk * block_stride(MO)) + half * 64 + lane_src;
+#pragma unroll
+      for (int p = 0; p < PA; ++p) {
+        int piece = wid + NW * p;
+        if constexpr (PA * NW != 2 * MT) piece = piece < 2 * MT ? piece : 2 * MT - 1;
+        dma_1k(ga + piece * 2048, st + piece * 1024);
+      }
     }
     unsigned char* sb = st + A_BYTES;
     const unsigned char* g1 = reinterpret_cast<const unsigned char*>(emb + (size_t)blk * block_stride(ke) + (size_t)k0 * 64) + half * 64 + lane_src;
@@ -373,6 +393,20 @@
     }
   };
   const unsigned lds_base = (unsigned)(size_t)(__attribute__((address_space(3))) unsigned char*)lds;
+  const int hp = HD ? (int)(threadIdx.x % (unsigned)(16 * wm.mout)) : 0;
+  const int ho = HD ? hp % wm.mout : 0, ht = HD ? 2 * (hp / wm.mout) : 0;
+  const unsigned hrd = lds_base + (unsigned)(NSTAGE * STAGE) + (unsigned)((ht * wm.mout + ho) * 4);
+  const unsigned hwr = lds_base + (unsigned)(ho * 64 + (((ht >> 3) ^ ((ho >> 2) & 3)) * 16) + (ht & 7) * 2);
+  auto convert = [&](int t, int buf) {
+    const int sg = ((s_begin >> 6) + (t >> 1)) * 64 + (t & 1) * 32 + ht;
+    const unsigned ra = hrd + (unsigned)(buf * RAW);
+    float v0, v1;
+    asm volatile("ds_read_b32 %0, %1" : "=v"(v0) : "v"(ra));
+    asm volatile("ds_read_b32 %0, %1" : "=v"(v1) : "v"(ra + (unsigned)(wm.mout * 4)));
+    asm volatile("s_waitcnt lgkmcnt(0)" : "+v"(v0), "+v"(v1));
+    const unsigned w = pack2bf(sg < S ? v0 : 0.f, sg + 1 < S ? v1 : 0.f);
+    asm volatile("ds_write_b32 %0, %1\n\ts_waitcnt lgkmcnt(0)" ::"v"(hwr + (unsigned)(buf * STAGE)), "v"(w) : "memory");
+  };
   const unsigned f = (row >> 2) & 3;
   const unsigned la0 = lds_base + (unsigned)((wr * TM * 32 + row) * 64) + ((unsigned)(h ^ f) * 16u);
   const unsigned lb0 = lds_base + (unsigned)A_BYTES + (unsigned)((wc * TN * 32 + row) * 64) + ((unsigned)(h ^ f) * 16u);
@@ -440,12 +474,23 @@
   const int N = ((s_end >> 6) - (s_begin >> 6)) * 2;
   if (N > 0) {
     u32x4_t a0[TM], b0[TN], a1[TM], b1[TN];
+    if constexpr (HD) {
+      for (int i = threadIdx.x; i < NSTAGE * (A_BYTES / 16); i += 64 * NW)
+        *reinterpret_cast<uint4*>(lds + (i / (A_BYTES / 16)) * STAGE + (i % (A_BYTES / 16)) * 16) = make_uint4(0u, 0u, 0u, 0u);
+      issue_raw(0, 0);
+    }
 #pragma unroll
     for (int i = 0; i < AHEAD; ++i)
       if (i < N) issue(i, i);
     wait_landed(min(AHEAD - 1, N - 1));
+    if constexpr (HD) asm volatile("s_waitcnt lgkmcnt(0)" ::: "memory");
     __builtin_amdgcn_s_barrier();
     asm volatile("" ::: "memory");
+    if constexpr (HD) {
+      convert(0, 0);
+      __builtin_amdgcn_s_barrier();
+      asm volatile("" ::: "memory");
+    }
     read_frags(0, IC<0>{}, a0, b0);
     int buf = 0;
     for (int s = 0; s < N; ++s) {
@@ -456,6 +501,7 @@
       wait_frags(IC<0>{}, a1, b1);
       if (s + 1 < N) {
         if (s + NSTAGE - 1 < N) issue(s + NSTAGE - 1, prev);
+        if constexpr (HD) convert(s + 1, next);
         wait_landed(min(NSTAGE - 2, N - 2 - s));
         __builtin_amdgcn_s_barrier();
         asm volatile("" ::: "memory");
@@ -670,7 +716,9 @@
       LAB4D_REQUIRE(a->WT[l], "mlp_backward: layer %d transposed weights missing", l);
       LAB4D_REQUIRE(!(Net::L[l].relu && l + 1 < Net::NL) || a->mask[l], "mlp_backward: layer %d ReLU mask missing", l);
       LAB4D_REQUIRE(!Net::L[l].ext_grad || a->ext_gin, "mlp_backward: layer %d needs ext_gin", l);
-      LAB4D_REQUIRE(a->dz[l] || (dx_only_ok<Net>() && !a->dz[0] && a->d_x), "mlp_backward: dz[%d] missing (every layer's dZ is written, or none: point gradient only)", l);
+      const bool head_skip = l == Net::NL - 1 && head_dz_optional<Net>() && a->precision == LAB4D_PREC_BF16 && a->dz[0];
+      LAB4D_REQUIRE(a->dz[l] || head_skip || (dx_only_ok<Net>() && !a->dz[0] && a->d_x),
+                    "mlp_backward: dz[%d] missing (every layer's dZ is written, every one but the head's, or none: point gradient only)", l);
       LAB4D_REQUIRE(!Net::L[l].add_ext || a->ext_gout, "mlp_backward: layer %d needs ext_gout", l);
       k.WT[l] = a->WT[l]; k.act[l] = a->act[l]; k.mask[l] = (const unsigned int*)a->mask[l]; k.dz[l] = a->dz[l];
     }
@@ -716,14 +764,42 @@
   return lab4d_mlp_wgrad_mapped(net, layer, precision, S, S_pad, ld, spf, dz, emb, act_prev, dW, 0, nullptr, db, pf_db, M, stream);
 }
 
+namespace {
+int wgrad_impl(int net, int layer, int precision, int S, int S_pad, int ld, int spf, const void* dz, const float* d_out, const void* emb,
+               const void* act_prev, float* dW, int ld_ref, const int32_t* col_map, float* db, float* pf_db, int M, void* stream);
+}
+
 extern "C" int lab4d_mlp_wgrad_mapped(int net, int layer, int precision, int S, int S_pad, int ld, int spf, const void* dz, const void* emb,
                                       const void* act_prev, float* dW, int ld_ref, const int32_t* col_map, float* db, float* pf_db, int M,
                                       void* stream) {
+  LAB4D_REQUIRE(dz, "mlp_wgrad: null dz/dW");
+  return wgrad_impl(net, layer, precision, S, S_pad, ld, spf, dz, nullptr, emb, act_prev, dW, ld_ref, col_map, db, pf_db, M, stream);
+}
+
+extern "C" int lab4d_mlp_wgrad_head_mapped(int net, int layer, int precision, int S, int S_pad, int ld, int spf, const float* d_out,
+                                           const void* emb, const void* act_prev, float* dW, int ld_ref, const int32_t* col_map, float* db,
+                                           float* pf_db, int M, void* stream) {
+  lab4d_mlp_desc d;
+  if (int e = lab4d_mlp_describe(net, &d)) return e;
+  LAB4D_REQUIRE(layer >= 0 && layer < d.n_layers, "mlp_wgrad_head: bad layer %d", layer);
+  const lab4d_mlp_layer& L = d.layers[layer];
+  LAB4D_REQUIRE(d_out, "mlp_wgrad_head: null d_out");
+  LAB4D_REQUIRE(precision == LAB4D_PREC_BF16, "mlp_wgrad_head: bf16 only (precision %d)", precision);
+  LAB4D_REQUIRE(layer == d.n_layers - 1, "mlp_wgrad_head: layer %d is not the head of net %d", layer, net);
+  LAB4D_REQUIRE(L.mout_pad == 32 && L.ke + L.kin <= 256, "mlp_wgrad_head: the head must be on the LDS-DMA ring (mout_pad 32, ke + kin <= 256; have %d, %d)",
+                L.mout_pad, L.ke + L.kin);
+  LAB4D_REQUIRE(L.mout <= 16, "mlp_wgrad_head: heads of up to 16 outputs (have %d)", L.mout);
+  return wgrad_impl(net, layer, precision, S, S_pad, ld, spf, nullptr, d_out, emb, act_prev, dW, ld_ref, col_map, db, pf_db, M, stream);
+}
+
+namespace {
+int wgrad_impl(int net, int layer, int precision, int S, int S_pad, int ld, int spf, const void* dz, const float* d_out, const void* emb,
+               const void* act_prev, float* dW, int ld_ref, const int32_t* col_map, float* db, float* pf_db, int M, void* stream) {
   lab4d_mlp_desc d;
   if (int e = lab4d_mlp_describe(net, &d)) return e;
   LAB4D_REQUIRE(layer >= 0 && layer < d.n_layers, "mlp_wgrad: bad layer %d", layer);
   const lab4d_mlp_layer& L = d.layers[layer];
-  LAB4D_REQUIRE(dz && dW, "mlp_wgrad: null dz/dW");
+  LAB4D_REQUIRE((dz || d_out) && dW, "mlp_wgrad: null dz/dW");
   LAB4D_REQUIRE(col_map == nullptr || ld_ref > 0, "mlp_wgrad_mapped: a column map needs the reference row stride");
   LAB4D_REQUIRE(L.ke == 0 || emb, "mlp_wgrad: layer %d needs the stored embedding", layer);
   LAB4D_REQUIRE(L.kin == 0 || act_prev, "mlp_wgrad: layer %d needs the previous activation", layer);
@@ -733,7 +809,7 @@
   const bool big = mo_tiles >= 8;
   const int Kt = L.ke + L.kin;
   static const int head_dma = getenv("LAB4D_WGRAD_HEAD_DMA") ? atoi(getenv("LAB4D_WGRAD_HEAD_DMA")) : 1;
-  const bool dma = precision == LAB4D_PREC_BF16 && (mo_tiles == 8 || mo_tiles == 4 || mo_tiles == 2 || (mo_tiles == 1 && head_dma && Kt <= 256));
+  const bool dma = precision == LAB4D_PREC_BF16 && (mo_tiles == 8 || mo_tiles == 4 || mo_tiles == 2 || (mo_tiles == 1 && (head_dma || d_out) && Kt <= 256));
   const int nbw = (dma && mo_tiles == 1) ? (Kt <= 128 ? 2 : 4)
                   : Kt <= 64 ? 1 : (Kt <= 128 ? 2 : (Kt <= 192 ? 3 : (Kt <= 256 ? 4 : (mo_tiles == 8 && Kt <= 320 ? 5 : 3))));
   const int TM = mo_tiles >= 4 ? 4 : (mo_tiles >= 2 ? 2 : 1);
@@ -745,6 +821,7 @@
   int chunk = div_up(div_up(S_pad, nchunks), 256) * 256; if (chunk < 1024) chunk = 1024;
   const bool fold_pf = pf_db != nullptr && spf % 256 == 0 && M > 0 && (long)M * spf >= S;
   LAB4D_REQUIRE(pf_db == nullptr || fold_pf || (M > 0 && spf > 0 && (long)M * spf >= S), "mlp_wgrad: pf_db needs M and spf, with M * spf >= S");
+  LAB4D_REQUIRE(!d_out || pf_db == nullptr || fold_pf, "mlp_wgrad_head: a per-frame bias gradient needs 256-sample aligned frames (the second pass reads a dZ tile)");
   int cpf = 0;
   if (fold_pf) {
     if (chunk > spf) chunk = spf;
@@ -763,18 +840,25 @@
 #define WGB(P) hipLaunchKernelGGL((k_mlp_wgrad_big<P>), grid, block, 0, st, (const typename P::store_t*)dz, (const typename P::store_t*)emb, \
                                   (const typename P::store_t*)act_prev, mo_tiles, L.ke, L.kin, S_pad, chunk, spf, cpf, dW, db_arg, wm)
 #define WGD(MTV, NBV) hipLaunchKernelGGL((k_mlp_wgrad_dma<MTV, NBV>), grid, block, 0, st, (const unsigned short*)dz, (const unsigned short*)emb, \
-                                         (const unsigned short*)act_prev, L.ke, L.kin, S_pad, chunk, spf, cpf, dW, db_arg, wm)
+                                         (const unsigned short*)act_prev, L.ke, L.kin, S_pad, chunk, spf, cpf, dW, db_arg, wm, (const float*)nullptr, S)
 #define WGD8(NBV) hipLaunchKernelGGL((k_mlp_wgrad_dma<8, NBV, 8>), grid, block8, 0, st, (const unsigned short*)dz, (const unsigned short*)emb, \
-                                     (const unsigned short*)act_prev, L.ke, L.kin, S_pad, chunk, spf, cpf, dW, db_arg, wm)
+                                     (const unsigned short*)act_prev, L.ke, L.kin, S_pad, chunk, spf, cpf, dW, db_arg, wm, (const float*)nullptr, S)
 #define WGD_NB(MTV) do { if (nbw == 1) WGD(MTV, 1); else if (nbw == 2) WGD(MTV, 2); else if (nbw == 3) WGD(MTV, 3); else WGD(MTV, 4); } while (0)
+#define WGH(NBV, HDV) hipLaunchKernelGGL((k_mlp_wgrad_dma<1, NBV, 4, 4, HDV>), grid, block, 0, st, (const unsigned short*)nullptr, (const unsigned short*)emb, \
+                                         (const unsigned short*)act_prev, L.ke, L.kin, S_pad, chunk, spf, cpf, dW, db_arg, wm, d_out, S)
+  if (d_out) {
+    if (nbw == 2) { if (L.mout <= 8) WGH(2, 1); else WGH(2, 2); }
+    else { if (L.mout <= 8) WGH(4, 1); else WGH(4, 2); }
+  } else
+#undef WGH
   if (dma) {
     if (mo_tiles == 8) {
       if (nbw == 1) WGD8(1); else if (nbw == 2) WGD8(2); else if (nbw == 3) WGD8(3); else if (nbw == 4) WGD8(4); else WGD8(5);
     } else if (mo_tiles == 4) WGD_NB(4); else if (mo_tiles == 2) WGD_NB(2);
     else if (nbw == 2) hipLaunchKernelGGL((k_mlp_wgrad_dma<1, 2, 4, 4>), grid, block, 0, st, (const unsigned short*)dz, (const unsigned short*)emb,
-                                          (const unsigned short*)act_prev, L.ke, L.kin, S_pad, chunk, spf, cpf, dW, db_arg, wm);
+                                          (const unsigned short*)act_prev, L.ke, L.kin, S_pad, chunk, spf, cpf, dW, db_arg, wm, (const float*)nullptr, S);
     else hipLaunchKernelGGL((k_mlp_wgrad_dma<1, 4, 4, 4>), grid, block, 0, st, (const unsigned short*)dz, (const unsigned short*)emb,
-                            (const unsigned short*)act_prev, L.ke, L.kin, S_pad, chunk, spf, cpf, dW, db_arg, wm);
+                            (const unsigned short*)act_prev, L.ke, L.kin, S_pad, chunk, spf, cpf, dW, db_arg, wm, (const float*)nullptr, S);
   }
 #undef WGD_NB
 #undef WGD8
@@ -796,6 +880,7 @@
   }
   return LAB4D_OK;
 }
+}
 
 namespace {
 template <class Net>
diff --git a/lab4d_amd/csrc/mlp_kernels.hpp b/lab4d_amd/csrc/mlp_kernels.hpp
--- a/lab4d_amd/csrc/mlp_kernels.hpp
+++ b/lab4d_amd/csrc/mlp_kernels.hpp
@@ -965,7 +965,7 @@
   return c;
 }
 
-template <class Net, class P, bool AU = true, bool DZ = true>
+template <class Net, class P, bool AU = true, bool DZ = true, bool HDZ = DZ>
 __global__ void __launch_bounds__(256, (want_occ<Net, P, true>())) k_mlp_bwd(BwdK a) {
   static_assert(Net::EMB == 0 || emb_layer_count<Net>() == 1, "raw-input nets may use the input in one layer only");
   constexpr int NT = P::NT, TILE = P::TILE, NL = Net::NL, UW = Slab<Net, P>::UW;
@@ -1059,7 +1059,7 @@
           g[t][r] = (f < Net::COUT && sidx[t] < a.S) ? a.d_out[(size_t)sidx[t] * Net::COUT + f] : 0.f;
         }
       }
-      if constexpr (DZ) store_tile<P>((GLOBAL_AS void*)a.dz[NL - 1], pad32(Net::L[NL - 1].mout), s0, 0, lane, g);
+      if constexpr (HDZ) store_tile<P>((GLOBAL_AS void*)a.dz[NL - 1], pad32(Net::L[NL - 1].mout), s0, 0, lane, g);
 #pragma unroll
       for (int t = 0; t < NT; ++t) {
         uint4 u[P::UPT];
@@ -1418,12 +1418,23 @@
 template <class Net>
 constexpr bool dx_only_ok() { return Net::ID == LAB4D_NET_FG_BASE || Net::ID == LAB4D_NET_BG_BASE; }
 template <class Net>
+constexpr bool head_dz_optional() {
+  return Net::EMB != 2 && Net::NL >= 2 && Net::COUT <= 16 && Net::L[Net::NL - 1].ke + Net::L[Net::NL - 1].kin <= 256;
+}
+template <class Net>
 inline bool launch_ws_bwd(const BwdK& k0, hipStream_t st) {
   if constexpr (ws_ok<Net>()) {
     if (!ws_enabled()) return false;
     if (!k0.dz[0]) {
       if constexpr (dx_only_ok<Net>()) {
         hipLaunchKernelGGL((k_mlp_bwd_ws<Net, false>), dim3(mlp_grid_ws(k0.S_pad / WS_TILE)), dim3(512), 0, st, k0);
+        return true;
+      }
+      return false;
+    }
+    if (!k0.dz[Net::NL - 1]) {
+      if constexpr (head_dz_optional<Net>()) {
+        hipLaunchKernelGGL((k_mlp_bwd_ws<Net, true, false>), dim3(mlp_grid_ws(k0.S_pad / WS_TILE)), dim3(512), 0, st, k0);
         return true;
       }
       return false;
@@ -1489,6 +1500,8 @@
         else LAB4D_MLP_LAUNCH((k_mlp_bwd<Net, PBF16, true>), k, st);                                                      \
       } else if (!k.dz[0]) {                                                                                              \
         if constexpr (dx_only_ok<Net>()) LAB4D_MLP_LAUNCH((k_mlp_bwd<Net, PBF16, true, false>), k, st);                   \
+      } else if (!k.dz[Net::NL - 1]) {                                                                                    \
+        if constexpr (head_dz_optional<Net>()) LAB4D_MLP_LAUNCH((k_mlp_bwd<Net, PBF16, true, true, false>), k, st);       \
       } else LAB4D_MLP_LAUNCH((k_mlp_bwd<Net, PBF16>), k, st);                         \
     } else if (precision == LAB4D_PREC_F32) {                                                                             \
       k.ntiles = k.S_pad / PF32::TILE;                                                                                   \
diff --git a/lab4d_amd/csrc/mlp_kernels_ws.hpp b/lab4d_amd/csrc/mlp_kernels_ws.hpp
--- a/lab4d_amd/csrc/mlp_kernels_ws.hpp
+++ b/lab4d_amd/csrc/mlp_kernels_ws.hpp
@@ -643,7 +643,7 @@
   return v;
 }
 
-template <class Net, bool DZ = true>
+template <class Net, bool DZ = true, bool HDZ = DZ>
 __global__ void __launch_bounds__(512) k_mlp_bwd_ws(BwdK a) {
   static_assert(ws_ok<Net>(), "weights-stationary chain: 256-wide posenc nets only");
   using P = PBF16;
@@ -730,7 +730,7 @@
           else g[t][r] = (f < Net::COUT && s < a.S) ? a.d_out[(size_t)s * Net::COUT + f] : 0.f;
         }
       }
-      if constexpr (DZ) store_tile<P>((GLOBAL_AS void*)a.dz[NL - 1], pad32(Net::L[NL - 1].mout), s0 + 64 * b, 0, lane, g);
+      if constexpr (HDZ) store_tile<P>((GLOBAL_AS void*)a.dz[NL - 1], pad32(Net::L[NL - 1].mout), s0 + 64 * b, 0, lane, g);
 #pragma unroll
       for (int t = 0; t < 2; ++t) {
         uint4 u[2];
diff --git a/lab4d_amd/mlp.py b/lab4d_amd/mlp.py
--- a/lab4d_amd/mlp.py
+++ b/lab4d_amd/mlp.py
@@ -102,10 +102,19 @@
     return "k_mlp_wgrad<%d>" % (4 if L.mout_pad >= 128 else (2 if L.mout_pad >= 64 else 1))
 
 
-def wgrad_work(L, S_pad, prec):
+def head_dout(net, prec):
+    if prec != PREC_BF16 or os.environ.get("LAB4D_HEAD_DOUT", "1") in ("", "0") or os.environ.get("LAB4D_WGRAD_HEAD_DMA", "1") in ("", "0"):
+        return False
+    d = describe(net)
+    L = d.layers[d.n_layers - 1]
+    return bool(d.emb_kind != 2 and d.n_layers >= 2 and L.mout_pad == 32 and L.mout <= 16 and L.ke + L.kin <= 256 and not L.pf_bias)
+
+
+def wgrad_work(L, S_pad, prec, S_dout=None):
     K = L.ke + L.kin
     esize = 2 if prec == PREC_BF16 else 4
-    return (2.0 * S_pad * L.mout * K, float((L.mout_pad + K) * S_pad * esize + L.mout_pad * K * 4))
+    dz_bytes = L.mout_pad * S_pad * esize if S_dout is None else S_dout * L.mout * 4
+    return (2.0 * S_pad * L.mout * K, float(dz_bytes + K * S_pad * esize + L.mout_pad * K * 4))
 
 
 _DESC = {}
@@ -356,7 +365,7 @@
     return a, packed, biases, tables
 
 
-def bind_backward(net, prec, S, S_pad, spf, Ws, masks, with_dz=True, ext_gin=None):
+def bind_backward(net, prec, S, S_pad, spf, Ws, masks, with_dz=True, ext_gin=None, head_dz=True):
     d = describe(net)
     dev, sdt = Ws[0].device, store_dtype(prec)
     a = BwdArgs()
@@ -369,7 +378,7 @@
         packed_t.append(pw)
         if masks[l] is not None:
             a.mask[l] = _lib.dp(masks[l])
-        if with_dz:
+        if with_dz and (head_dz or l + 1 < d.n_layers):
             dz[l] = torch.empty(buf_numel(L.mout_pad, S_pad), dtype=sdt, device=dev)
             a.dz[l] = _lib.dp(dz[l])
         if L.ext_grad:
@@ -391,7 +400,7 @@
     return gW
 
 
-def collect_wgrads(net, prec, S, S_pad, spf, M, Ws, bs, emb, layers, eikonal=False):
+def collect_wgrads(net, prec, S, S_pad, spf, M, Ws, bs, emb, layers, eikonal=False, d_out=None):
     d = describe(net)
     bias_out, tag, what = (False, "@eik", "(eikonal)") if eikonal else (True, "", "")
     dev = emb.device
@@ -414,8 +423,13 @@
             dWk = arena[aoff:aoff + n0].view(L.mout_pad, L.ke + L.kin) if sw is None else None
             dbk = arena[aoff + n0:aoff + n0 + n1] if (bias_out and sb is None) else None
             pfd = arena[aoff + n0 + n1:aoff + n0 + n1 + n2].view(M, L.mout_pad) if need_pf else None
-            with _lib.timed(wgrad_kernel_name(L, prec) + tag, wgrad_work(L, S_pad, prec)):
-                if sw is not None:
+            head = d_out is not None and l + 1 == d.n_layers
+            with _lib.timed(wgrad_kernel_name(L, prec) + tag, wgrad_work(L, S_pad, prec, S_dout=S if head else None)):
+                if head:
+                    _lib.call("mlp_wgrad_head_mapped", net, l, prec, S, S_pad, S_pad, spf, d_out, emb, prev, sw if sw is not None else dWk,
+                              sw.shape[1] if sw is not None else 0, col_map(net, l, dev) if sw is not None else None,
+                              sb if sb is not None else dbk, pfd, M, what="mlp_wgrad_head_mapped" + what)
+                elif sw is not None:
                     _lib.call("mlp_wgrad_mapped", net, l, prec, S, S_pad, S_pad, spf, dz, emb, prev, sw, sw.shape[1], col_map(net, l, dev),
                               sb if sb is not None else dbk, pfd, M, what="mlp_wgrad_mapped" + what)
                 else:
@@ -547,7 +561,9 @@
     NL = d.n_layers
     Ws, bs = st.params[0::2], st.params[1::2]
     dev = d_out.device
-    a, packed_t, dz, d_export = bind_backward(net, prec, S, S_pad, spf, Ws, st.masks, with_dz=not st.dx_only, ext_gin=d_export)
+    head_direct = not st.dx_only and bool(want.params[2 * NL - 2] or want.params[2 * NL - 1]) and head_dout(net, prec)
+    a, packed_t, dz, d_export = bind_backward(net, prec, S, S_pad, spf, Ws, st.masks, with_dz=not st.dx_only, ext_gin=d_export,
+                                              head_dz=not head_direct)
     for l in range(NL):
         if st.acts[l] is not None:
             a.act[l] = _lib.dp(st.acts[l])
@@ -579,7 +595,7 @@
     need_pf = iter(want.pfs)
     layers = [(dz[l], st.acts[l - 1] if d.layers[l].kin else None, want.params[2 * l], want.params[2 * l + 1],
                bool(d.layers[l].pf_bias) and bool(next(need_pf))) for l in range(NL)]
-    grads = collect_wgrads(net, prec, S, S_pad, spf, (S + spf - 1) // spf, Ws, bs, st.emb, layers)
+    grads = collect_wgrads(net, prec, S, S_pad, spf, (S + spf - 1) // spf, Ws, bs, st.emb, layers, d_out=d_out if head_direct else None)
     _release(st, g_aff)
     return d_x, ext_g, d_x2, [g[2] for l, g in enumerate(grads) if d.layers[l].pf_bias], [t for g in grads for t in g[:2]]
 
```

Result: no change. 781,200, median of 6 (+0.6%).
